# salemmohammed/Distributed-TensorFlow-Guide

Hardware: AMD Instinct MI355X
Metric: images/sec (whole node) ResNet-50 sync DP at 1/2/4/8 MI355X; scaling efficiency (higher is better)
Workload: dtype bf16; 1 GPU; model=ResNet-50, global_batch=1024, per_gpu_batch=1024, image_size=224, optimizer=momentum-sgd (fused), parallelism=dp1, allreduce=rccl bf16, 8 MB buckets, overlapped, step_launch=eager

## Files before the change

csrc/bindings/ops.cc:

```cpp
#include <torch/extension.h>
#include <c10/core/DeviceGuard.h>
#include <c10/hip/HIPStream.h>

#include "dtg/kernels.h"

namespace {

using at::Tensor;
using dtg::bf16_t;

hipStream_t cur_stream() { return c10::hip::getCurrentHIPStream().stream(); }

at::Tensor zeros_f32(long long n, const at::Tensor& like) {
  c10::DeviceGuard dg(like.device());
  at::Tensor t = at::empty({n}, like.options().dtype(at::kFloat));
  dtg::fill_zero(t.data_ptr(), n * 4, cur_stream());
  return t;
}

#define CHECK_CUDA(x) TORCH_CHECK((x).is_cuda(), #x " must be a GPU tensor")
#define CHECK_CONTIG(x) TORCH_CHECK((x).is_contiguous(), #x " must be contiguous")
#define CHECK_DT(x, dt) TORCH_CHECK((x).scalar_type() == (dt), #x " must be " #dt)
#define CHECK_IN(x) \
  CHECK_CUDA(x);    \
// ... 304 lines not shown
  TORCH_CHECK(C % 8 == 0, "C must be a multiple of 8");
  for (const Tensor* t : {&gamma, &beta, &rmean, &rvar}) {
    CHECK_IN(*t);
    CHECK_DT(*t, at::kFloat);
    TORCH_CHECK(t->numel() == C, "per-channel tensor size mismatch");
  }
  if (res.has_value() && res->defined()) {
    CHECK_IN(*res);
    CHECK_DT(*res, at::kBFloat16);
    TORCH_CHECK(res->sizes() == x.sizes(), "residual shape mismatch");
  }
  c10::DeviceGuard dg(x.device());
  auto y = at::empty_like(x);
  auto fopt = x.options().dtype(at::kFloat);
  auto smean = at::empty({C}, fopt), sinv = at::empty({C}, fopt);
  auto ws = at::empty({dtg::bn_workspace_floats(M, C)}, fopt);
  dtg::bn_fwd_train(cbfp(x), res.has_value() && res->defined() ? cbfp(*res) : nullptr, bfp(y),
                    gamma.data_ptr<float>(), beta.data_ptr<float>(), rmean.data_ptr<float>(), rvar.data_ptr<float>(),
                    smean.data_ptr<float>(), sinv.data_ptr<float>(), ws.data_ptr<float>(), M, C, (float)momentum,
                    (float)eps, relu, cur_stream());
  return {y, smean, sinv};
}

Tensor bn_fwd_infer(Tensor x, c10::optional<Tensor> res, Tensor gamma, Tensor beta, Tensor rmean, Tensor rvar,
                    double eps, bool relu) {
  CHECK_IN(x);
  CHECK_DT(x, at::kBFloat16);
  TORCH_CHECK(x.dim() == 2, "x must be [M, C]");
  const long long M = x.size(0);
  const int C = (int)x.size(1);
  TORCH_CHECK(C % 8 == 0, "C must be a multiple of 8");
  for (const Tensor* t : {&gamma, &beta, &rmean, &rvar}) {
    CHECK_IN(*t);
    CHECK_DT(*t, at::kFloat);
    TORCH_CHECK(t->numel() == C, "per-channel tensor size mismatch");
  }
  if (res.has_value() && res->defined()) {
    CHECK_IN(*res);
    TORCH_CHECK(res->sizes() == x.sizes(), "residual shape mismatch");
  }
  c10::DeviceGuard dg(x.device());
  auto y = at::empty_like(x);
  auto ws = at::empty({2LL * C}, x.options().dtype(at::kFloat));
  dtg::bn_fwd_infer(cbfp(x), res.has_value() && res->defined() ? cbfp(*res) : nullptr, bfp(y),
                    gamma.data_ptr<float>(), beta.data_ptr<float>(), rmean.data_ptr<float>(), rvar.data_ptr<float>(),
                    ws.data_ptr<float>(), M, C, (float)eps, relu, cur_stream());
  return y;
}

std::tuple<Tensor, c10::optional<Tensor>, Tensor, Tensor> bn_bwd(Tensor dy, c10::optional<Tensor> y, Tensor x,
                                                                  Tensor gamma, Tensor smean, Tensor sinv, bool relu,
                                                                  bool want_dres, c10::optional<Tensor> dgamma_acc,
                                                                  c10::optional<Tensor> dbeta_acc) {
  CHECK_IN(dy);
  CHECK_IN(x);
  CHECK_DT(dy, at::kBFloat16);
  CHECK_DT(x, at::kBFloat16);
  TORCH_CHECK(dy.sizes() == x.sizes() && x.dim() == 2, "dy/x must be [M, C]");
  const long long M = x.size(0);
  const int C = (int)x.size(1);
  TORCH_CHECK(C % 8 == 0, "C must be a multiple of 8");
  if (relu) {
    TORCH_CHECK(y.has_value() && y->defined(), "relu backward needs the saved output");
    CHECK_IN(*y);
    TORCH_CHECK(y->sizes() == x.sizes(), "y shape mismatch");
  }
  for (const Tensor* t : {&gamma, &smean, &sinv}) {
    CHECK_IN(*t);
    CHECK_DT(*t, at::kFloat);
    TORCH_CHECK(t->numel() == C, "per-channel tensor size mismatch");
  }
  c10::DeviceGuard dg(x.device());
  auto dx = at::empty_like(x);
  c10::optional<Tensor> dres;
  if (want_dres) dres = at::empty_like(x);
  auto fopt = x.options().dtype(at::kFloat);
  const bool acc = dgamma_acc.has_value() && dgamma_acc->defined() && dbeta_acc.has_value() && dbeta_acc->defined();
  Tensor dgamma, dbeta;
  if (acc) {
    dgamma = *dgamma_acc;
    dbeta = *dbeta_acc;
    for (const Tensor* t : {&dgamma, &dbeta}) {
      CHECK_IN(*t);
      CHECK_DT(*t, at::kFloat);
      TORCH_CHECK(t->numel() == C, "gradient accumulator size mismatch");
    }
  } else {
    dgamma = at::empty({C}, fopt);
    dbeta = at::empty({C}, fopt);
  }
  auto ws = at::empty({dtg::bn_workspace_floats(M, C) + C}, fopt);
  dtg::bn_bwd(cbfp(dy), relu ? cbfp(*y) : nullptr, cbfp(x), gamma.data_ptr<float>(), smean.data_ptr<float>(),
              sinv.data_ptr<float>(), bfp(dx), want_dres ? bfp(*dres) : nullptr, dgamma.data_ptr<float>(),
              dbeta.data_ptr<float>(), ws.data_ptr<float>(), M, C, relu, acc, cur_stream());
  return {dx, dres, dgamma, dbeta};
}

std::tuple<Tensor, c10::optional<Tensor>, Tensor> softmax_xent(Tensor logits, Tensor labels, double scale,
                                                                bool want_grad) {
  CHECK_IN(logits);
  CHECK_IN(labels);
  TORCH_CHECK(logits.dim() == 2, "logits must be [B, V]");
  TORCH_CHECK(logits.scalar_type() == at::kBFloat16 || logits.scalar_type() == at::kFloat, "logits bf16/fp32");
  CHECK_DT(labels, at::kLong);
  TORCH_CHECK(labels.numel() == logits.size(0), "labels size mismatch");
  c10::DeviceGuard dg(logits.device());
  const long long B = logits.size(0);
  const int V = (int)logits.size(1);
  auto fopt = logits.options().dtype(at::kFloat);
  auto loss = at::empty({B}, fopt), lse = at::empty({B}, fopt);
  c10::optional<Tensor> dx;
  if (want_grad) dx = at::empty_like(logits);
  if (B > 0)
    dtg::softmax_xent(logits.data_ptr(), logits.scalar_type() == at::kBFloat16, reinterpret_cast<const long long*>(labels.data_ptr<int64_t>()), B, V,
                      (float)scale, loss.data_ptr<float>(), want_grad ? dx->data_ptr() : nullptr,
                      lse.data_ptr<float>(), cur_stream());
  return {loss, dx, lse};
}

Tensor softmax_xent_bwd(Tensor logits, Tensor labels, Tensor lse, Tensor g, double scale) {
  CHECK_IN(logits);
  CHECK_IN(labels);
  CHECK_IN(lse);
  TORCH_CHECK(logits.dim() == 2, "logits must be [B, V]");
  TORCH_CHECK(logits.scalar_type() == at::kBFloat16 || logits.scalar_type() == at::kFloat, "logits bf16/fp32");
  CHECK_DT(labels, at::kLong);
  CHECK_DT(lse, at::kFloat);
  const long long B = logits.size(0);
  const int V = (int)logits.size(1);
  TORCH_CHECK(labels.numel() == B && lse.numel() == B, "labels / lse size mismatch");
  CHECK_CUDA(g);
  TORCH_CHECK(g.numel() == 1, "g must hold one element");
  Tensor gf = g.scalar_type() == at::kFloat ? g.contiguous() : g.to(at::kFloat);
  c10::DeviceGuard dg(logits.device());
  auto dx = at::empty_like(logits);
  if (B > 0)
    dtg::softmax_xent_bwd(logits.data_ptr(), logits.scalar_type() == at::kBFloat16,
                          reinterpret_cast<const long long*>(labels.data_ptr<int64_t>()), lse.data_ptr<float>(), B, V,
                          (float)scale, gf.data_ptr<float>(), dx.data_ptr(), cur_stream());
  return dx;
}

void gemm(Tensor A, bool a_kc, Tensor B, bool b_kc, Tensor out, double alpha, double beta,
          c10::optional<Tensor> bias, int64_t act, int64_t split_k, c10::optional<Tensor> aux, int64_t aux_mode,
          c10::optional<Tensor> colsum) {
  CHECK_CUDA(A);
  CHECK_CUDA(B);
  CHECK_CUDA(out);
  CHECK_DT(A, at::kBFloat16);
  CHECK_DT(B, at::kBFloat16);
  TORCH_CHECK(A.dim() == 2 && B.dim() == 2 && out.dim() == 2, "gemm operands must be 2-D");
  TORCH_CHECK(A.stride(1) == 1 && B.stride(1) == 1 && out.stride(1) == 1, "inner dim must be contiguous");
  TORCH_CHECK(out.scalar_type() == at::kFloat || out.scalar_type() == at::kBFloat16, "out fp32/bf16");
  const int M = (int)(a_kc ? A.size(0) : A.size(1));
  const int K = (int)(a_kc ? A.size(1) : A.size(0));
  const int N = (int)(b_kc ? B.size(0) : B.size(1));
  const int Kb = (int)(b_kc ? B.size(1) : B.size(0));
  TORCH_CHECK(K == Kb, "gemm K mismatch: ", K, " vs ", Kb);
  TORCH_CHECK(out.size(0) == M && out.size(1) == N, "gemm out shape mismatch");
  TORCH_CHECK(K % 8 == 0 || (!a_kc && !b_kc), "K-contiguous operands need K % 8 == 0 (pad the reduction dim)");
  TORCH_CHECK(a_kc || M % 8 == 0, "K-major A needs M % 8 == 0");
  TORCH_CHECK(b_kc || N % 8 == 0, "K-major B needs N % 8 == 0");
  TORCH_CHECK(A.stride(0) % 8 == 0 && B.stride(0) % 8 == 0, "row strides must be 16-byte multiples");
  TORCH_CHECK(((uintptr_t)A.data_ptr() % 16) == 0 && ((uintptr_t)B.data_ptr() % 16) == 0, "16-byte alignment");
  const float* bptr = nullptr;
  if (bias.has_value() && bias->defined()) {
    CHECK_IN(*bias);
    CHECK_DT(*bias, at::kFloat);
    TORCH_CHECK(bias->numel() == N, "bias size mismatch");
    bptr = bias->data_ptr<float>();
  }
  void* auxp = nullptr;
  if (aux_mode != 0) {
    TORCH_CHECK(aux_mode >= 1 && aux_mode <= 4, "aux_mode in {0, 1, 2, 3, 4}");
    TORCH_CHECK(aux_mode != 3 || act != 0, "aux_mode 3 stores act'(pre): needs an activation");
    TORCH_CHECK(aux.has_value() && aux->defined(), "aux_mode needs an aux tensor");
    TORCH_CHECK(aux->is_cuda() && aux->scalar_type() == at::kBFloat16 && aux->dim() == 2, "aux must be bf16 2-D");
    TORCH_CHECK(aux->size(0) == M && aux->size(1) == N && aux->stride(0) == out.stride(0) && aux->stride(1) == 1,
                "aux must match out's shape and row stride");
    auxp = aux->data_ptr();
  }
  c10::DeviceGuard dg(A.device());
  if (colsum.has_value() && colsum->defined()) {
    CHECK_IN(*colsum);
    CHECK_DT(*colsum, at::kFloat);
    TORCH_CHECK(colsum->numel() == N, "colsum must hold N floats");
    TORCH_CHECK(a_kc && !b_kc && out.scalar_type() == at::kBFloat16 && alpha == 1.0 && beta == 0.0,
                "colsum epilogue: A [M,K], B [K,N], bf16 out, alpha 1, beta 0");
    TORCH_CHECK(out.stride(0) % 8 == 0 && N % 8 == 0 && ((uintptr_t)out.data_ptr() % 16) == 0 &&
                    (bptr == nullptr || ((uintptr_t)bptr % 16) == 0) && (auxp == nullptr || ((uintptr_t)auxp % 16) == 0),
                "colsum epilogue needs 16-byte aligned rows");
    dtg::gemm_bf16_colsum(cbfp(A), A.stride(0), cbfp(B), B.stride(0), bfp(out), out.stride(0), M, N, K, bptr, (int)act,
                          auxp, (int)aux_mode, colsum->data_ptr<float>(), cur_stream());
    return;
  }
  int sk = split_k > 0 ? (int)split_k : dtg::gemm_pick_split(M, N, K, a_kc ? 1 : 0);
  Tensor ws;
  float* wsp = nullptr;
  if (sk > 1) {
    ws = at::empty({dtg::gemm_workspace_floats(M, N, K, sk)}, A.options().dtype(at::kFloat));
    wsp = ws.data_ptr<float>();
  }
  dtg::gemm_bf16(cbfp(A), A.stride(0), a_kc, cbfp(B), B.stride(0), b_kc, out.data_ptr(), out.stride(0),
                 out.scalar_type() == at::kBFloat16, M, N, K, (float)alpha, (float)beta, bptr, (int)act, sk, wsp,
                 cur_stream(), dtg::GemmBatch(), auxp, (int)aux_mode);
}

void check_nhwc(const Tensor& t, const char* what) {
  CHECK_CUDA(t);
  TORCH_CHECK(t.scalar_type() == at::kBFloat16, what, " must be bf16");
  TORCH_CHECK(t.dim() == 4 && t.is_contiguous(), what, " must be a contiguous [N,H,W,C] tensor");
  TORCH_CHECK(((uintptr_t)t.data_ptr() % 16) == 0, what, " must be 16-byte aligned");
}

bool conv_supported(int64_t C, int64_t K, int64_t R, int64_t S, int64_t stride, int64_t pad, int64_t which) {
  return dtg::conv_supported((int)C, (int)K, (int)R, (int)S, (int)stride, (int)pad, (int)which) != 0;
}

Tensor conv_fwd(Tensor x, Tensor w, int64_t stride, int64_t pad) {
  check_nhwc(x, "x");
  check_nhwc(w, "w");
  const int N = x.size(0), H = x.size(1), W = x.size(2), C = x.size(3);
  const int K = w.size(0), R = w.size(1), S = w.size(2);
  TORCH_CHECK(w.size(3) == C, "weight channels mismatch");
  TORCH_CHECK(dtg::conv_supported(C, K, R, S, stride, pad, 0), "conv shape not supported by the HIP kernel");
  const int P = (H + 2 * pad - R) / stride + 1, Q = (W + 2 * pad - S) / stride + 1;
  TORCH_CHECK(P > 0 && Q > 0, "empty output");
  TORCH_CHECK((long long)N * H * W * C < (1LL << 31) && (long long)N * P * Q * K < (1LL << 31), "tensor too large");
  c10::DeviceGuard dg(x.device());
  auto y = at::empty({N, P, Q, K}, x.options());
  dtg::conv_fwd(cbfp(x), cbfp(w), bfp(y), N, H, W, C, K, R, S, stride, pad, cur_stream());
  return y;
}


Tensor conv_dgrad(Tensor dy, Tensor w, int64_t H, int64_t W, int64_t stride, int64_t pad, c10::optional<Tensor> out,
                  double beta, bool zero_rest) {
  check_nhwc(dy, "dy");
  check_nhwc(w, "w");
  const int N = dy.size(0), P = dy.size(1), Q = dy.size(2), K = dy.size(3);
  const int R = w.size(1), S = w.size(2), C = w.size(3);
  TORCH_CHECK(w.size(0) == K, "weight/dy channel mismatch");
  TORCH_CHECK(dtg::conv_supported(C, K, R, S, stride, pad, 1), "dgrad shape not supported by the HIP kernel");
  TORCH_CHECK((H + 2 * pad - R) / stride + 1 == P && (W + 2 * pad - S) / stride + 1 == Q, "dgrad geometry mismatch");
  c10::DeviceGuard dg(dy.device());
  Tensor dx;
  if (out.has_value()) {
    dx = *out;
    check_nhwc(dx, "out");
    TORCH_CHECK(dx.size(0) == N && dx.size(1) == H && dx.size(2) == W && dx.size(3) == C, "out shape mismatch");
  } else {
    TORCH_CHECK(beta == 0.0, "beta != 0 needs out");
    dx = at::empty({N, H, W, C}, dy.options());
  }
  Tensor wT;
  TORCH_CHECK(zero_rest || (stride == 2 && R == 1 && S == 1 && pad == 0 && beta == 0.0),
              "zero_rest=False is for a stride-2 1x1 dgrad (beta 0)");
  dtg::conv_dgrad(cbfp(dy), cbfp(w), bfp(dx), N, H, W, C, K, R, S, stride, pad, (float)beta, cur_stream(),
                  dtg::BnEpi(), wT.defined() ? cbfp(wT) : nullptr, zero_rest ? 1 : 0);
  return dx;
}

std::tuple<Tensor, Tensor> conv_fwd_c8(Tensor x, Tensor w, int64_t R, int64_t S, int64_t stride, int64_t pad,
                                       bool with_stats, int64_t stride_w) {
  check_nhwc(x, "x");
  CHECK_IN(w);
  CHECK_DT(w, at::kBFloat16);
  const int sw = stride_w > 0 ? (int)stride_w : (int)stride;
  const int N = x.size(0), H = x.size(1), W = x.size(2), K = w.size(0);
  TORCH_CHECK(x.size(3) == 8, "conv_fwd_c8 needs 8 input channels");
  TORCH_CHECK(w.dim() == 2 && w.size(1) == (R * S * 8 + 63) / 64 * 64, "w must be [K, ceil64(R*S*8)]");
  TORCH_CHECK(K % 64 == 0, "K % 64");
  TORCH_CHECK(stride > 0 && sw > 0 && pad >= 0, "bad stride / pad");
  const int P = (H + 2 * pad - R) / stride + 1, Q = (W + 2 * pad - S) / sw + 1;
  TORCH_CHECK(P > 0 && Q > 0 && (long long)N * P * Q * K < (1LL << 31), "bad geometry");
  c10::DeviceGuard dg(x.device());
  auto y = at::empty({N, P, Q, K}, x.options());
  Tensor part;
  dtg::BnEpi bn;
  if (with_stats) {
    part = zeros_f32((long long)dtg::kBnStatSlots * 2 * K, x);
    bn.part = part.data_ptr<float>();
    bn.mode = 1;
  } else {
    part = at::empty({0}, x.options().dtype(at::kFloat));
  }
  dtg::conv_fwd_c8(cbfp(x), cbfp(w), bfp(y), N, H, W, K, (int)R, (int)S, (int)stride, (int)pad, cur_stream(), bn, sw);
  return {y, part};
}

constexpr int kPartRing = 16;
constexpr long long kPartCap = (long long)dtg::kBnStatSlots * 2 * 2048;
Tensor bn_part(const Tensor& like, int64_t C, bool pooled = false) {
  if (!pooled || C > 2048) return zeros_f32((long long)dtg::kBnStatSlots * 2 * C, like);
  static Tensor* ring = new Tensor[64];
  static int next[64] = {0};
  const int dev = like.get_device();
  TORCH_CHECK(dev >= 0 && dev < 64, "device index");
  if (!ring[dev].defined()) ring[dev] = zeros_f32((long long)kPartRing * kPartCap, like);
  const int i = next[dev]++ % kPartRing;
  return ring[dev].narrow(0, i * kPartCap, (long long)dtg::kBnStatSlots * 2 * C);
}

dtg::BnEpi bn_bwd_epi(Tensor& part, const Tensor& x, const Tensor& mean, const Tensor& invstd, const Tensor& gamma,
                      const Tensor& beta, long long M, int C) {
  CHECK_IN(x);
  CHECK_DT(x, at::kBFloat16);
  TORCH_CHECK(x.numel() == M * C, "BN input shape mismatch");
  for (const Tensor* t : {&mean, &invstd, &gamma, &beta}) {
    CHECK_IN(*t);
    CHECK_DT(*t, at::kFloat);
    TORCH_CHECK(t->numel() == C, "per-channel tensor size mismatch");
  }
  dtg::BnEpi bn;
  bn.part = part.data_ptr<float>();
  bn.mode = 2;
  bn.x = cbfp(x);
  bn.mean = mean.data_ptr<float>();
  bn.invstd = invstd.data_ptr<float>();
  bn.gamma = gamma.data_ptr<float>();
  bn.beta = beta.data_ptr<float>();
  return bn;
}

std::tuple<Tensor, Tensor> gemm_bn(Tensor A, Tensor B, int64_t mode, c10::optional<Tensor> x,
                                   c10::optional<Tensor> mean, c10::optional<Tensor> invstd,
                                   c10::optional<Tensor> gamma, c10::optional<Tensor> beta,
                                   c10::optional<Tensor> mask, c10::optional<Tensor> out, bool pooled,
                                   c10::optional<Tensor> x2, c10::optional<Tensor> mean2,
                                   c10::optional<Tensor> invstd2, c10::optional<Tensor> part2,
                                   c10::optional<std::tuple<int64_t, int64_t>> sub2_hw) {
  CHECK_IN(A);
  CHECK_DT(A, at::kBFloat16);
  CHECK_CUDA(B);
  CHECK_DT(B, at::kBFloat16);
  TORCH_CHECK(mode >= 1 && mode <= 3, "mode in {1, 2, 3}");
  TORCH_CHECK(A.dim() == 2 && B.dim() == 2 && B.stride(1) == 1, "2-D operands, contiguous rows");
  const int M = (int)A.size(0), K = (int)A.size(1);
  const int N = (int)(mode == 1 ? B.size(0) : B.size(1));
  TORCH_CHECK((mode == 1 ? B.size(1) : B.size(0)) == K, "gemm_bn K mismatch");
  TORCH_CHECK(K % 8 == 0 && N % 8 == 0 && B.stride(0) % 8 == 0, "K, N and row strides must be multiples of 8");
  TORCH_CHECK(((uintptr_t)A.data_ptr() % 16) == 0 && ((uintptr_t)B.data_ptr() % 16) == 0, "16-byte alignment");
  c10::DeviceGuard dg(A.device());
  Tensor o;
  float bt = 0.f;
  if (out.has_value() && out->defined()) {
    TORCH_CHECK(mode == 3, "accumulating into `out` is mode 3 only");
    o = *out;
    CHECK_IN(o);
    CHECK_DT(o, at::kBFloat16);
    TORCH_CHECK(o.numel() == (long long)M * N, "out shape mismatch");
    bt = 1.f;
  } else {
    o = at::empty({M, N}, A.options());
  }
  auto part = bn_part(A, N, pooled);
  dtg::BnEpi bn;
  if (mode >= 2) {
    TORCH_CHECK(x && mean && invstd && gamma && beta, "modes 2/3 need x, mean, invstd, gamma, beta");
    bn = bn_bwd_epi(part, *x, *mean, *invstd, *gamma, *beta, M, N);
    if (mode == 3) {
      TORCH_CHECK(mask.has_value() && mask->defined(), "mode 3 needs the mask tensor");
      CHECK_IN(*mask);
      bn.mode = 3;
      if (x2.has_value() && x2->defined()) {
        TORCH_CHECK(mean2 && invstd2 && part2, "x2 needs mean2, invstd2 and part2");
        CHECK_IN(*x2);
        CHECK_DT(*x2, at::kBFloat16);
        TORCH_CHECK(x2->numel() == (long long)M * N, "x2 shape mismatch");
        for (const Tensor* t : {&*mean2, &*invstd2}) {
          CHECK_IN(*t);
          CHECK_DT(*t, at::kFloat);
          TORCH_CHECK(t->numel() == N, "per-channel tensor size mismatch");
        }
        CHECK_IN(*part2);
        CHECK_DT(*part2, at::kFloat);
        TORCH_CHECK(part2->numel() == (long long)dtg::kBnStatSlots * 2 * N, "part2 size mismatch");
        bn.x2 = cbfp(*x2);
        bn.mean2 = mean2->data_ptr<float>();
        bn.invstd2 = invstd2->data_ptr<float>();
        bn.part2 = part2->data_ptr<float>();
      }
      if (sub2_hw.has_value()) {
        const auto [sh, sw] = *sub2_hw;
        TORCH_CHECK(bt != 0.f && sh > 0 && sw > 0 && (long long)M % (sh * sw) == 0, "sub2_hw needs out and M = N*H*W");
        dtg::bn_sub2_rows(bn, (int)sh, (int)sw);
      }
      if (mask->scalar_type() == at::kByte) {
        TORCH_CHECK(mask->numel() == (long long)M * (N / 8), "mask bits shape mismatch");
        bn.maskbits = mask->data_ptr<uint8_t>();
      } else {
        CHECK_DT(*mask, at::kBFloat16);
        TORCH_CHECK(mask->numel() == (long long)M * N, "mask shape mismatch");
        bn.mask = cbfp(*mask);
      }
    }
  } else {
    bn.part = part.data_ptr<float>();
    bn.mode = 1;
  }
  dtg::gemm_bf16_bn(cbfp(A), A.stride(0), cbfp(B), B.stride(0), bfp(o), N, M, N, K, bt, bn, cur_stream());
  return {o, part};
}

std::tuple<Tensor, Tensor> conv_fwd_bn(Tensor x, Tensor w, int64_t stride, int64_t pad, bool pooled) {
  check_nhwc(x, "x");
  check_nhwc(w, "w");
  const int N = x.size(0), H = x.size(1), W = x.size(2), C = x.size(3);
  const int K = w.size(0), R = w.size(1), S = w.size(2);
  TORCH_CHECK(w.size(3) == C, "weight channels mismatch");
  TORCH_CHECK(dtg::conv_supported(C, K, R, S, stride, pad, 0), "conv shape not supported by the HIP kernel");
  const int P = (H + 2 * pad - R) / stride + 1, Q = (W + 2 * pad - S) / stride + 1;
  TORCH_CHECK(P > 0 && Q > 0, "empty output");
  TORCH_CHECK((long long)N * H * W * C < (1LL << 31) && (long long)N * P * Q * K < (1LL << 31), "tensor too large");
  c10::DeviceGuard dg(x.device());
  auto y = at::empty({N, P, Q, K}, x.options());
  auto part = bn_part(x, K, pooled);
  dtg::BnEpi bn;
  bn.part = part.data_ptr<float>();
  bn.mode = 1;
  dtg::conv_fwd(cbfp(x), cbfp(w), bfp(y), N, H, W, C, K, R, S, stride, pad, cur_stream(), bn);
  return {y, part};
}

uint8_t* bits_ptr(const c10::optional<Tensor>& bits, long long M, int C) {
  if (!bits.has_value() || !bits->defined()) return nullptr;
  CHECK_IN(*bits);
  TORCH_CHECK(bits->scalar_type() == at::kByte && bits->numel() == M * (C / 8), "bits must be uint8 [M, C/8]");
  return bits->data_ptr<uint8_t>();
}

std::tuple<Tensor, Tensor> conv_dgrad_bn(Tensor dy, Tensor w, int64_t H, int64_t W, int64_t stride, int64_t pad,
                                         Tensor x, Tensor mean, Tensor invstd, Tensor gamma, Tensor beta,
                                         bool pooled, c10::optional<Tensor> bits) {
  check_nhwc(dy, "dy");
  check_nhwc(w, "w");
  const int N = dy.size(0), P = dy.size(1), Q = dy.size(2), K = dy.size(3);
  const int R = w.size(1), S = w.size(2), C = w.size(3);
  TORCH_CHECK(w.size(0) == K, "weight/dy channel mismatch");
  TORCH_CHECK(dtg::conv_supported(C, K, R, S, stride, pad, 1), "dgrad shape not supported by the HIP kernel");
  TORCH_CHECK((H + 2 * pad - R) / stride + 1 == P && (W + 2 * pad - S) / stride + 1 == Q, "dgrad geometry mismatch");
  c10::DeviceGuard dg(dy.device());
  auto dx = at::empty({N, H, W, C}, dy.options());
  auto part = bn_part(dy, C, pooled);
  dtg::BnEpi bn = bn_bwd_epi(part, x, mean, invstd, gamma, beta, (long long)N * H * W, C);
  if (uint8_t* mb = bits_ptr(bits, (long long)N * H * W, C)) {
    bn.mode = 3;
    bn.maskbits = mb;
  }
  Tensor wT;
  TORCH_CHECK(dtg::conv_dgrad(cbfp(dy), cbfp(w), bfp(dx), N, H, W, C, K, R, S, stride, pad, 0.f, cur_stream(), bn,
                              wT.defined() ? cbfp(wT) : nullptr),
              "conv_dgrad_bn: geometry leaves rows unwritten (use conv_dgrad + bn_bwd)");
  return {dx, part};
}

std::tuple<Tensor, Tensor, Tensor> bn_fwd_part(Tensor x, Tensor part, c10::optional<Tensor> res, Tensor gamma,
                                               Tensor beta, Tensor rmean, Tensor rvar, double momentum, double eps,
                                               bool relu, c10::optional<Tensor> bits) {
  CHECK_IN(x);
  CHECK_DT(x, at::kBFloat16);
  TORCH_CHECK(x.dim() == 2, "x must be [M, C]");
  const long long M = x.size(0);
  const int C = (int)x.size(1);
  TORCH_CHECK(C % 8 == 0, "C must be a multiple of 8");
  CHECK_IN(part);
  CHECK_DT(part, at::kFloat);
  TORCH_CHECK(part.numel() == (long long)dtg::kBnStatSlots * 2 * C, "partials size mismatch");
  for (const Tensor* t : {&gamma, &beta, &rmean, &rvar}) {
    CHECK_IN(*t);
    CHECK_DT(*t, at::kFloat);
    TORCH_CHECK(t->numel() == C, "per-channel tensor size mismatch");
  }
  const bool has_res = res.has_value() && res->defined();
  if (has_res) {
    CHECK_IN(*res);
    CHECK_DT(*res, at::kBFloat16);
    TORCH_CHECK(res->sizes() == x.sizes(), "residual shape mismatch");
  }
  c10::DeviceGuard dg(x.device());
  auto y = at::empty_like(x);
  auto fopt = x.options().dtype(at::kFloat);
  auto smean = at::empty({C}, fopt), sinv = at::empty({C}, fopt), ws = at::empty({2LL * C}, fopt);
  dtg::bn_fwd_from_part(cbfp(x), has_res ? cbfp(*res) : nullptr, bfp(y), gamma.data_ptr<float>(),
                        beta.data_ptr<float>(), rmean.data_ptr<float>(), rvar.data_ptr<float>(),
                        smean.data_ptr<float>(), sinv.data_ptr<float>(), part.data_ptr<float>(), ws.data_ptr<float>(),
                        M, C, (float)momentum, (float)eps, relu, cur_stream(), bits_ptr(bits, M, C));
  return {y, smean, sinv};
}

std::tuple<Tensor, Tensor, Tensor, Tensor, Tensor> bn_fwd2_part(Tensor x, Tensor part, Tensor gamma, Tensor beta,
                                                                Tensor rmean, Tensor rvar, Tensor r, Tensor part2,
                                                                Tensor gamma2, Tensor beta2, Tensor rmean2,
                                                                Tensor rvar2, double momentum, double eps,
                                                                c10::optional<Tensor> bits) {
  CHECK_IN(x);
  CHECK_IN(r);
  CHECK_DT(x, at::kBFloat16);
  CHECK_DT(r, at::kBFloat16);
  TORCH_CHECK(x.dim() == 2 && r.sizes() == x.sizes(), "x/r must be [M, C]");
  const long long M = x.size(0);
  const int C = (int)x.size(1);
  TORCH_CHECK(C % 8 == 0, "C must be a multiple of 8");
  for (const Tensor* t : {&part, &part2}) {
    CHECK_IN(*t);
    CHECK_DT(*t, at::kFloat);
    TORCH_CHECK(t->numel() == (long long)dtg::kBnStatSlots * 2 * C, "partials size mismatch");
  }
  for (const Tensor* t : {&gamma, &beta, &rmean, &rvar, &gamma2, &beta2, &rmean2, &rvar2}) {
    CHECK_IN(*t);
    CHECK_DT(*t, at::kFloat);
    TORCH_CHECK(t->numel() == C, "per-channel tensor size mismatch");
  }
  c10::DeviceGuard dg(x.device());
  auto y = at::empty_like(x);
  auto fopt = x.options().dtype(at::kFloat);
  auto m1 = at::empty({C}, fopt), i1 = at::empty({C}, fopt), m2 = at::empty({C}, fopt), i2 = at::empty({C}, fopt);
  auto ws = at::empty({4LL * C}, fopt);
  dtg::bn_fwd2_from_part(cbfp(x), cbfp(r), bfp(y), part.data_ptr<float>(), part2.data_ptr<float>(),
                         gamma.data_ptr<float>(), beta.data_ptr<float>(), rmean.data_ptr<float>(),
                         rvar.data_ptr<float>(), m1.data_ptr<float>(), i1.data_ptr<float>(), gamma2.data_ptr<float>(),
                         beta2.data_ptr<float>(), rmean2.data_ptr<float>(), rvar2.data_ptr<float>(),
                         m2.data_ptr<float>(), i2.data_ptr<float>(), ws.data_ptr<float>(), M, C, (float)momentum,
                         (float)eps, cur_stream(), bits_ptr(bits, M, C));
  return {y, m1, i1, m2, i2};
}

static void check_wgrad_fuse(const Tensor& x, const c10::optional<Tensor>& wact, const c10::optional<Tensor>& wgrad) {
  TORCH_CHECK(wact.has_value() && wgrad.has_value() && wact->defined() && wgrad->defined(), "wact needs wgrad");
  CHECK_CUDA(*wact);
  CHECK_DT(*wact, at::kBFloat16);
  CHECK_IN(*wgrad);
  TORCH_CHECK(wgrad->scalar_type() == at::kFloat || wgrad->scalar_type() == at::kBFloat16, "wgrad fp32/bf16");
  const long long M = x.size(0);
  const int C = (int)x.size(1), CI = (int)wact->size(1);
  TORCH_CHECK(wact->dim() == 2 && wact->size(0) == M && wact->stride(1) == 1 && wact->stride(0) % 8 == 0 &&
                  ((uintptr_t)wact->data_ptr() % 16) == 0,
              "wact must be [M, CI] with 16-byte aligned rows");
  TORCH_CHECK(wgrad->numel() == (long long)C * CI, "wgrad must be [C, CI]");
  TORCH_CHECK(dtg::bn_dx_wgrad_ok(M, C, CI), "fused dx + wgrad: unsupported shape (see bn_dx_wgrad_ok)");
}

std::tuple<Tensor, Tensor> bn_bwd2_part(Tensor dp, Tensor x, Tensor part, Tensor gamma, Tensor smean, Tensor sinv,
                                        Tensor dgamma, Tensor dbeta, Tensor x2, Tensor part2, Tensor gamma2,
                                        Tensor smean2, Tensor sinv2, Tensor dgamma2, Tensor dbeta2,
                                        c10::optional<Tensor> wact, c10::optional<Tensor> wgrad,
                                        c10::optional<Tensor> wact2, c10::optional<Tensor> wgrad2) {
  for (const Tensor* t : {&dp, &x, &x2}) {
    CHECK_IN(*t);
    CHECK_DT(*t, at::kBFloat16);
  }
  TORCH_CHECK(x.dim() == 2 && dp.numel() == x.numel() && x2.sizes() == x.sizes(), "dp/x/x2 must be [M, C]");
  const long long M = x.size(0);
  const int C = (int)x.size(1);
  TORCH_CHECK(C % 8 == 0, "C must be a multiple of 8");
  for (const Tensor* t : {&part, &part2}) {
    CHECK_IN(*t);
    CHECK_DT(*t, at::kFloat);
    TORCH_CHECK(t->numel() == (long long)dtg::kBnStatSlots * 2 * C, "partials size mismatch");
  }
  for (const Tensor* t : {&gamma, &smean, &sinv, &dgamma, &dbeta, &gamma2, &smean2, &sinv2, &dgamma2, &dbeta2}) {
    CHECK_IN(*t);
    CHECK_DT(*t, at::kFloat);
    TORCH_CHECK(t->numel() == C, "per-channel tensor size mismatch");
  }
  c10::DeviceGuard dg(x.device());
  auto dx = at::empty_like(x), dx2 = at::empty_like(x);
  auto ws = at::empty({6LL * C}, x.options().dtype(at::kFloat));
  if (wact.has_value() && wact->defined()) {
    check_wgrad_fuse(x, wact, wgrad);
    const int CI = (int)wact->size(1);
    const bool w2 = wact2.has_value() && wact2->defined();
    if (w2) {
      check_wgrad_fuse(x2, wact2, wgrad2);
      TORCH_CHECK(C == 256 && CI == 64 && wact2->size(1) == CI && wgrad2->scalar_type() == wgrad->scalar_type(),
                  "wact2: 256 x 64 only, wgrad2 of wgrad's dtype");
    }
    const long long ns = (long long)dtg::bn_dx_wgrad_slabs(C, CI, w2) * C * CI;
    auto slabs = at::empty({w2 ? 2 * ns : ns}, x.options().dtype(at::kFloat));
    float* w = ws.data_ptr<float>();
    dtg::bn_bwd_coef_from_part(part.data_ptr<float>(), gamma.data_ptr<float>(), smean.data_ptr<float>(),
                               sinv.data_ptr<float>(), w, dgamma.data_ptr<float>(), dbeta.data_ptr<float>(), M, C, 1,
                               cur_stream());
    dtg::bn_bwd_coef_from_part(part2.data_ptr<float>(), gamma2.data_ptr<float>(), smean2.data_ptr<float>(),
                               sinv2.data_ptr<float>(), w + 3LL * C, dgamma2.data_ptr<float>(),
                               dbeta2.data_ptr<float>(), M, C, 1, cur_stream());
    dtg::bn_dx_wgrad(cbfp(dp), cbfp(x), w, cbfp(x2), w + 3LL * C, bfp(dx), bfp(dx2), cbfp(*wact), wact->stride(0),
                     wgrad->data_ptr(), wgrad->scalar_type() == at::kBFloat16, slabs.data_ptr<float>(), M, C, CI,
                     cur_stream(), w2 ? cbfp(*wact2) : nullptr, w2 ? wact2->stride(0) : 0,
                     w2 ? wgrad2->data_ptr() : nullptr, w2 ? slabs.data_ptr<float>() + ns : nullptr);
    return {dx, dx2};
  }
  dtg::bn_bwd2_from_part(cbfp(dp), cbfp(x), cbfp(x2), part.data_ptr<float>(), part2.data_ptr<float>(),
                         gamma.data_ptr<float>(), smean.data_ptr<float>(), sinv.data_ptr<float>(),
                         gamma2.data_ptr<float>(), smean2.data_ptr<float>(), sinv2.data_ptr<float>(), bfp(dx),
                         bfp(dx2), dgamma.data_ptr<float>(), dbeta.data_ptr<float>(), dgamma2.data_ptr<float>(),
                         dbeta2.data_ptr<float>(), ws.data_ptr<float>(), M, C, 1, cur_stream());
  return {dx, dx2};
}

std::tuple<Tensor, c10::optional<Tensor>, Tensor, Tensor> bn_bwd_part(Tensor dp, Tensor x, Tensor part, Tensor gamma,
                                                                       Tensor smean, Tensor sinv, bool want_dres,
                                                                       c10::optional<Tensor> dgamma_acc,
                                                                       c10::optional<Tensor> dbeta_acc,
                                                                       c10::optional<Tensor> wact,
                                                                       c10::optional<Tensor> wgrad) {
  CHECK_IN(dp);
  CHECK_IN(x);
  CHECK_DT(dp, at::kBFloat16);
  CHECK_DT(x, at::kBFloat16);
  TORCH_CHECK(x.dim() == 2 && dp.numel() == x.numel(), "dp/x must be [M, C]");
  const long long M = x.size(0);
  const int C = (int)x.size(1);
  TORCH_CHECK(C % 8 == 0, "C must be a multiple of 8");
  CHECK_IN(part);
  CHECK_DT(part, at::kFloat);
  TORCH_CHECK(part.numel() == (long long)dtg::kBnStatSlots * 2 * C, "partials size mismatch");
  for (const Tensor* t : {&gamma, &smean, &sinv}) {
    CHECK_IN(*t);
    CHECK_DT(*t, at::kFloat);
    TORCH_CHECK(t->numel() == C, "per-channel tensor size mismatch");
  }
  c10::DeviceGuard dg(x.device());
  auto dx = at::empty_like(x);
  c10::optional<Tensor> dres;
  if (want_dres) dres = at::empty_like(x);
  auto fopt = x.options().dtype(at::kFloat);
  const bool acc = dgamma_acc.has_value() && dgamma_acc->defined() && dbeta_acc.has_value() && dbeta_acc->defined();
  Tensor dgamma, dbeta;
  if (acc) {
    dgamma = *dgamma_acc;
    dbeta = *dbeta_acc;
    for (const Tensor* t : {&dgamma, &dbeta}) {
      CHECK_IN(*t);
      CHECK_DT(*t, at::kFloat);
      TORCH_CHECK(t->numel() == C, "gradient accumulator size mismatch");
    }
  } else {
    dgamma = at::empty({C}, fopt);
    dbeta = at::empty({C}, fopt);
  }
  auto ws = at::empty({3LL * C}, fopt);
  if (wact.has_value() && wact->defined()) {
    TORCH_CHECK(!want_dres, "fused dx + wgrad: no dres");
    check_wgrad_fuse(x, wact, wgrad);
    const int CI = (int)wact->size(1);
    auto slabs = at::empty({(long long)dtg::bn_dx_wgrad_slabs(C, CI) * C * CI}, fopt);
    dtg::bn_bwd_coef_from_part(part.data_ptr<float>(), gamma.data_ptr<float>(), smean.data_ptr<float>(),
                               sinv.data_ptr<float>(), ws.data_ptr<float>(), dgamma.data_ptr<float>(),
                               dbeta.data_ptr<float>(), M, C, acc, cur_stream());
    dtg::bn_dx_wgrad(cbfp(dp), cbfp(x), ws.data_ptr<float>(), nullptr, nullptr, bfp(dx), nullptr, cbfp(*wact),
                     wact->stride(0), wgrad->data_ptr(), wgrad->scalar_type() == at::kBFloat16, slabs.data_ptr<float>(),
                     M, C, CI, cur_stream());
    return {dx, dres, dgamma, dbeta};
  }
  dtg::bn_bwd_from_part(cbfp(dp), cbfp(x), gamma.data_ptr<float>(), smean.data_ptr<float>(), sinv.data_ptr<float>(),
                        part.data_ptr<float>(), bfp(dx), want_dres ? bfp(*dres) : nullptr, dgamma.data_ptr<float>(),
                        dbeta.data_ptr<float>(), ws.data_ptr<float>(), M, C, acc, cur_stream());
  return {dx, dres, dgamma, dbeta};
}

void conv_wgrad(Tensor dy, Tensor x, Tensor dw, double beta, int64_t stride, int64_t pad, int64_t stride_w,
                int64_t target_wgs, int64_t sched) {
  check_nhwc(dy, "dy");
  check_nhwc(x, "x");
  CHECK_CUDA(dw);
  TORCH_CHECK(dw.dim() == 4 && dw.is_contiguous(), "dw must be contiguous [K,R,S,C]");
  TORCH_CHECK(dw.scalar_type() == at::kFloat || dw.scalar_type() == at::kBFloat16, "dw fp32/bf16");
  const int N = x.size(0), H = x.size(1), W = x.size(2), C = x.size(3);
  const int K = dw.size(0), R = dw.size(1), S = dw.size(2);
  TORCH_CHECK(dw.size(3) == C && dy.size(3) == K && dy.size(0) == N, "wgrad shape mismatch");
  TORCH_CHECK(dtg::conv_supported(C, K, R, S, stride, pad, 2), "wgrad shape not supported by the HIP kernel");
  const int sw = stride_w > 0 ? (int)stride_w : (int)stride;
  const int P = (H + 2 * pad - R) / stride + 1, Q = (W + 2 * pad - S) / sw + 1;
  TORCH_CHECK(dy.size(1) == P && dy.size(2) == Q, "wgrad geometry mismatch");
  c10::DeviceGuard dg(x.device());
  const int split = dtg::conv_wgrad_split(N, H, W, C, K, R, S, stride, pad, sw, (int)target_wgs);
  auto ws = at::empty({(long long)split * K * R * S * C}, x.options().dtype(at::kFloat));
  dtg::conv_wgrad(cbfp(dy), cbfp(x), dw.data_ptr(), dw.scalar_type() == at::kBFloat16, (float)beta,
                  ws.data_ptr<float>(), split, N, H, W, C, K, R, S, stride, pad, cur_stream(), sw, (int)sched);
}

}

void register_transformer_ops(pybind11::module_& m);
void register_pool_ops(pybind11::module_& m);

PYBIND11_MODULE(TORCH_EXTENSION_NAME, m) {
  m.def("conv_supported", &conv_supported);
  m.def("conv_fwd", &conv_fwd);
  m.def("conv_dgrad", &conv_dgrad, pybind11::arg("dy"), pybind11::arg("w"), pybind11::arg("H"), pybind11::arg("W"),
        pybind11::arg("stride"), pybind11::arg("pad"), pybind11::arg("out") = pybind11::none(),
        pybind11::arg("beta") = 0.0, pybind11::arg("zero_rest") = true);
  m.def("conv_wgrad", &conv_wgrad, pybind11::arg("dy"), pybind11::arg("x"), pybind11::arg("dw"),
        pybind11::arg("beta"), pybind11::arg("stride"), pybind11::arg("pad"), pybind11::arg("stride_w") = 0,
        pybind11::arg("target_wgs") = 0, pybind11::arg("sched") = 0);
  m.def("gemm_bn", &gemm_bn, pybind11::arg("A"), pybind11::arg("B"), pybind11::arg("mode"),
        pybind11::arg("x") = pybind11::none(), pybind11::arg("mean") = pybind11::none(),
        pybind11::arg("invstd") = pybind11::none(), pybind11::arg("gamma") = pybind11::none(),
        pybind11::arg("beta") = pybind11::none(), pybind11::arg("mask") = pybind11::none(),
        pybind11::arg("out") = pybind11::none(), pybind11::arg("pooled") = false,
        pybind11::arg("x2") = pybind11::none(), pybind11::arg("mean2") = pybind11::none(),
        pybind11::arg("invstd2") = pybind11::none(), pybind11::arg("part2") = pybind11::none(),
        pybind11::arg("sub2_hw") = pybind11::none());
  m.def("bn_part_alloc", [](Tensor like, int64_t C, bool pooled) { return bn_part(like, C, pooled); },
        pybind11::arg("like"), pybind11::arg("C"), pybind11::arg("pooled") = false);
  m.def("bn_bwd2_part", &bn_bwd2_part, pybind11::arg("dp"), pybind11::arg("x"), pybind11::arg("part"),
        pybind11::arg("gamma"), pybind11::arg("smean"), pybind11::arg("sinv"), pybind11::arg("dgamma"),
        pybind11::arg("dbeta"), pybind11::arg("x2"), pybind11::arg("part2"), pybind11::arg("gamma2"),
        pybind11::arg("smean2"), pybind11::arg("sinv2"), pybind11::arg("dgamma2"), pybind11::arg("dbeta2"),
        pybind11::arg("wact") = pybind11::none(), pybind11::arg("wgrad") = pybind11::none(),
        pybind11::arg("wact2") = pybind11::none(), pybind11::arg("wgrad2") = pybind11::none());
  m.def("bn_dx_wgrad_ok", [](int64_t M, int64_t C, int64_t CI) { return dtg::bn_dx_wgrad_ok(M, (int)C, (int)CI); });
  m.def("conv_fwd_bn", &conv_fwd_bn, pybind11::arg("x"), pybind11::arg("w"), pybind11::arg("stride"),
        pybind11::arg("pad"), pybind11::arg("pooled") = false);
  m.def("conv_dgrad_bn", &conv_dgrad_bn, pybind11::arg("dy"), pybind11::arg("w"), pybind11::arg("H"),
        pybind11::arg("W"), pybind11::arg("stride"), pybind11::arg("pad"), pybind11::arg("x"), pybind11::arg("mean"),
        pybind11::arg("invstd"), pybind11::arg("gamma"), pybind11::arg("beta"), pybind11::arg("pooled") = false,
        pybind11::arg("bits") = pybind11::none());
  m.def("bn_fwd2_part", &bn_fwd2_part, pybind11::arg("x"), pybind11::arg("part"), pybind11::arg("gamma"),
        pybind11::arg("beta"), pybind11::arg("rmean"), pybind11::arg("rvar"), pybind11::arg("r"), pybind11::arg("part2"),
        pybind11::arg("gamma2"), pybind11::arg("beta2"), pybind11::arg("rmean2"), pybind11::arg("rvar2"),
        pybind11::arg("momentum"), pybind11::arg("eps"), pybind11::arg("bits") = pybind11::none());
  m.def("conv_fwd_c8", &conv_fwd_c8, pybind11::arg("x"), pybind11::arg("w"), pybind11::arg("R"), pybind11::arg("S"),
        pybind11::arg("stride"), pybind11::arg("pad"), pybind11::arg("with_stats") = false,
        pybind11::arg("stride_w") = 0);
  m.def("bn_fwd_part", &bn_fwd_part, pybind11::arg("x"), pybind11::arg("part"), pybind11::arg("res"),
        pybind11::arg("gamma"), pybind11::arg("beta"), pybind11::arg("rmean"), pybind11::arg("rvar"),
        pybind11::arg("momentum"), pybind11::arg("eps"), pybind11::arg("relu"), pybind11::arg("bits") = pybind11::none());
  m.def("bn_bwd_part", &bn_bwd_part, pybind11::arg("dp"), pybind11::arg("x"), pybind11::arg("part"),
        pybind11::arg("gamma"), pybind11::arg("smean"), pybind11::arg("sinv"), pybind11::arg("want_dres"),
        pybind11::arg("dgamma_acc") = pybind11::none(), pybind11::arg("dbeta_acc") = pybind11::none(),
        pybind11::arg("wact") = pybind11::none(), pybind11::arg("wgrad") = pybind11::none());
  m.doc() = "dtg gfx950 HIP kernels";
  m.def("sgd_apply", &sgd_apply);
  m.def("momentum_apply", &momentum_apply);
  m.def("adagrad_apply", &adagrad_apply);
  m.def("adam_apply", &adam_apply);
  m.def("axpby", &axpby);
  m.def("sgd_sum_apply", &sgd_sum_apply);
  m.def("momentum_sum_apply", &momentum_sum_apply);
  m.def("adagrad_sum_apply", &adagrad_sum_apply);
  m.def("adam_sum_apply", &adam_sum_apply);
  m.def("grad_sum", &grad_sum);
  m.def("state_chunk_table", &state_chunk_table);
  m.def("state_pack", &state_pack);
  m.def("state_unpack", &state_unpack);
  m.def("comm_spin", [](double seconds, int64_t wgs, int64_t lds_bytes) {
    dtg::comm_spin(seconds, (int)wgs, (int)lds_bytes, cur_stream());
  }, pybind11::arg("seconds"), pybind11::arg("wgs") = 32, pybind11::arg("lds_bytes") = 0);
  m.def("comm_emu", [](double seconds, int64_t wgs, int64_t mode, c10::optional<Tensor> scratch, int64_t base,
                       int64_t traffic_bytes, c10::optional<Tensor> bucket, double factor) {
    long long sbytes = 0, n = 0;
    int bf = 0;
    const Tensor* dev_t = nullptr;
    if (scratch.has_value() && scratch->defined()) {
      CHECK_IN(*scratch);
      TORCH_CHECK(((uintptr_t)scratch->data_ptr() % 16) == 0, "scratch: 16-B aligned");
      sbytes = scratch->numel() * scratch->element_size();
      dev_t = &*scratch;
    }
    if (bucket.has_value() && bucket->defined()) {
      CHECK_IN(*bucket);
      TORCH_CHECK(bucket->scalar_type() == at::kFloat || bucket->scalar_type() == at::kBFloat16, "bucket fp32/bf16");
      n = bucket->numel();
      bf = bucket->scalar_type() == at::kBFloat16;
      dev_t = &*bucket;
    }
    TORCH_CHECK(!(mode & 2) || sbytes > 0, "traffic mode needs scratch");
    TORCH_CHECK(!(mode & 4) || n > 0 || !(bucket.has_value() && bucket->defined()), "data mode needs the bucket");
    c10::optional<c10::DeviceGuard> dg;
    if (dev_t) dg.emplace(dev_t->device());
    return dtg::comm_emu(seconds, (int)wgs, (int)mode, sbytes ? scratch->data_ptr() : nullptr, sbytes, base,
                         traffic_bytes, n ? bucket->data_ptr() : nullptr, n, bf, (float)factor, cur_stream());
  }, pybind11::arg("seconds"), pybind11::arg("wgs") = 32, pybind11::arg("mode") = 0,
        pybind11::arg("scratch") = pybind11::none(), pybind11::arg("base") = 0, pybind11::arg("traffic_bytes") = 0,
        pybind11::arg("bucket") = pybind11::none(), pybind11::arg("factor") = 1.0);
  m.def("stem_stream_set", [](int64_t on) { dtg::stem_stream_set((int)on); });
  m.def("gemm_expand_k256_set", [](int64_t on) { dtg::gemm_expand_k256_set((int)on); });
  m.def("stem_pool_rows_set", [](int64_t on) { dtg::stem_pool_rows_set((int)on); });
  m.def("gemm_expand_s2_set", [](int64_t on) { dtg::gemm_expand_s2_set((int)on); });
  m.def("conv_halo_fwd_set", [](int64_t on) { dtg::conv3x3_halo_fwd_set((int)on); });
  m.def("conv_halo_dgrad_set", [](int64_t on) { dtg::conv3x3_halo_dgrad_set((int)on); });
  m.def("conv_halo_wgrad_set", [](int64_t on) { dtg::conv3x3_halo_wgrad_set((int)on); });
  m.def("conv_lin_wgrad_set", [](int64_t on) { dtg::conv3x3_lin_wgrad_set((int)on); });
  m.def("hyper_tick", [](Tensor hyper) {
    check_hyper(hyper);
    c10::DeviceGuard dg(hyper.device());
    dtg::hyper_tick(hyper.data_ptr<float>(), cur_stream());
  });
  m.def("stem_pack_weights", [](Tensor w) {
    CHECK_CUDA(w);
    CHECK_DT(w, at::kBFloat16);
    TORCH_CHECK(w.dim() == 4 && w.is_contiguous(at::MemoryFormat::ChannelsLast) && w.size(1) <= 4,
                "w: channels_last [K, C<=4, R, S]");
    const int K = w.size(0), C = w.size(1), R = w.size(2), S = w.size(3), S2 = (S + 1) / 2;
    const int KP = (R * S2 * 8 + 63) / 64 * 64;
    c10::DeviceGuard dg(w.device());
    auto wp = at::empty({K, KP}, w.options().memory_format(at::MemoryFormat::Contiguous));
    dtg::stem_pack_weights(cbfp(w), bfp(wp), K, C, R, S, S2, KP, cur_stream());
    return wp;
  });
  m.def("stem_dw_add", [](Tensor src, Tensor grad, bool pair) {
    CHECK_IN(src);
    CHECK_DT(src, at::kFloat);
    CHECK_CUDA(grad);
    TORCH_CHECK(grad.dim() == 4 && grad.is_contiguous(at::MemoryFormat::ChannelsLast), "grad: channels_last [K,C,R,S]");
    TORCH_CHECK(grad.scalar_type() == at::kFloat || grad.scalar_type() == at::kBFloat16, "grad fp32/bf16");
    const int K = grad.size(0), C = grad.size(1), R = grad.size(2), S = grad.size(3);
    TORCH_CHECK(src.dim() == 4 && src.size(0) == K && src.size(1) == R && src.size(3) == 8 && C <= 4 &&
                    src.size(2) == (pair ? (S + 1) / 2 : S), "stem dw source shape");
    c10::DeviceGuard dg(grad.device());
    dtg::stem_dw_add(src.data_ptr<float>(), grad.data_ptr(), grad.scalar_type() == at::kBFloat16, K, R, S, C,
                     (int)src.size(2), pair ? 1 : 0, cur_stream());
  });
  m.def("stream_probe", [](int64_t kind, Tensor a, c10::optional<Tensor> b, c10::optional<Tensor> o, Tensor sink,
                           int64_t wgs, int64_t unroll, bool nt) {
    CHECK_IN(a);
    CHECK_IN(sink);
    TORCH_CHECK(sink.scalar_type() == at::kInt && sink.numel() >= wgs, "sink: int32 with >= wgs elements");
    const long long bytes = a.numel() * a.element_size();
    TORCH_CHECK(bytes % 16 == 0 && ((uintptr_t)a.data_ptr() % 16) == 0, "a: 16-B multiple, 16-B aligned");
    for (const auto* t : {&b, &o})
      if (t->has_value() && (*t)->defined()) {
        CHECK_IN(**t);
        TORCH_CHECK((*t)->numel() * (*t)->element_size() == bytes && ((uintptr_t)(*t)->data_ptr() % 16) == 0,
                    "b / o: the byte size of a, 16-B aligned");
      }
    TORCH_CHECK(kind >= 0 && kind <= 3, "kind 0..3");
    TORCH_CHECK(kind == 0 || (o.has_value() && o->defined()), "kinds 1-3 write o");
    TORCH_CHECK(kind != 3 || (b.has_value() && b->defined()), "kind 3 reads b");
    TORCH_CHECK(wgs >= 1 && wgs <= 65536, "wgs");
    c10::DeviceGuard dg(a.device());
    dtg::stream_probe((int)kind, a.data_ptr(), opt_ptr<void>(b), opt_ptr<void>(o), bytes / 16,
                      reinterpret_cast<unsigned*>(sink.data_ptr()), (int)wgs, (int)unroll, nt ? 1 : 0, cur_stream());
  }, pybind11::arg("kind"), pybind11::arg("a"), pybind11::arg("b") = pybind11::none(),
        pybind11::arg("o") = pybind11::none(), pybind11::arg("sink"), pybind11::arg("wgs") = 1024,
        pybind11::arg("unroll") = 4, pybind11::arg("nt") = false);
  m.def("launch_probe", [](int64_t grid, int64_t lds_bytes) {
    dtg::launch_probe((int)grid, (int)lds_bytes, cur_stream());
  });
  m.def("f32_to_bf16", &f32_to_bf16);
  m.def("bn_fwd_train", &bn_fwd_train);
  m.def("bn_fwd_infer", &bn_fwd_infer);
  m.def("bn_bwd", &bn_bwd, pybind11::arg("dy"), pybind11::arg("y"), pybind11::arg("x"), pybind11::arg("gamma"),
        pybind11::arg("smean"), pybind11::arg("sinv"), pybind11::arg("relu"), pybind11::arg("want_dres"),
        pybind11::arg("dgamma_acc") = pybind11::none(), pybind11::arg("dbeta_acc") = pybind11::none());
  m.def("softmax_xent", &softmax_xent);
  m.def("gemm_bn_force_cfg", [](int64_t c) { dtg::gemm_bn_force_cfg((int)c); });
  m.def("conv_force_tile", [](int64_t which, int64_t c) { dtg::conv_force_tile((int)which, (int)c); });
  m.def("conv_set_stages", [](int64_t which, int64_t s) { dtg::conv_set_stages((int)which, (int)s); });
  m.def("softmax_xent_bwd", &softmax_xent_bwd);
  m.def("gemm_pick_split", [](int64_t M, int64_t N, int64_t K, bool a_kc, int64_t target_wgs) {
    return dtg::gemm_pick_split((int)M, (int)N, (int)K, a_kc ? 1 : 0, (int)target_wgs);
  }, pybind11::arg("M"), pybind11::arg("N"), pybind11::arg("K"), pybind11::arg("a_kc") = false,
        pybind11::arg("target_wgs") = 0);
  m.def("gemm", &gemm, pybind11::arg("A"), pybind11::arg("a_kc"), pybind11::arg("B"), pybind11::arg("b_kc"),
        pybind11::arg("out"), pybind11::arg("alpha") = 1.0, pybind11::arg("beta") = 0.0,
        pybind11::arg("bias") = pybind11::none(), pybind11::arg("act") = 0, pybind11::arg("split_k") = 0,
        pybind11::arg("aux") = pybind11::none(), pybind11::arg("aux_mode") = 0,
        pybind11::arg("colsum") = pybind11::none());
  register_transformer_ops(m);
  register_pool_ops(m);
}
```

csrc/include/dtg/kernels.h:

```cpp
#pragma once
#include <hip/hip_runtime.h>
#include <stdint.h>

namespace dtg {
typedef unsigned short bf16_t;

void sgd_apply(float* w, bf16_t* mirror, void* grad, int grad_bf16, long long n, const float* hyper, float wd,
               float gscale, int zero_grad, hipStream_t st);
void momentum_apply(float* w, bf16_t* mirror, void* grad, int grad_bf16, float* mom, long long n,
                    const float* hyper, float mu, float wd, int nesterov, float gscale, int zero_grad,
                    hipStream_t st);
void adagrad_apply(float* w, bf16_t* mirror, void* grad, int grad_bf16, float* acc, long long n,
                   const float* hyper, float eps, float gscale, int zero_grad, hipStream_t st);
void adam_apply(float* w, bf16_t* mirror, void* grad, int grad_bf16, float* m, float* v, long long n,
                const float* hyper, float b1, float b2, float eps, float wd, float gscale, int zero_grad,
                hipStream_t st);
void axpby(float* acc, const void* g, int g_bf16, long long n, float alpha, float beta, hipStream_t st);
void f32_to_bf16(const float* x, bf16_t* y, long long n, hipStream_t st);
void hyper_tick(float* hyper, hipStream_t st);
struct GradSrcs {
  const void* p[8] = {nullptr, nullptr, nullptr, nullptr, nullptr, nullptr, nullptr, nullptr};
};
void sgd_sum_apply(float* w, bf16_t* mirror, const float* acc, const GradSrcs& src, int k, int src_bf16, long long n,
                   const float* hyper, float wd, float gscale, hipStream_t st);
void momentum_sum_apply(float* w, bf16_t* mirror, const float* acc, const GradSrcs& src, int k, int src_bf16,
                        float* mom, long long n, const float* hyper, float mu, float wd, int nesterov, float gscale,
                        hipStream_t st);
void adagrad_sum_apply(float* w, bf16_t* mirror, const float* acc, const GradSrcs& src, int k, int src_bf16,
                       float* slot, long long n, const float* hyper, float eps, float gscale, hipStream_t st);
void adam_sum_apply(float* w, bf16_t* mirror, const float* acc, const GradSrcs& src, int k, int src_bf16, float* m,
                    float* v, long long n, const float* hyper, float b1, float b2, float eps, float wd, float gscale,
                    hipStream_t st);
void grad_sum(float* acc, const GradSrcs& src, int k, int src_bf16, long long n, int first, float scale,
              hipStream_t st);
constexpr int kMaxStateSrcs = 4;
constexpr int kStateChunk = 2048;
struct StatePtrs {
  float* p[4] = {nullptr, nullptr, nullptr, nullptr};
};
void state_pack(const StatePtrs& src, int k, float* image, long long n, const long long* rows, const int* chunks,
                int n_chunks, hipStream_t st);
void state_unpack(const StatePtrs& dst, int k, const float* image, long long n, const long long* rows,
                  const int* chunks, int n_chunks, hipStream_t st);
void mul_bf16(const bf16_t* a, const bf16_t* b, bf16_t* out, long long n, hipStream_t st);
void mask_additive(const void* mask, int is_f32, float* out, long long n, hipStream_t st);
void fill_zero(void* p, long long bytes, hipStream_t st);

void comm_spin(double seconds, int wgs, int lds_bytes, hipStream_t st);
long long comm_emu(double seconds, int wgs, int mode, void* scratch, long long scratch_bytes, long long base,
                   long long traffic_bytes, void* buf, long long n, int buf_bf16, float factor, hipStream_t st);
void launch_probe(int grid, int lds_bytes, hipStream_t st);
void stream_probe(int kind, const void* a, const void* b, void* o, long long n16, unsigned* sink, int wgs, int unroll,
                  int nt, hipStream_t st);

constexpr int kBnStatSlots = 32;
struct BnEpi {
  float* part = nullptr;
  int mode = 0;
  const bf16_t* x = nullptr;
  const float* mean = nullptr;
  const float* invstd = nullptr;
  const float* gamma = nullptr;
  const float* beta = nullptr;
  const bf16_t* mask = nullptr;
  const uint8_t* maskbits = nullptr;
  const bf16_t* x2 = nullptr;
  const float* mean2 = nullptr;
  const float* invstd2 = nullptr;
  float* part2 = nullptr;
  int old_sub2 = 0;
  uint32_t old_hw = 1, old_w = 1, hw_m = 0, hw_l = 0, w_m = 0, w_l = 0;
};

inline void bn_sub2_rows(BnEpi& bn, int H, int W) {
  auto magic = [](uint32_t d, uint32_t& m, uint32_t& l) {
    l = 0;
    while ((1u << l) < d) ++l;
    m = (uint32_t)((((uint64_t)1 << 32) * (((uint64_t)1 << l) - d)) / d + 1);
  };
  bn.old_sub2 = 1;
  bn.old_hw = (uint32_t)(H * W);
  bn.old_w = (uint32_t)W;
  magic(bn.old_hw, bn.hw_m, bn.hw_l);
  magic(bn.old_w, bn.w_m, bn.w_l);
}

long long bn_workspace_floats(long long M, int C);
void bn_fwd_from_part(const bf16_t* x, const bf16_t* res, bf16_t* y, const float* gamma, const float* beta,
                      float* rmean, float* rvar, float* smean, float* sinv, const float* part, float* ws, long long M,
                      int C, float momentum, float eps, int relu, hipStream_t st, uint8_t* bits = nullptr);
void bn_fwd2_from_part(const bf16_t* x, const bf16_t* r, bf16_t* y, const float* part, const float* part2,
                       const float* gamma, const float* beta, float* rmean, float* rvar, float* smean, float* sinv,
                       const float* gamma2, const float* beta2, float* rmean2, float* rvar2, float* smean2,
                       float* sinv2, float* ws, long long M, int C, float momentum, float eps, hipStream_t st,
                       uint8_t* bits = nullptr);
void bn_bwd2_from_part(const bf16_t* dp, const bf16_t* x, const bf16_t* x2, const float* part, const float* part2,
                       const float* gamma, const float* smean, const float* sinv, const float* gamma2,
                       const float* smean2, const float* sinv2, bf16_t* dx, bf16_t* dx2, float* dgamma, float* dbeta,
                       float* dgamma2, float* dbeta2, float* ws, long long M, int C, int accum, hipStream_t st);
void bn_bwd_coef_from_part(const float* part, const float* gamma, const float* smean, const float* sinv, float* coef,
                           float* dgamma, float* dbeta, long long M, int C, int accum, hipStream_t st);
void bn_dx_from_coef(const bf16_t* dp, const bf16_t* x, const float* coef, bf16_t* dx, bf16_t* dres, long long M, int C,
                     hipStream_t st);
bool bn_dx_wgrad_ok(long long M, int C, int CI);
int bn_dx_wgrad_slabs(int C, int CI, int w2 = 0);
void bn_dx_wgrad(const bf16_t* dp, const bf16_t* x, const float* coef, const bf16_t* x2, const float* coef2,
                 bf16_t* dx, bf16_t* dx2, const bf16_t* act, long long ldact, void* wgrad, int wgrad_bf16,
                 float* slabs, long long M, int C, int CI, hipStream_t st, const bf16_t* act2 = nullptr,
                 long long ldact2 = 0, void* wgrad2 = nullptr, float* slabs2 = nullptr);
void bn_bwd_from_part(const bf16_t* dp, const bf16_t* x, const float* gamma, const float* smean, const float* sinv,
                      const float* part, bf16_t* dx, bf16_t* dres, float* dgamma, float* dbeta, float* ws, long long M,
                      int C, int accum, hipStream_t st);
void bn_fwd_train(const bf16_t* x, const bf16_t* res, bf16_t* y, const float* gamma, const float* beta,
                  float* rmean, float* rvar, float* smean, float* sinv, float* ws, long long M, int C,
                  float momentum, float eps, int relu, hipStream_t st);
void bn_fwd_infer(const bf16_t* x, const bf16_t* res, bf16_t* y, const float* gamma, const float* beta,
                  const float* rmean, const float* rvar, float* ws, long long M, int C, float eps, int relu,
                  hipStream_t st);
void bn_bwd(const bf16_t* dy, const bf16_t* y, const bf16_t* x, const float* gamma, const float* smean,
            const float* sinv, bf16_t* dx, bf16_t* dres, float* dgamma, float* dbeta, float* ws, long long M, int C,
            int relu, int accum, hipStream_t st);

void softmax_xent(const void* x, int x_bf16, const long long* label, long long B, int V, float scale, float* loss,
                  void* dx, float* lse, hipStream_t st);
void softmax_xent_bwd(const void* x, int x_bf16, const long long* label, const float* lse, long long B, int V,
                      float scale, const float* g, void* dx, hipStream_t st);

struct GemmBatch {
  int count = 1, nh = 1;
  long long sa_b = 0, sa_h = 0, sb_b = 0, sb_h = 0, sc_b = 0, sc_h = 0;
};
void gemm_bn_force_cfg(int cfg);
void conv_force_tile(int which, int code);
long long gemm_workspace_floats(int M, int N, int K, int split_k);
int gemm_pick_split(int M, int N, int K, int a_kc = 0, int target_wgs = 0);
void gemm_bf16(const bf16_t* A, long long lda, int a_kc, const bf16_t* B, long long ldb, int b_kc, void* C,
               long long ldc, int c_bf16, int M, int N, int K, float alpha, float beta, const float* bias, int act,
               int split_k, float* ws, hipStream_t st, const GemmBatch& batch = GemmBatch(), void* aux = nullptr,
               int aux_mode = 0);
void gemm_bf16_bn(const bf16_t* A, long long lda, const bf16_t* B, long long ldb, bf16_t* C, long long ldc, int M,
                  int N, int K, float beta, const BnEpi& bn, hipStream_t st);
void gemm_bf16_colsum(const bf16_t* A, long long lda, const bf16_t* B, long long ldb, bf16_t* C, long long ldc, int M,
                      int N, int K, const float* bias, int act, void* aux, int aux_mode, float* colsum, hipStream_t st);

int ln_max_hidden();
void ln_fwd(const bf16_t* h, const bf16_t* res, const float* gamma, const float* beta, bf16_t* y, bf16_t* s_out,
            float* mean, float* rstd, int T, int H, float eps, float p_in, uint32_t seed_in, float p_out,
            uint32_t seed_out, hipStream_t st);
int ln_bwd_blocks(int T);
void ln_bwd(const bf16_t* dy, const bf16_t* s, const float* gamma, const float* mean, const float* rstd,
            bf16_t* ds_out, bf16_t* dh_out, float* dgamma, float* dbeta, float* dbias, float* ws, int T, int H,
            float p_in, uint32_t seed_in, float p_out, uint32_t seed_out, hipStream_t st);
int attn_max_keys();
void attn_softmax_fwd(const float* sc, const float* mask, bf16_t* P, bf16_t* Pd, int rows, int rows_per_b, int Sk,
                      float p, uint32_t seed, hipStream_t st);
void attn_softmax_bwd(const bf16_t* P, const bf16_t* Pd, const float* dPd, bf16_t* dS, int rows, int Sk, float scale,
                      hipStream_t st);
int colsum_splits(int T, int N);
void colsum(const bf16_t* x, long long ld, int T, int N, const long long* sel, int nsel, void* out, int out_bf16,
            int accumulate, float* ws, int splits, hipStream_t st);
void emb_fwd(const long long* ids, const long long* tt, const bf16_t* word, const bf16_t* pos, const bf16_t* type,
             bf16_t* s, int T, int S, int H, hipStream_t st);
void emb_word_bwd(const bf16_t* ds, const long long* sorted, const long long* perm, bf16_t* gW, int T, int H,
                  hipStream_t st);
void emb_pos_bwd(const bf16_t* ds, bf16_t* gP, int T, int S, int H, hipStream_t st);

void gather_rows(const bf16_t* src, const long long* pos, bf16_t* out, int R, int P, int S, int H, hipStream_t st);
void scatter_rows_add(bf16_t* dst, const long long* pos, const bf16_t* src, int R, int P, int S, int H,
                      hipStream_t st);
void nsp_loss_fwd(const bf16_t* pooled, const bf16_t* wn, const float* bn, const long long* labels, const float* extra,
                  float* probs, float* out, int B, int H, hipStream_t st);
void nsp_loss_bwd(const bf16_t* pooled, const bf16_t* wn, const float* probs, const long long* labels, const float* gout,
                  bf16_t* dpre, bf16_t* gwn, float* gbn, int B, int H, hipStream_t st);
void row_sum(const float* x, float* out, long long n, float scale, hipStream_t st);
void emb_word_bwd_owned(const bf16_t* ds, const long long* ids, bf16_t* gW, int T, int H, int V, hipStream_t st);

int attn_fused_supported(int S, int dh, int backward);
void attn_fwd(const bf16_t* qkv, const float* mask, bf16_t* out, float* lse, int B, int S, int nh, float p,
              uint32_t seed, hipStream_t st);
void attn_bwd(const bf16_t* qkv, const bf16_t* o, const bf16_t* dout, const float* lse, const float* mask,
              bf16_t* dqkv, int B, int S, int nh, float p, uint32_t seed, float* dbias, hipStream_t st);

void maxpool_fwd(const bf16_t* x, bf16_t* y, uint8_t* idx, int N, int H, int W, int C, int k, int s, int pad, int P,
                 int Q, hipStream_t st);
void maxpool_bwd(const bf16_t* dy, const uint8_t* idx, bf16_t* dx, int N, int H, int W, int C, int k, int s, int pad,
                 int P, int Q, hipStream_t st);
void avgpool_fwd(const bf16_t* x, bf16_t* y, int N, int HW, int C, hipStream_t st);
void avgpool_bwd(const bf16_t* dy, bf16_t* dx, int N, int HW, int C, hipStream_t st);

void stem_bn_pool_fwd(const bf16_t* y, const float* part, const float* gamma, const float* beta, float* rmean,
                      float* rvar, float* smean, float* sinv, float* coef, bf16_t* out, uint8_t* idx, int N, int H,
                      int W, int C, int k, int s, int pad, int P, int Q, float momentum, float eps, hipStream_t st,
                      bf16_t* yam = nullptr);
long long stem_bwd_workspace_floats(long long M, int C);
bool stem_pooled_stats_ok(int C);
void stem_pack_weights(const bf16_t* w, bf16_t* wp, int K, int C, int R, int S, int S2, int KP, hipStream_t st);
void stem_dw_add(const float* src, void* grad, int grad_bf16, int K, int R, int S, int C, int S2, int pair,
                 hipStream_t st);
void stem_pack_pairs(const bf16_t* x, bf16_t* xp, int N, int H, int W, int C, int pad, int Hp, int Wp,
                     hipStream_t st);
void stem_bn_pool_bwd(const bf16_t* dout, const uint8_t* idx, const bf16_t* y, const float* gamma, const float* beta,
                      const float* smean, const float* sinv, bf16_t* dy, float* dgamma, float* dbeta, int accum,
                      float* ws, int N, int H, int W, int C, int k, int s, int pad, int P, int Q, hipStream_t st,
                      const bf16_t* yam = nullptr);

void im2col(const bf16_t* x, bf16_t* cols, int N, int H, int W, int C, int R, int S, int stride, int pad, int Kp,
            hipStream_t st);
void col2im(const bf16_t* dcols, bf16_t* dx, int N, int H, int W, int C, int R, int S, int stride, int pad, int Kp,
            hipStream_t st);

int conv_supported(int C, int K, int R, int S, int stride, int pad, int which);
int conv3x3_halo_bn_ok(int C, int K, int H, int W);
bool conv3x3_halo_bn_fwd(const bf16_t* x, const bf16_t* w, bf16_t* y, int N, int H, int W, float* part, hipStream_t st);
void conv3x3_halo_fwd_set(int on);
bool conv3x3_halo_bn_dgrad(const bf16_t* dy, const bf16_t* w, bf16_t* dp, int N, int H, int W, const BnEpi& bn,
                           hipStream_t st);
void conv3x3_halo_dgrad_set(int on);
int conv3x3_halo_wgrad_split(int N, int H, int W, int C, int K, int R, int S, int stride, int pad, int stride_w);
void conv3x3_halo_wgrad(const bf16_t* dy, const bf16_t* x, float* ws, int grid, int N, int H, hipStream_t st);
void conv3x3_halo_wgrad_set(int on);
int conv3x3_lin_wgrad_split(int N, int H, int W, int C, int K, int R, int S, int stride, int pad, int stride_w);
void conv3x3_lin_wgrad(const bf16_t* dy, const bf16_t* x, float* ws, int split, int N, int H, int W, int C, int K,
                       hipStream_t st);
void conv3x3_lin_wgrad_set(int on);
void conv_fwd(const bf16_t* x, const bf16_t* w, bf16_t* y, int N, int H, int W, int C, int K, int R, int S,
              int stride, int pad, hipStream_t st, const BnEpi& bn = BnEpi());
int conv_dgrad(const bf16_t* dy, const bf16_t* w, bf16_t* dx, int N, int H, int W, int C, int K, int R, int S,
               int stride, int pad, float beta, hipStream_t st, const BnEpi& bn = BnEpi(),
               const bf16_t* wT = nullptr, int zero_rest = 1);
void stem_stream_set(int on);
void stem_pool_rows_set(int on);
void gemm_expand_k256_set(int on);
void gemm_expand_s2_set(int on);
bool conv1x1_s2_expand_bn(const bf16_t* x, int Nb, int H, int W, int Cin, const bf16_t* w, bf16_t* y, int Kout,
                          float* part, hipStream_t st);
void conv_fwd_c8(const bf16_t* x, const bf16_t* w, bf16_t* y, int N, int H, int W, int K, int R, int S, int stride,
                 int pad, hipStream_t st, const BnEpi& bn = BnEpi(), int stride_w = 0);
void conv_set_stages(int which, int stages);
int conv_wgrad_split(int N, int H, int W, int C, int K, int R, int S, int stride, int pad, int stride_w = 0,
                     int target_wgs = 0);
void conv_wgrad(const bf16_t* dy, const bf16_t* x, void* dw, int dw_bf16, float beta, float* ws, int split, int N,
                int H, int W, int C, int K, int R, int S, int stride, int pad, hipStream_t st, int stride_w = 0,
                int sched = 0);

}
```

csrc/kernels/batchnorm.hip:

```cpp
#include <stdlib.h>
#include "dtg/common.h"
#include "dtg/kernels.h"
#include "dtg/bn_finalize.cuh"

namespace dtg {

long long bn_workspace_floats(long long M, int C) {
  BnGeom g = bn_geom(M, C);
  return (long long)g.nchunk * 2 * C + 4LL * C;
}

template <int TPR>
__global__ void __launch_bounds__(kBlk) bn_stats_kernel(const bf16_t* __restrict__ x, long long M, int C,
                                                        long long rpc, float* __restrict__ part) {
  constexpr int RPP = kBlk / TPR, CW = TPR * 8;
  __shared__ float sh[2][RPP][CW + 4];
  const int tx = threadIdx.x % TPR, ty = threadIdx.x / TPR;
  const int c0 = blockIdx.y * CW + tx * 8;
  const long long m0 = (long long)blockIdx.x * rpc;
  const long long m1 = m0 + rpc < M ? m0 + rpc : M;
  float s[8] = {0, 0, 0, 0, 0, 0, 0, 0}, q[8] = {0, 0, 0, 0, 0, 0, 0, 0};
  if (c0 < C) {
    long long m = m0 + ty;
    for (; m + RPP < m1; m += 2 * RPP) {
      float a[8], b[8];
      load8_bf16(x + m * C + c0, a);
      load8_bf16(x + (m + RPP) * C + c0, b);
#pragma unroll
      for (int k = 0; k < 8; ++k) { s[k] += a[k] + b[k]; q[k] += a[k] * a[k] + b[k] * b[k]; }
    }
    if (m < m1) {
      float a[8];
      load8_bf16(x + m * C + c0, a);
#pragma unroll
      for (int k = 0; k < 8; ++k) { s[k] += a[k]; q[k] += a[k] * a[k]; }
    }
  }
#pragma unroll
  for (int k = 0; k < 8; ++k) { sh[0][ty][tx * 8 + k] = s[k]; sh[1][ty][tx * 8 + k] = q[k]; }
  __syncthreads();
  for (int c = threadIdx.x; c < CW; c += kBlk) {
    float ts = 0.f, tq = 0.f;
#pragma unroll 4
    for (int r = 0; r < RPP; ++r) { ts += sh[0][r][c]; tq += sh[1][r][c]; }
    const int cc = blockIdx.y * CW + c;
    if (cc < C) {
      part[((long long)blockIdx.x * 2 + 0) * C + cc] = ts;
      part[((long long)blockIdx.x * 2 + 1) * C + cc] = tq;
    }
  }
}

__device__ __forceinline__ uint8_t pos_bits8(const float (&v)[8]) {
  uint32_t b = 0;
#pragma unroll
  for (int k = 0; k < 8; ++k) b |= (v[k] > 0.f ? 1u : 0u) << k;
  return (uint8_t)b;
}

__device__ __forceinline__ void store_bits(uint8_t* bits, long long off, const float (&v)[8], int tx, int C) {
  const uint32_t b = pos_bits8(v);
  if ((C & 31) == 0) {
    uint32_t w = b << (8 * (tx & 3));
    w |= __shfl_xor(w, 1, 64);
    w |= __shfl_xor(w, 2, 64);
    if ((tx & 3) == 0) *reinterpret_cast<uint32_t*>(bits + (off >> 3)) = w;
  } else {
    bits[off >> 3] = (uint8_t)b;
  }
}

template <int TPR, bool RES, bool RELU, int RU = 4>
__global__ void __launch_bounds__(kBlk) bn_apply_kernel(const bf16_t* __restrict__ x, const bf16_t* __restrict__ res,
                                                        bf16_t* __restrict__ y, const float* __restrict__ coef,
                                                        long long M, int C, long long rpc,
                                                        uint8_t* __restrict__ bits = nullptr) {
  constexpr int RPP = kBlk / TPR, CW = TPR * 8;
  const int tx = threadIdx.x % TPR, ty = threadIdx.x / TPR;
  const int c0 = blockIdx.y * CW + tx * 8;
  if (c0 >= C) return;
  float sc[8], sf[8];
  load8_f32(coef + c0, sc);
  load8_f32(coef + C + c0, sf);
  const long long m0 = (long long)blockIdx.x * rpc;
  const long long m1 = m0 + rpc < M ? m0 + rpc : M;
  auto finish = [&](float (&a)[8], const float (&r)[8], long long off) {
#pragma unroll
    for (int k = 0; k < 8; ++k) {
      float v = a[k] * sc[k] + sf[k];
      if constexpr (RES) v += r[k];
      if constexpr (RELU) v = fmaxf(v, 0.f);
      a[k] = v;
    }
    store8_bf16(y + off, a);
    if (bits) store_bits(bits, off, a, tx, C);
  };
  long long m = m0 + ty;
  for (; m + (RU - 1) * RPP < m1; m += RU * RPP) {
    float a[RU][8], r[RU][8];
#pragma unroll
    for (int u = 0; u < RU; ++u) {
      load8_bf16(x + (m + u * RPP) * C + c0, a[u]);
      if constexpr (RES) load8_bf16(res + (m + u * RPP) * C + c0, r[u]);
    }
#pragma unroll
    for (int u = 0; u < RU; ++u) finish(a[u], r[u], (m + u * RPP) * C + c0);
  }
  for (; m < m1; m += RPP) {
    const long long o0 = m * C + c0;
    float a0[8], r0[8];
    load8_bf16(x + o0, a0);
    if constexpr (RES) load8_bf16(res + o0, r0);
    finish(a0, r0, o0);
  }
}

template <int TPR, int RU = 4>
__global__ void __launch_bounds__(kBlk) bn_apply2_kernel(const bf16_t* __restrict__ x, const bf16_t* __restrict__ r,
                                                         bf16_t* __restrict__ y, const float* __restrict__ coef,
                                                         const float* __restrict__ coef2, long long M, int C,
                                                         long long rpc, uint8_t* __restrict__ bits) {
  constexpr int RPP = kBlk / TPR, CW = TPR * 8;
  const int tx = threadIdx.x % TPR, ty = threadIdx.x / TPR;
  const int c0 = blockIdx.y * CW + tx * 8;
  if (c0 >= C) return;
  float sc[8], sf[8], sc2[8], sf2[8];
  load8_f32(coef + c0, sc);
  load8_f32(coef + C + c0, sf);
  load8_f32(coef2 + c0, sc2);
  load8_f32(coef2 + C + c0, sf2);
#pragma unroll
  for (int k = 0; k < 8; ++k) sf[k] += sf2[k];
  const long long m0 = (long long)blockIdx.x * rpc;
  const long long m1 = m0 + rpc < M ? m0 + rpc : M;
  auto finish = [&](float (&a)[8], const float (&b)[8], long long o) {
#pragma unroll
    for (int k = 0; k < 8; ++k) a[k] = fmaxf(fmaf(a[k], sc[k], fmaf(b[k], sc2[k], sf[k])), 0.f);
    store8_bf16(y + o, a);
    if (bits) store_bits(bits, o, a, tx, C);
  };
  long long m = m0 + ty;
  for (; m + (RU - 1) * RPP < m1; m += RU * RPP) {
    float a[RU][8], b[RU][8];
#pragma unroll
    for (int u = 0; u < RU; ++u) {
      load8_bf16(x + (m + u * RPP) * C + c0, a[u]);
      load8_bf16(r + (m + u * RPP) * C + c0, b[u]);
    }
#pragma unroll
    for (int u = 0; u < RU; ++u) finish(a[u], b[u], (m + u * RPP) * C + c0);
  }
  for (; m < m1; m += RPP) {
    const long long o0 = m * C + c0;
    float a0[8], b0[8];
    load8_bf16(x + o0, a0);
    load8_bf16(r + o0, b0);
    finish(a0, b0, o0);
  }
}

template <int TPR, bool RELU>
__global__ void __launch_bounds__(kBlk) bn_bwd_reduce_kernel(const bf16_t* __restrict__ dy,
                                                             const bf16_t* __restrict__ y,
                                                             const bf16_t* __restrict__ x,
                                                             const float* __restrict__ smean,
                                                             const float* __restrict__ sinv, long long M, int C,
                                                             long long rpc, float* __restrict__ part) {
  constexpr int RPP = kBlk / TPR, CW = TPR * 8;
  __shared__ float sh[2][RPP][CW + 4];
  const int tx = threadIdx.x % TPR, ty = threadIdx.x / TPR;
  const int c0 = blockIdx.y * CW + tx * 8;
  float s[8] = {0, 0, 0, 0, 0, 0, 0, 0}, q[8] = {0, 0, 0, 0, 0, 0, 0, 0};
  if (c0 < C) {
    float mu[8], is[8];
    load8_f32(smean + c0, mu);
    load8_f32(sinv + c0, is);
    const long long m0 = (long long)blockIdx.x * rpc;
    const long long m1 = m0 + rpc < M ? m0 + rpc : M;
    auto acc = [&](float (&g)[8], const float (&xv)[8], const float (&yv)[8]) {
      if constexpr (RELU) {
#pragma unroll
        for (int k = 0; k < 8; ++k) g[k] = yv[k] > 0.f ? g[k] : 0.f;
      }
#pragma unroll
      for (int k = 0; k < 8; ++k) { s[k] += g[k]; q[k] += g[k] * (xv[k] - mu[k]) * is[k]; }
    };
    long long m = m0 + ty;
    for (; m + RPP < m1; m += 2 * RPP) {
      const long long o0 = m * C + c0, o1 = (m + RPP) * C + c0;
      float g0[8], g1[8], x0[8], x1[8], y0[8], y1[8];
      load8_bf16(dy + o0, g0);
      load8_bf16(dy + o1, g1);
      load8_bf16(x + o0, x0);
      load8_bf16(x + o1, x1);
      if constexpr (RELU) {
        load8_bf16(y + o0, y0);
        load8_bf16(y + o1, y1);
      }
      acc(g0, x0, y0);
      acc(g1, x1, y1);
    }
    if (m < m1) {
      const long long o0 = m * C + c0;
      float g0[8], x0[8], y0[8];
      load8_bf16(dy + o0, g0);
      load8_bf16(x + o0, x0);
      if constexpr (RELU) load8_bf16(y + o0, y0);
      acc(g0, x0, y0);
    }
  }
#pragma unroll
  for (int k = 0; k < 8; ++k) { sh[0][ty][tx * 8 + k] = s[k]; sh[1][ty][tx * 8 + k] = q[k]; }
  __syncthreads();
  for (int c = threadIdx.x; c < CW; c += kBlk) {
    float ts = 0.f, tq = 0.f;
#pragma unroll 4
    for (int r = 0; r < RPP; ++r) { ts += sh[0][r][c]; tq += sh[1][r][c]; }
    const int cc = blockIdx.y * CW + c;
    if (cc < C) {
      part[((long long)blockIdx.x * 2 + 0) * C + cc] = ts;
      part[((long long)blockIdx.x * 2 + 1) * C + cc] = tq;
    }
  }
}

template <int TPR, bool RELU, bool DRES, bool NT = true, int RU = 4>
__global__ void __launch_bounds__(kBlk) bn_bwd_dx_kernel(const bf16_t* __restrict__ dy, const bf16_t* __restrict__ y,
                                                         const bf16_t* __restrict__ x, const float* __restrict__ coef,
                                                         bf16_t* __restrict__ dx, bf16_t* __restrict__ dres,
                                                         long long M, int C, long long rpc) {
  constexpr int RPP = kBlk / TPR, CW = TPR * 8;
  const int tx = threadIdx.x % TPR, ty = threadIdx.x / TPR;
  const int c0 = blockIdx.y * CW + tx * 8;
  if (c0 >= C) return;
  float a[8], bx[8], cc[8];
  load8_f32(coef + c0, a);
  load8_f32(coef + C + c0, bx);
  load8_f32(coef + 2 * C + c0, cc);
  const long long m0 = (long long)blockIdx.x * rpc;
  const long long m1 = m0 + rpc < M ? m0 + rpc : M;
  auto finish = [&](float (&g)[8], const float (&xv)[8], const float (&yv)[8], long long off) {
    if constexpr (RELU) {
#pragma unroll
      for (int k = 0; k < 8; ++k) g[k] = yv[k] > 0.f ? g[k] : 0.f;
    }
    if constexpr (DRES) store8_bf16(dres + off, g);
    float o[8];
#pragma unroll
    for (int k = 0; k < 8; ++k) o[k] = a[k] * g[k] + bx[k] * xv[k] + cc[k];
    store8_bf16(dx + off, o);
  };
  auto ld = [&](const bf16_t* p, float (&v)[8]) {
    if constexpr (NT) load8_bf16_nt(p, v);
    else load8_bf16(p, v);
  };
  long long m = m0 + ty;
  for (; m + (RU - 1) * RPP < m1; m += RU * RPP) {
    float g[RU][8], xv[RU][8], yv[RU][8];
#pragma unroll
    for (int u = 0; u < RU; ++u) {
      const long long o = (m + u * RPP) * C + c0;
      ld(dy + o, g[u]);
      ld(x + o, xv[u]);
      if constexpr (RELU) load8_bf16(y + o, yv[u]);
    }
#pragma unroll
    for (int u = 0; u < RU; ++u) finish(g[u], xv[u], yv[u], (m + u * RPP) * C + c0);
  }
  for (; m < m1; m += RPP) {
    const long long o0 = m * C + c0;
    float g0[8], x0[8], y0[8];
    ld(dy + o0, g0);
    ld(x + o0, x0);
    if constexpr (RELU) load8_bf16(y + o0, y0);
    finish(g0, x0, y0, o0);
  }
}

#define DTG_RU_SWITCH(...) \
  { constexpr int RU = 2; __VA_ARGS__; }

static void bn_apply_launch(const BnGeom& g, const bf16_t* x, const bf16_t* res, bf16_t* y, const float* coef,
                            long long M, int C, int relu, hipStream_t st, uint8_t* bits = nullptr) {
  const long long rpa = elementwise_rpc(g, M);
  dim3 ga((unsigned)((M + rpa - 1) / rpa), g.gy);
  DTG_TPR_SWITCH(g.tpr, DTG_RU_SWITCH({
    if (res) {
      if (relu) { bn_apply_kernel<T, true, true, RU><<<ga, kBlk, 0, st>>>(x, res, y, coef, M, C, rpa, bits); DTG_LAUNCH_CHECK(); }
      else { bn_apply_kernel<T, true, false, RU><<<ga, kBlk, 0, st>>>(x, res, y, coef, M, C, rpa, bits); DTG_LAUNCH_CHECK(); }
    } else {
      if (relu) { bn_apply_kernel<T, false, true, RU><<<ga, kBlk, 0, st>>>(x, res, y, coef, M, C, rpa, bits); DTG_LAUNCH_CHECK(); }
      else { bn_apply_kernel<T, false, false, RU><<<ga, kBlk, 0, st>>>(x, res, y, coef, M, C, rpa, bits); DTG_LAUNCH_CHECK(); }
    }
  }));
}

void bn_fwd_train(const bf16_t* x, const bf16_t* res, bf16_t* y, const float* gamma, const float* beta,
                  float* rmean, float* rvar, float* smean, float* sinv, float* ws, long long M, int C,
                  float momentum, float eps, int relu, hipStream_t st) {
  const BnGeom g = bn_geom(M, C);
  float* part = ws;
  float* coef = ws + (long long)g.nchunk * 2 * C;
  dim3 grid(g.nchunk, g.gy);
  DTG_TPR_SWITCH(g.tpr, bn_stats_kernel<T><<<grid, kBlk, 0, st>>>(x, M, C, g.rows_per_chunk, part)); DTG_LAUNCH_CHECK();
  bn_finalize_kernel<16><<<(C + 63) / 64, 1024, 0, st>>>(part, g.nchunk, M, C, 0, gamma, beta, rmean, rvar, smean, sinv,
                                                    momentum, eps, coef, nullptr, nullptr); DTG_LAUNCH_CHECK();
  bn_apply_launch(g, x, res, y, coef, M, C, relu, st);
}

void bn_fwd_from_part(const bf16_t* x, const bf16_t* res, bf16_t* y, const float* gamma, const float* beta,
                      float* rmean, float* rvar, float* smean, float* sinv, const float* part, float* ws, long long M,
                      int C, float momentum, float eps, int relu, hipStream_t st, uint8_t* bits) {
  const BnGeom g = bn_geom(M, C);
  bn_finalize_kernel<16><<<(C + 63) / 64, 1024, 0, st>>>(part, kBnStatSlots, M, C, 0, gamma, beta, rmean, rvar, smean,
                                                    sinv, momentum, eps, ws, nullptr, nullptr, 1); DTG_LAUNCH_CHECK();
  bn_apply_launch(g, x, res, y, ws, M, C, relu, st, bits);
}

__global__ void bn_infer_coef_kernel(const float* gamma, const float* beta, const float* rmean, const float* rvar,
                                     float eps, int C, float* coef) {
  const int c = blockIdx.x * blockDim.x + threadIdx.x;
  if (c >= C) return;
  const float inv = rsqrtf(rvar[c] + eps);
  const float sc = (gamma ? gamma[c] : 1.f) * inv;
  coef[c] = sc;
  coef[C + c] = (beta ? beta[c] : 0.f) - rmean[c] * sc;
}

void bn_fwd_infer(const bf16_t* x, const bf16_t* res, bf16_t* y, const float* gamma, const float* beta,
                  const float* rmean, const float* rvar, float* ws, long long M, int C, float eps, int relu,
                  hipStream_t st) {
  const BnGeom g = bn_geom(M, C);
  float* coef = ws;
  bn_infer_coef_kernel<<<(C + 255) / 256, 256, 0, st>>>(gamma, beta, rmean, rvar, eps, C, coef); DTG_LAUNCH_CHECK();
  dim3 grid(g.nchunk, g.gy);
  const long long rpa = elementwise_rpc(g, M);
  dim3 ga((unsigned)((M + rpa - 1) / rpa), g.gy);
  DTG_TPR_SWITCH(g.tpr, {
    if (res) {
      if (relu) { bn_apply_kernel<T, true, true><<<ga, kBlk, 0, st>>>(x, res, y, coef, M, C, rpa); DTG_LAUNCH_CHECK(); }
      else { bn_apply_kernel<T, true, false><<<ga, kBlk, 0, st>>>(x, res, y, coef, M, C, rpa); DTG_LAUNCH_CHECK(); }
    } else {
      if (relu) { bn_apply_kernel<T, false, true><<<ga, kBlk, 0, st>>>(x, res, y, coef, M, C, rpa); DTG_LAUNCH_CHECK(); }
      else { bn_apply_kernel<T, false, false><<<ga, kBlk, 0, st>>>(x, res, y, coef, M, C, rpa); DTG_LAUNCH_CHECK(); }
    }
  });
}

void bn_bwd(const bf16_t* dy, const bf16_t* y, const bf16_t* x, const float* gamma, const float* smean,
            const float* sinv, bf16_t* dx, bf16_t* dres, float* dgamma, float* dbeta, float* ws, long long M, int C,
            int relu, int accum, hipStream_t st) {
  const BnGeom g = bn_geom(M, C);
  float* part = ws;
  float* coef = ws + (long long)g.nchunk * 2 * C;
  dim3 grid(g.nchunk, g.gy);
  DTG_TPR_SWITCH(g.tpr, {
    if (relu) { bn_bwd_reduce_kernel<T, true><<<grid, kBlk, 0, st>>>(dy, y, x, smean, sinv, M, C, g.rows_per_chunk, part); DTG_LAUNCH_CHECK(); }
    else { bn_bwd_reduce_kernel<T, false><<<grid, kBlk, 0, st>>>(dy, y, x, smean, sinv, M, C, g.rows_per_chunk, part); DTG_LAUNCH_CHECK(); }
  });
  bn_finalize_kernel<16><<<(C + 63) / 64, 1024, 0, st>>>(part, g.nchunk, M, C, accum ? 2 : 1, gamma, nullptr, nullptr, nullptr,
                                                    const_cast<float*>(smean), const_cast<float*>(sinv), 0.f, 0.f,
                                                    coef, dgamma, dbeta); DTG_LAUNCH_CHECK();
  const long long rpa = elementwise_rpc(g, M);
  dim3 ga((unsigned)((M + rpa - 1) / rpa), g.gy);
  DTG_TPR_SWITCH(g.tpr, {
    if (relu) {
      if (dres) { bn_bwd_dx_kernel<T, true, true><<<ga, kBlk, 0, st>>>(dy, y, x, coef, dx, dres, M, C, rpa); DTG_LAUNCH_CHECK(); }
      else { bn_bwd_dx_kernel<T, true, false><<<ga, kBlk, 0, st>>>(dy, y, x, coef, dx, dres, M, C, rpa); DTG_LAUNCH_CHECK(); }
    } else {
      if (dres) { bn_bwd_dx_kernel<T, false, true><<<ga, kBlk, 0, st>>>(dy, y, x, coef, dx, dres, M, C, rpa); DTG_LAUNCH_CHECK(); }
      else { bn_bwd_dx_kernel<T, false, false><<<ga, kBlk, 0, st>>>(dy, y, x, coef, dx, dres, M, C, rpa); DTG_LAUNCH_CHECK(); }
    }
  });
}

void bn_fwd2_from_part(const bf16_t* x, const bf16_t* r, bf16_t* y, const float* part, const float* part2,
                       const float* gamma, const float* beta, float* rmean, float* rvar, float* smean, float* sinv,
                       const float* gamma2, const float* beta2, float* rmean2, float* rvar2, float* smean2,
                       float* sinv2, float* ws, long long M, int C, float momentum, float eps, hipStream_t st,
                       uint8_t* bits) {
  const BnGeom g = bn_geom(M, C);
  bn_finalize_kernel<16><<<(C + 63) / 64, 1024, 0, st>>>(part, kBnStatSlots, M, C, 0, gamma, beta, rmean, rvar, smean,
                                                    sinv, momentum, eps, ws, nullptr, nullptr, 1); DTG_LAUNCH_CHECK();
  bn_finalize_kernel<16><<<(C + 63) / 64, 1024, 0, st>>>(part2, kBnStatSlots, M, C, 0, gamma2, beta2, rmean2, rvar2,
                                                    smean2, sinv2, momentum, eps, ws + 2LL * C, nullptr, nullptr, 1); DTG_LAUNCH_CHECK();
  const long long rpa = elementwise_rpc(g, M);
  dim3 ga((unsigned)((M + rpa - 1) / rpa), g.gy);
  DTG_TPR_SWITCH(g.tpr, DTG_RU_SWITCH(bn_apply2_kernel<T, RU><<<ga, kBlk, 0, st>>>(x, r, y, ws, ws + 2LL * C, M, C, rpa,
                                                                                 bits))); DTG_LAUNCH_CHECK();
}

template <int TPR, int RU = 4>
__global__ void __launch_bounds__(kBlk) bn_bwd_dx2_kernel(const bf16_t* __restrict__ dp, const bf16_t* __restrict__ x,
                                                          const bf16_t* __restrict__ x2,
                                                          const float* __restrict__ coef,
                                                          const float* __restrict__ coef2, bf16_t* __restrict__ dx,
                                                          bf16_t* __restrict__ dx2, long long M, int C, long long rpc) {
  constexpr int RPP = kBlk / TPR, CW = TPR * 8;
  const int tx = threadIdx.x % TPR, ty = threadIdx.x / TPR;
  const int c0 = blockIdx.y * CW + tx * 8;
  if (c0 >= C) return;
  float a[8], bx[8], cc[8], a2[8], bx2[8], cc2[8];
  load8_f32(coef + c0, a);
  load8_f32(coef + C + c0, bx);
  load8_f32(coef + 2 * C + c0, cc);
  load8_f32(coef2 + c0, a2);
  load8_f32(coef2 + C + c0, bx2);
  load8_f32(coef2 + 2 * C + c0, cc2);
  const long long m0 = (long long)blockIdx.x * rpc;
  const long long m1 = m0 + rpc < M ? m0 + rpc : M;
  auto finish = [&](const float (&g)[8], const float (&xv)[8], const float (&x2v)[8], long long o) {
    float o1[8], o2[8];
#pragma unroll
    for (int k = 0; k < 8; ++k) {
      o1[k] = fmaf(a[k], g[k], fmaf(bx[k], xv[k], cc[k]));
      o2[k] = fmaf(a2[k], g[k], fmaf(bx2[k], x2v[k], cc2[k]));
    }
    store8_bf16(dx + o, o1);
    store8_bf16(dx2 + o, o2);
  };
  long long m = m0 + ty;
  for (; m + (RU - 1) * RPP < m1; m += RU * RPP) {
    float g[RU][8], xv[RU][8], x2v[RU][8];
#pragma unroll
    for (int u = 0; u < RU; ++u) {
      const long long o = (m + u * RPP) * C + c0;
      load8_bf16(dp + o, g[u]);
      load8_bf16(x + o, xv[u]);
      load8_bf16(x2 + o, x2v[u]);
    }
#pragma unroll
    for (int u = 0; u < RU; ++u) finish(g[u], xv[u], x2v[u], (m + u * RPP) * C + c0);
  }
  for (; m < m1; m += RPP) {
    const long long o = m * C + c0;
    float g[8], xv[8], x2v[8];
    load8_bf16(dp + o, g);
    load8_bf16(x + o, xv);
    load8_bf16(x2 + o, x2v);
    finish(g, xv, x2v, o);
  }
}

void bn_bwd2_from_part(const bf16_t* dp, const bf16_t* x, const bf16_t* x2, const float* part, const float* part2,
                       const float* gamma, const float* smean, const float* sinv, const float* gamma2,
                       const float* smean2, const float* sinv2, bf16_t* dx, bf16_t* dx2, float* dgamma, float* dbeta,
                       float* dgamma2, float* dbeta2, float* ws, long long M, int C, int accum, hipStream_t st) {
  const BnGeom g = bn_geom(M, C);
  bn_finalize_kernel<16><<<(C + 63) / 64, 1024, 0, st>>>(part, kBnStatSlots, M, C, accum ? 2 : 1, gamma, nullptr, nullptr,
                                                    nullptr, const_cast<float*>(smean), const_cast<float*>(sinv), 0.f,
                                                    0.f, ws, dgamma, dbeta, 1); DTG_LAUNCH_CHECK();
  bn_finalize_kernel<16><<<(C + 63) / 64, 1024, 0, st>>>(part2, kBnStatSlots, M, C, accum ? 2 : 1, gamma2, nullptr,
                                                    nullptr, nullptr, const_cast<float*>(smean2),
                                                    const_cast<float*>(sinv2), 0.f, 0.f, ws + 3LL * C, dgamma2,
                                                    dbeta2, 1); DTG_LAUNCH_CHECK();
  const long long rpa = elementwise_rpc(g, M);
  dim3 ga((unsigned)((M + rpa - 1) / rpa), g.gy);
  DTG_TPR_SWITCH(g.tpr, DTG_RU_SWITCH(bn_bwd_dx2_kernel<T, RU><<<ga, kBlk, 0, st>>>(dp, x, x2, ws, ws + 3LL * C, dx,
                                                                                   dx2, M, C, rpa))); DTG_LAUNCH_CHECK();
}

void bn_bwd_coef_from_part(const float* part, const float* gamma, const float* smean, const float* sinv, float* coef,
                           float* dgamma, float* dbeta, long long M, int C, int accum, hipStream_t st) {
  bn_finalize_kernel<16><<<(C + 63) / 64, 1024, 0, st>>>(part, kBnStatSlots, M, C, accum ? 2 : 1, gamma, nullptr, nullptr,
                                                    nullptr, const_cast<float*>(smean), const_cast<float*>(sinv), 0.f,
                                                    0.f, coef, dgamma, dbeta, 1); DTG_LAUNCH_CHECK();
}

void bn_dx_from_coef(const bf16_t* dp, const bf16_t* x, const float* coef, bf16_t* dx, bf16_t* dres, long long M, int C,
                     hipStream_t st) {
  const BnGeom g = bn_geom(M, C);
  const long long rpa = elementwise_rpc(g, M);
  dim3 ga((unsigned)((M + rpa - 1) / rpa), g.gy);
  const float* ws = coef;
  DTG_TPR_SWITCH(g.tpr, DTG_RU_SWITCH({
    if (dres) { bn_bwd_dx_kernel<T, false, true, true, RU><<<ga, kBlk, 0, st>>>(dp, nullptr, x, ws, dx, dres, M, C,
                                                                                      rpa); DTG_LAUNCH_CHECK(); }
    else { bn_bwd_dx_kernel<T, false, false, true, RU><<<ga, kBlk, 0, st>>>(dp, nullptr, x, ws, dx, dres, M, C, rpa); DTG_LAUNCH_CHECK(); }
  }));
}

void bn_bwd_from_part(const bf16_t* dp, const bf16_t* x, const float* gamma, const float* smean, const float* sinv,
                      const float* part, bf16_t* dx, bf16_t* dres, float* dgamma, float* dbeta, float* ws, long long M,
                      int C, int accum, hipStream_t st) {
  bn_bwd_coef_from_part(part, gamma, smean, sinv, ws, dgamma, dbeta, M, C, accum, st);
  bn_dx_from_coef(dp, x, ws, dx, dres, M, C, st);
}

}
```

csrc/kernels/bn_dx_wgrad.hip:

```cpp
#include "dtg/common.h"
#include "dtg/kernels.h"
#include "dtg/mfma_gemm.cuh"
#include "dtg/gemm_epi.cuh"

namespace dtg {

namespace {
using namespace gemm;

constexpr int kDC = 256;
constexpr int kDR = 32;
constexpr int kDX_LDS = kDR * kDC * 2;

template <int CI, bool DUAL, bool W2 = false>
__global__ void __launch_bounds__(256, (CI == 64 && !W2) ? 2 : 1) bn_dx_wgrad_kernel(const bf16_t* __restrict__ dp, const bf16_t* __restrict__ x,
                                                          const float* __restrict__ coef,
                                                          const bf16_t* __restrict__ x2,
                                                          const float* __restrict__ coef2, bf16_t* __restrict__ dx,
                                                          bf16_t* __restrict__ dx2, const bf16_t* __restrict__ act,
                                                          long long ldact, float* __restrict__ slabs, int nblk,
                                                          int C, const bf16_t* __restrict__ act2, long long ldact2,
                                                          float* __restrict__ slabs2) {
  static_assert(!W2 || (DUAL && CI == 64), "the second weight gradient is the dual form's, at 256 x 64");
  constexpr int kACT_LDS = kDR * CI * 2;
  constexpr int NJ = CI / 16;
  constexpr int NX = W2 ? 2 : 1;
  __shared__ __attribute__((aligned(16))) char smem_raw[NX * (kDX_LDS + 2 * kACT_LDS)];
  lds_char* sdx = (lds_char*)smem_raw;
  lds_char* sact = sdx + kDX_LDS;
  lds_char* sdx2 = sact + 2 * kACT_LDS;
  lds_char* sact2 = sdx2 + kDX_LDS;
  const int tid = threadIdx.x, lane = tid & 63;
  const int wave = __builtin_amdgcn_readfirstlane(tid >> 6);
  const int G = gridDim.x;
  const int ns = C / kDC, gid = xcd_remap(blockIdx.x, G);
  const int sl = gid % ns;
  const int c8 = tid & 31, rs = tid >> 5, c0 = sl * kDC + c8 * 8;
  float a[8], bx[8], cc[8], a2[8], bx2[8], cc2[8];
  load8_f32(coef + c0, a);
  load8_f32(coef + C + c0, bx);
  load8_f32(coef + 2 * C + c0, cc);
  if constexpr (DUAL) {
    load8_f32(coef2 + c0, a2);
    load8_f32(coef2 + C + c0, bx2);
    load8_f32(coef2 + 2 * C + c0, cc2);
  }
  DenseMC<false> sa{act, ldact, CI, 0};
  DenseMC<false> sa2{act2, ldact2, CI, 0};
  f32x4 acc[4][NJ], acc2[W2 ? 4 : 1][W2 ? NJ : 1];
#pragma unroll
  for (int i = 0; i < 4; ++i)
#pragma unroll
    for (int j = 0; j < NJ; ++j) acc[i][j] = f32x4{0.f, 0.f, 0.f, 0.f};
  if constexpr (W2) {
#pragma unroll
    for (int i = 0; i < 4; ++i)
#pragma unroll
      for (int j = 0; j < NJ; ++j) acc2[i][j] = f32x4{0.f, 0.f, 0.f, 0.f};
  }

  auto unpack = [](const u32x4v& v, float (&f)[8]) {
    f[0] = __uint_as_float(v.x << 16); f[1] = __uint_as_float(v.x & 0xffff0000u);
    f[2] = __uint_as_float(v.y << 16); f[3] = __uint_as_float(v.y & 0xffff0000u);
    f[4] = __uint_as_float(v.z << 16); f[5] = __uint_as_float(v.z & 0xffff0000u);
    f[6] = __uint_as_float(v.w << 16); f[7] = __uint_as_float(v.w & 0xffff0000u);
  };
  u32x4v g[4], xv[4], x2v[4];
  auto issue = [&](int b, int slot) {
    const long long m0 = (long long)b * kDR;
    stage_mc<CI, DenseMC<false>, 4, kDR>(sa, sact + slot * kACT_LDS, 0, (int)m0, wave, lane);
    if constexpr (W2) stage_mc<CI, DenseMC<false>, 4, kDR>(sa2, sact2 + slot * kACT_LDS, 0, (int)m0, wave, lane);
#pragma unroll
    for (int u = 0; u < 4; ++u) {
      const long long off = (m0 + rs + 8 * u) * C + c0;
      g[u] = *reinterpret_cast<const u32x4v*>(dp + off);
      xv[u] = *reinterpret_cast<const u32x4v*>(x + off);
      if constexpr (DUAL) x2v[u] = *reinterpret_cast<const u32x4v*>(x2 + off);
    }
  };
  const int b0 = gid / ns, gb = G / ns;
  if (b0 < nblk) issue(b0, 0);
  int slot = 0;
  for (int b = b0; b < nblk; b += gb, slot ^= 1) {
    const long long m0 = (long long)b * kDR;
#pragma unroll
    for (int u = 0; u < 4; ++u) {
      const int m = rs + 8 * u;
      const long long off = (m0 + m) * C + c0;
      float gf[8], xf[8], o[8];
      unpack(g[u], gf);
      unpack(xv[u], xf);
#pragma unroll
      for (int k = 0; k < 8; ++k) o[k] = fmaf(a[k], gf[k], fmaf(bx[k], xf[k], cc[k]));
      u32x4v w;
      w.x = pack_bf2(o[0], o[1]);
      w.y = pack_bf2(o[2], o[3]);
      w.z = pack_bf2(o[4], o[5]);
      w.w = pack_bf2(o[6], o[7]);
      *reinterpret_cast<u32x4v*>(dx + off) = w;
      *reinterpret_cast<__attribute__((address_space(3))) u32x4v*>(sdx + m * (kDC * 2) +
                                                                   ((c8 ^ mc_swz<kDC / 8>(m)) << 4)) = w;
      if constexpr (DUAL) {
        float x2f[8], o2[8];
        unpack(x2v[u], x2f);
#pragma unroll
        for (int k = 0; k < 8; ++k) o2[k] = fmaf(a2[k], gf[k], fmaf(bx2[k], x2f[k], cc2[k]));
        u32x4v w2;
        w2.x = pack_bf2(o2[0], o2[1]);
        w2.y = pack_bf2(o2[2], o2[3]);
        w2.z = pack_bf2(o2[4], o2[5]);
        w2.w = pack_bf2(o2[6], o2[7]);
        *reinterpret_cast<u32x4v*>(dx2 + off) = w2;
        if constexpr (W2)
          *reinterpret_cast<__attribute__((address_space(3))) u32x4v*>(sdx2 + m * (kDC * 2) +
                                                                       ((c8 ^ mc_swz<kDC / 8>(m)) << 4)) = w2;
      }
    }
    const bool more = b + gb < nblk;
    if (more) issue(b + gb, slot ^ 1);
    constexpr int PIECES = (CI / 64) * (W2 ? 2 : 1);
    if (more) asm volatile("s_waitcnt vmcnt(%0) lgkmcnt(0)" ::"n"(DUAL ? 8 + PIECES + 12 : 4 + PIECES + 8) : "memory");
    else asm volatile("s_waitcnt vmcnt(%0) lgkmcnt(0)" ::"n"(DUAL ? 8 : 4) : "memory");
    __builtin_amdgcn_s_barrier();
    v8bf fa[4], fb[NJ];
#pragma unroll
    for (int i = 0; i < 4; ++i) fa[i] = frag_mc<kDC>(sdx, wave * 64 + i * 16, 0, lane);
#pragma unroll
    for (int j = 0; j < NJ; ++j) fb[j] = frag_mc<CI>(sact + slot * kACT_LDS, j * 16, 0, lane);
#pragma unroll
    for (int i = 0; i < 4; ++i)
#pragma unroll
      for (int j = 0; j < NJ; ++j)
        acc[i][j] = __builtin_amdgcn_mfma_f32_16x16x32_bf16(fa[i], fb[j], acc[i][j], 0, 0, 0);
    if constexpr (W2) {
#pragma unroll
      for (int i = 0; i < 4; ++i) fa[i] = frag_mc<kDC>(sdx2, wave * 64 + i * 16, 0, lane);
#pragma unroll
      for (int j = 0; j < NJ; ++j) fb[j] = frag_mc<CI>(sact2 + slot * kACT_LDS, j * 16, 0, lane);
#pragma unroll
      for (int i = 0; i < 4; ++i)
#pragma unroll
        for (int j = 0; j < NJ; ++j)
          acc2[i][j] = __builtin_amdgcn_mfma_f32_16x16x32_bf16(fa[i], fb[j], acc2[i][j], 0, 0, 0);
    }
    asm volatile("s_waitcnt lgkmcnt(0)" ::: "memory");
    __builtin_amdgcn_s_barrier();
  }
  asm volatile("s_waitcnt vmcnt(0)" ::: "memory");
  float* slab = slabs + ((long long)(gid / ns) * C + sl * kDC) * CI;
  const int q = lane & 15, gq = lane >> 4;
#pragma unroll
  for (int i = 0; i < 4; ++i)
#pragma unroll
    for (int j = 0; j < NJ; ++j)
#pragma unroll
      for (int r = 0; r < 4; ++r) slab[(wave * 64 + i * 16 + gq * 4 + r) * CI + j * 16 + q] = acc[i][j][r];
  if constexpr (W2) {
    float* slab2 = slabs2 + ((long long)(gid / ns) * C + sl * kDC) * CI;
#pragma unroll
    for (int i = 0; i < 4; ++i)
#pragma unroll
      for (int j = 0; j < NJ; ++j)
#pragma unroll
        for (int r = 0; r < 4; ++r) slab2[(wave * 64 + i * 16 + gq * 4 + r) * CI + j * 16 + q] = acc2[i][j][r];
  }
}

template <int CI, bool W2 = false>
int dx_wgrad_grid() {
  static int G = 0;
  if (G == 0) {
    int dev = 0, cus = 0, per_cu = 0;
    DTG_HIP_CHECK(hipGetDevice(&dev));
    DTG_HIP_CHECK(hipDeviceGetAttribute(&cus, hipDeviceAttributeMultiprocessorCount, dev));
    DTG_HIP_CHECK(hipOccupancyMaxActiveBlocksPerMultiprocessor(&per_cu, bn_dx_wgrad_kernel<CI, true, W2>, 256, 0));
    G = cus * (per_cu < 1 ? 1 : (per_cu > 2 ? 2 : per_cu));
    G -= G % 8;
    if (G < 8) G = 8;
  }
  return G;
}

}

bool bn_dx_wgrad_ok(long long M, int C, int CI) {
  return ((C == 256 && CI == 64) || (C == 512 && CI == 128)) && M % kDR == 0 && M >= 64LL * kDR;
}

int bn_dx_wgrad_slabs(int C, int CI, int w2) {
  return (w2 ? dx_wgrad_grid<64, true>() : CI == 64 ? dx_wgrad_grid<64>() : dx_wgrad_grid<128>()) / (C / kDC);
}

void bn_dx_wgrad(const bf16_t* dp, const bf16_t* x, const float* coef, const bf16_t* x2, const float* coef2,
                 bf16_t* dx, bf16_t* dx2, const bf16_t* act, long long ldact, void* wgrad, int wgrad_bf16,
                 float* slabs, long long M, int C, int CI, hipStream_t st, const bf16_t* act2, long long ldact2,
                 void* wgrad2, float* slabs2) {
  const int nblk = (int)(M / kDR);
  auto launch = [&](auto kern, int G) {
    hipLaunchKernelGGL(kern, dim3(G), dim3(256), 0, st, dp, x, coef, x2, coef2, dx, dx2, act, ldact, slabs, nblk, C,
                       act2, ldact2, slabs2);
    DTG_LAUNCH_CHECK();
    return G;
  };
  int G;
  if (act2) {
    G = launch(bn_dx_wgrad_kernel<64, true, true>, dx_wgrad_grid<64, true>());
    Epi e2{wgrad2, CI, wgrad_bf16, 1.f, 1.f, nullptr, 0};
    gemm_splitk_reduce(slabs2, G / (C / kDC), C, CI, e2, st);
  } else if (CI == 64) G = x2 ? launch(bn_dx_wgrad_kernel<64, true>, dx_wgrad_grid<64>())
                              : launch(bn_dx_wgrad_kernel<64, false>, dx_wgrad_grid<64>());
  else G = x2 ? launch(bn_dx_wgrad_kernel<128, true>, dx_wgrad_grid<128>())
              : launch(bn_dx_wgrad_kernel<128, false>, dx_wgrad_grid<128>());
  Epi e{wgrad, CI, wgrad_bf16, 1.f, 1.f, nullptr, 0};
  gemm_splitk_reduce(slabs, G / (C / kDC), C, CI, e, st);
}

}
```

csrc/kernels/gemm.hip:

```cpp
#include "dtg/common.h"
#include "dtg/kernels.h"
#include "dtg/gemm_launch.cuh"
#include <stdlib.h>
#include <type_traits>

namespace dtg {
using namespace gemm;


__global__ void __launch_bounds__(256) splitk_reduce_kernel(const float* __restrict__ ws, int split_k, int M, int N,
                                                            Epi e) {
  const int cgs = (N + 7) / 8;
  const long long total = (long long)M * cgs;
  const long long plane = (long long)M * N;
  const bool vec = (N & 7) == 0;
  for (long long i = (long long)blockIdx.x * blockDim.x + threadIdx.x; i < total;
       i += (long long)gridDim.x * blockDim.x) {
    const int m = (int)(i / cgs), n = (int)(i % cgs) * 8;
    const long long off = (long long)m * N + n;
    float s[8] = {0, 0, 0, 0, 0, 0, 0, 0};
    if (vec) {
      int k = 0;
      for (; k + 4 <= split_k; k += 4) {
        float v0[8], v1[8], v2[8], v3[8];
        load8_f32(ws + (k + 0) * plane + off, v0);
        load8_f32(ws + (k + 1) * plane + off, v1);
        load8_f32(ws + (k + 2) * plane + off, v2);
        load8_f32(ws + (k + 3) * plane + off, v3);
#pragma unroll
        for (int j = 0; j < 8; ++j) s[j] += (v0[j] + v1[j]) + (v2[j] + v3[j]);
      }
      for (; k < split_k; ++k) {
        float v[8];
        load8_f32(ws + k * plane + off, v);
#pragma unroll
        for (int j = 0; j < 8; ++j) s[j] += v[j];
      }
    } else {
      for (int k = 0; k < split_k; ++k)
        for (int j = 0; j < 8 && n + j < N; ++j) s[j] += ws[k * plane + off + j];
    }
    epi_store8(e, N, m, n, s);
  }
}

__global__ void __launch_bounds__(256) splitk_reduce_par_kernel(const float* __restrict__ ws, int split_k, int M,
                                                                int N, Epi e) {
  __shared__ float red[8][256 + 8];
  const long long plane = (long long)M * N;
  const long long base = (long long)blockIdx.x * 256;
  const int lane = threadIdx.x & 31, grp = threadIdx.x >> 5;
  float s[8] = {0, 0, 0, 0, 0, 0, 0, 0};
  if (base + lane * 8 < plane) {
    for (int k = grp; k < split_k; k += 8) {
      float v[8];
      load8_f32(ws + k * plane + base + lane * 8, v);
#pragma unroll
      for (int j = 0; j < 8; ++j) s[j] += v[j];
    }
  }
#pragma unroll
  for (int j = 0; j < 8; ++j) red[grp][lane * 8 + j] = s[j];
  __syncthreads();
  if (grp == 0 && base + lane * 8 < plane) {
#pragma unroll
    for (int g = 1; g < 8; ++g)
#pragma unroll
      for (int j = 0; j < 8; ++j) s[j] += red[g][lane * 8 + j];
    const long long i = base + lane * 8;
    epi_store8(e, N, (int)(i / N), (int)(i % N), s);
  }
}

long long gemm_workspace_floats(int M, int N, int K, int split_k) {
  return split_k > 1 ? (long long)split_k * M * N : 0;
}

static bool skinny(int N) { return N <= 64; }

static bool short_m(int M, int N) { return M <= 64 && N >= 128; }

int gemm_pick_split(int M, int N, int K, int a_kc, int target_wgs) {
  const int BMv = skinny(N) ? 256 : (short_m(M, N) ? 64 : 128), BNv = skinny(N) ? 64 : (short_m(M, N) ? 256 : 128);
  const long long tiles = (long long)((M + BMv - 1) / BMv) * ((N + BNv - 1) / BNv);
  if (a_kc && tiles >= 128) {
    int s = 1;
    if (K >= 8192)
      while (tiles * s < 384 && (long long)K / (s * 2) >= 4096) s *= 2;
    return s;
  }
  int s = 1;
  const long long target = target_wgs > 0 ? target_wgs : 512;
  while (tiles * s < target && (long long)K / (s * 2) >= 1024 && s < 256) s *= 2;
  return s;
}

template <int BM_, int BN_>
static void launch_cfg(int a_kc, int b_kc, const bf16_t* A, long long lda, const bf16_t* B, long long ldb, int M,
                       int N, int K, int split_k, int kps, const Epi& e, float* ws, hipStream_t st,
                       const GemmBatch& bt) {
  const bool full = (M % BM_ == 0) && (N % BN_ == 0) && (K % BK == 0);
  const bool short_k = kps <= 2 * BK;
  if (full) {
    if (short_k) launch_layout<Cfg<BM_, BN_, 1>, false>(a_kc, b_kc, A, lda, B, ldb, M, N, K, split_k, kps, e, ws, st, bt);
    else launch_layout<Cfg<BM_, BN_, 2>, false>(a_kc, b_kc, A, lda, B, ldb, M, N, K, split_k, kps, e, ws, st, bt);
  } else {
    if (short_k) launch_layout<Cfg<BM_, BN_, 1>, true>(a_kc, b_kc, A, lda, B, ldb, M, N, K, split_k, kps, e, ws, st, bt);
    else launch_layout<Cfg<BM_, BN_, 2>, true>(a_kc, b_kc, A, lda, B, ldb, M, N, K, split_k, kps, e, ws, st, bt);
  }
}


static bool use_rp(int M, int N, int kps) {
  if ((long long)((M + 127) / 128) * ((N + 127) / 128) > 2048) return false;
  if (kps >= 2048) return true;
  const double flop = 2.0 * M * N * kps, bytes = 2.0 * ((double)M * kps + (double)N * kps + (double)M * N);
  return kps >= 768 && flop / bytes >= 300.0;
}

void gemm_splitk_reduce(const float* ws, int split_k, int M, int N, const Epi& e, hipStream_t st) {
  if (N % 8 == 0 && split_k > 16) {
    const long long plane = (long long)M * N;
    splitk_reduce_par_kernel<<<(unsigned)((plane + 255) / 256), 256, 0, st>>>(ws, split_k, M, N, e); DTG_LAUNCH_CHECK();
  } else {
    const long long total = (long long)M * ((N + 7) / 8);
    splitk_reduce_kernel<<<grid_for(total, 256, 1 << 16), 256, 0, st>>>(ws, split_k, M, N, e); DTG_LAUNCH_CHECK();
  }
}

void gemm_bf16(const bf16_t* A, long long lda, int a_kc, const bf16_t* B, long long ldb, int b_kc, void* C,
               long long ldc, int c_bf16, int M, int N, int K, float alpha, float beta, const float* bias, int act,
               int split_k, float* ws, hipStream_t st, const GemmBatch& bt, void* aux, int aux_mode) {
  if (M <= 0 || N <= 0) return;
  if (bt.count > 1) split_k = 1;
  if (split_k < 1) split_k = 1;
  int kps = (K + split_k - 1) / split_k;
  kps = (kps + BK - 1) / BK * BK;
  if (kps < BK) kps = BK;
  split_k = (K + kps - 1) / kps;
  if (split_k < 1) split_k = 1;
  Epi e{C, ldc, c_bf16, alpha, beta, bias, act, aux, aux_mode};
  if (split_k > 1 || !a_kc) {
    launch_exact<Cfg<128, 128, 1, 4, 64, true>>(a_kc, b_kc, A, lda, B, ldb, M, N, K, split_k, kps, e, ws, st, bt);
    return;
  }
  if (short_m(M, N)) {
    launch_cfg<64, 256>(a_kc, b_kc, A, lda, B, ldb, M, N, K, split_k, kps, e, ws, st, bt);
    return;
  }
  const long long tiles128 = (long long)((M + 127) / 128) * ((N + 127) / 128) * split_k * bt.count;
  if (use_rp(M, N, kps)) {
    launch_exact<Cfg<128, 128, 1, 4, 64, true>>(a_kc, b_kc, A, lda, B, ldb, M, N, K, split_k, kps, e, ws, st, bt);
  } else if (tiles128 < 512 && kps >= 2048) {
    launch_exact<Cfg<128, 128, 2>>(a_kc, b_kc, A, lda, B, ldb, M, N, K, split_k, kps, e, ws, st, bt);
  } else if (skinny(N)) {
    launch_exact<Cfg<256, 64, 1>>(a_kc, b_kc, A, lda, B, ldb, M, N, K, split_k, kps, e, ws, st, bt);
  } else if (N >= 256 && M >= 64 && kps <= 256) {
    launch_exact<Cfg<64, 256, 1>>(a_kc, b_kc, A, lda, B, ldb, M, N, K, split_k, kps, e, ws, st, bt);
  } else {
    launch_exact<Cfg<128, 128, 1>>(a_kc, b_kc, A, lda, B, ldb, M, N, K, split_k, kps, e, ws, st, bt);
  }
}

template <class CF, int MODE, bool GUARD, bool PF>
static void launch_bn(const bf16_t* A, long long lda, const bf16_t* B, long long ldb, int M, int N, int K,
                      const Epi& e, const BnEpi& bn, hipStream_t st) {
  using SB = std::conditional_t<MODE == 1, DenseKC<GUARD>, DenseMC<GUARD>>;
  SB sb{B, ldb, N, K};
  const int tiles_m = (M + CF::BM - 1) / CF::BM, tiles_n = (N + CF::BN - 1) / CF::BN;
  using SA = DenseKC<GUARD>;
  SA sa{A, lda, M, K};
  hipLaunchKernelGGL((gemm_kernel<CF, true, MODE == 1, SA, SB, MODE, false, PF>), dim3(tiles_m * tiles_n, 1, 1),
                     dim3(CF::NTH), 0, st, sa, sb, M, N, K, tiles_n, 1, K, e, (float*)nullptr, GemmBatch(), bn); DTG_LAUNCH_CHECK();
}


template <class CF, int MODE>
static void launch_bn_cfg(const bf16_t* A, long long lda, const bf16_t* B, long long ldb, int M, int N, int K,
                          const Epi& e, const BnEpi& bn, hipStream_t st) {
  const bool full = (M % CF::BM == 0) && (N % CF::BN == 0) && (K % BK == 0);
  if constexpr (MODE >= 2 && MODE <= 4) {
    if (N >= 512 || K <= 128) {
      if (full) launch_bn<CF, MODE, false, true>(A, lda, B, ldb, M, N, K, e, bn, st);
      else launch_bn<CF, MODE, true, true>(A, lda, B, ldb, M, N, K, e, bn, st);
      return;
    }
  }
  if (full) launch_bn<CF, MODE, false, false>(A, lda, B, ldb, M, N, K, e, bn, st);
  else launch_bn<CF, MODE, true, false>(A, lda, B, ldb, M, N, K, e, bn, st);
}

static int g_bn_gemm_cfg = 0;
void gemm_bn_force_cfg(int cfg) { g_bn_gemm_cfg = cfg; }

template <int MODE>
static void gemm_bn_dispatch(const bf16_t* A, long long lda, const bf16_t* B, long long ldb, int M, int N, int K,
                             const Epi& e, const BnEpi& bn, hipStream_t st) {
  switch (g_bn_gemm_cfg) {
    case 1: return launch_bn_cfg<Cfg<128, 128, 1>, MODE>(A, lda, B, ldb, M, N, K, e, bn, st);
    case 2: return launch_bn_cfg<Cfg<64, 256, 1>, MODE>(A, lda, B, ldb, M, N, K, e, bn, st);
    case 3: return launch_bn_cfg<Cfg<128, 128, 1, 4, 64, true>, MODE>(A, lda, B, ldb, M, N, K, e, bn, st);
    case 4: return launch_bn_cfg<Cfg<256, 64, 1>, MODE>(A, lda, B, ldb, M, N, K, e, bn, st);
    case 5: return launch_bn_cfg<Cfg<128, 256, 1, 8>, MODE>(A, lda, B, ldb, M, N, K, e, bn, st);
    case 6: return launch_bn_cfg<Cfg<256, 128, 1, 8>, MODE>(A, lda, B, ldb, M, N, K, e, bn, st);
    default: break;
  }
  if (MODE == 1 && K <= 128 && N >= 256 && M >= 128) {
    launch_bn_cfg<Cfg<128, 128, 1>, MODE>(A, lda, B, ldb, M, N, K, e, bn, st);
    return;
  }
  if (MODE >= 2 && MODE <= 4 && K >= 256 && N >= 128) {
    launch_bn_cfg<Cfg<128, 128, 1, 4, 64, true>, MODE>(A, lda, B, ldb, M, N, K, e, bn, st);
    return;
  }
  if (use_rp(M, N, K)) launch_bn_cfg<Cfg<128, 128, 1, 4, 64, true>, MODE>(A, lda, B, ldb, M, N, K, e, bn, st);
  else if ((long long)((M + 127) / 128) * ((N + 127) / 128) < 512 && K >= 2048)
    launch_bn_cfg<Cfg<128, 128, 2>, MODE>(A, lda, B, ldb, M, N, K, e, bn, st);
  else if (skinny(N)) launch_bn_cfg<Cfg<256, 64, 1>, MODE>(A, lda, B, ldb, M, N, K, e, bn, st);
  else if (N >= 256 && M >= 64 && K <= 256) launch_bn_cfg<Cfg<64, 256, 1>, MODE>(A, lda, B, ldb, M, N, K, e, bn, st);
  else launch_bn_cfg<Cfg<128, 128, 1>, MODE>(A, lda, B, ldb, M, N, K, e, bn, st);
}

bool gemm_expand_bn(const bf16_t* A, long long lda, const bf16_t* W, long long ldw, bf16_t* C, long long ldc, int M,
                    int N, int K, float* part, hipStream_t st, int variant);

void gemm_bf16_bn(const bf16_t* A, long long lda, const bf16_t* B, long long ldb, bf16_t* C, long long ldc, int M,
                  int N, int K, float beta, const BnEpi& bn, hipStream_t st) {
  if (M <= 0 || N <= 0) return;
  Epi e{C, ldc, 1, 1.f, bn.mode == 3 ? beta : 0.f, nullptr, 0};
  if (bn.mode == 1) {
    if ((g_bn_gemm_cfg == 0 || g_bn_gemm_cfg <= -2) &&
        gemm_expand_bn(A, lda, B, ldb, C, ldc, M, N, K, bn.part, st, g_bn_gemm_cfg == 0 ? 0 : -1 - g_bn_gemm_cfg))
      return;
    gemm_bn_dispatch<1>(A, lda, B, ldb, M, N, K, e, bn, st);
  }
  else if (bn.mode == 2) gemm_bn_dispatch<2>(A, lda, B, ldb, M, N, K, e, bn, st);
  else if (bn.x2) gemm_bn_dispatch<4>(A, lda, B, ldb, M, N, K, e, bn, st);
  else gemm_bn_dispatch<3>(A, lda, B, ldb, M, N, K, e, bn, st);
}

void gemm_bf16_colsum(const bf16_t* A, long long lda, const bf16_t* B, long long ldb, bf16_t* C, long long ldc, int M,
                      int N, int K, const float* bias, int act, void* aux, int aux_mode, float* colsum, hipStream_t st) {
  if (M <= 0 || N <= 0) return;
  Epi e{C, ldc, 1, 1.f, 0.f, bias, act, aux, aux_mode};
  BnEpi bn;
  bn.part = colsum;
  bn.mode = 5;
  gemm_bn_dispatch<5>(A, lda, B, ldb, M, N, K, e, bn, st);
}

}
```

csrc/kernels/gemm_expand.hip:

```cpp
#include "dtg/common.h"
#include "dtg/kernels.h"
#include "dtg/mfma_gemm.cuh"

namespace dtg {

namespace {
using namespace gemm;

constexpr int kXR = 64;
constexpr int kXS = 3;

struct ExpandGather {
  int H, W;
  FastDiv fPQ, fQ;
};

template <int K, bool NT, int MINB, bool S2 = false>
__global__ void __launch_bounds__(256, MINB > 0 ? MINB : 1) gemm_expand_bn_kernel(const bf16_t* __restrict__ A, long long lda,
                                                             const bf16_t* __restrict__ W, long long ldw,
                                                             bf16_t* __restrict__ C, long long ldc,
                                                             float* __restrict__ part, int N, int nslice, int tiles,
                                                             ExpandGather gth) {
  constexpr int KS = K / 32;
  constexpr int KH = K / 64;
  constexpr int BLK = kXR * K * 2;
  constexpr int D = KH * 2;
  constexpr int T = 8;
  __shared__ __attribute__((aligned(16))) char smem_raw[kXS * BLK];
  lds_char* smem = (lds_char*)smem_raw;
  const int tid = threadIdx.x, lane = tid & 63;
  const int wave = __builtin_amdgcn_readfirstlane(tid >> 6);
  const int G = gridDim.x;
  const int base = xcd_remap(blockIdx.x, G);
  const int my = base < tiles ? (tiles - base + G - 1) / G : 0;
  if (my == 0) return;
  const int slice = base % nslice;
  const int col0 = slice * 256 + wave * 64;
  const int q = lane & 15, g = lane >> 4;

  v8bf wf[4][KS];
#pragma unroll
  for (int j = 0; j < 4; ++j)
#pragma unroll
    for (int ks = 0; ks < KS; ++ks) {
      const int n = col0 + 32 * (j >> 1) + 8 * (q >> 2) + 4 * (j & 1) + (q & 3);
      wf[j][ks] = *reinterpret_cast<const v8bf*>(W + (long long)n * ldw + ks * 32 + 8 * g);
    }

  const int rb0 = base / nslice, gs = G / nslice;
  auto stage = [&](int it) {
    const int rb = rb0 + (it < my ? it : my - 1) * gs;
    lds_char* dst = smem + (it % kXS) * BLK;
#pragma unroll
    for (int i = 0; i < 2; ++i) {
      const int r0 = (wave * 2 + i) * 8, r = r0 + (lane >> 3);
      const int c = (lane & 7) ^ (r & 7);
      long long arow = (long long)rb * kXR + r;
      if constexpr (S2) {
        uint32_t n, pq, pp, qq;
        gth.fPQ.divmod((uint32_t)arow, n, pq);
        gth.fQ.divmod(pq, pp, qq);
        arow = ((long long)n * gth.H + 2 * (int)pp) * gth.W + 2 * (int)qq;
      }
      const char* src = (const char*)(A + arow * lda + c * 8);
#pragma unroll
      for (int h = 0; h < KH; ++h)
        __builtin_amdgcn_global_load_lds((const void*)(src + h * 128), (lds_void*)(dst + h * kXR * 128 + r0 * 128), 16,
                                         0, 0);
    }
  };

  float s[16], sq[16];
#pragma unroll
  for (int c = 0; c < 16; ++c) s[c] = sq[c] = 0.f;
  const f32x4 zero4 = {0.f, 0.f, 0.f, 0.f};

  stage(0);
  stage(1);
  for (int it = 0; it < my; ++it) {
    if (it == 0) asm volatile("s_waitcnt vmcnt(%0)" ::"n"(D) : "memory");
    else if (it == 1) asm volatile("s_waitcnt vmcnt(%0)" ::"n"(D + T) : "memory");
    else asm volatile("s_waitcnt vmcnt(%0)" ::"n"(2 * T + D) : "memory");
    __builtin_amdgcn_s_barrier();
    stage(it + 2);
    const lds_char* ta = smem + (it % kXS) * BLK;
    const long long row0 = (long long)(rb0 + it * gs) * kXR;
#pragma unroll
    for (int i = 0; i < 4; ++i) {
      v8bf af[KS];
#pragma unroll
      for (int ks = 0; ks < KS; ++ks) af[ks] = frag_kc(ta + (ks >> 1) * kXR * 128, 16 * i, ks & 1, lane);
      f32x4 acc[4];
#pragma unroll
      for (int j = 0; j < 4; ++j) acc[j] = __builtin_amdgcn_mfma_f32_16x16x32_bf16(wf[j][0], af[0], zero4, 0, 0, 0);
#pragma unroll
      for (int ks = 1; ks < KS; ++ks)
#pragma unroll
        for (int j = 0; j < 4; ++j)
          acc[j] = __builtin_amdgcn_mfma_f32_16x16x32_bf16(wf[j][ks], af[ks], acc[j], 0, 0, 0);
      u32x4v w0, w1;
      w0.x = pack_bf2(acc[0][0], acc[0][1]);
      w0.y = pack_bf2(acc[0][2], acc[0][3]);
      w0.z = pack_bf2(acc[1][0], acc[1][1]);
      w0.w = pack_bf2(acc[1][2], acc[1][3]);
      w1.x = pack_bf2(acc[2][0], acc[2][1]);
      w1.y = pack_bf2(acc[2][2], acc[2][3]);
      w1.z = pack_bf2(acc[3][0], acc[3][1]);
      w1.w = pack_bf2(acc[3][2], acc[3][3]);
      const uint32_t wd[8] = {w0.x, w0.y, w0.z, w0.w, w1.x, w1.y, w1.z, w1.w};
#pragma unroll
      for (int c = 0; c < 8; ++c) {
        const float lo = __uint_as_float(wd[c] << 16), hi = __uint_as_float(wd[c] & 0xffff0000u);
        s[2 * c] += lo;
        s[2 * c + 1] += hi;
        sq[2 * c] = fmaf(lo, lo, sq[2 * c]);
        sq[2 * c + 1] = fmaf(hi, hi, sq[2 * c + 1]);
      }
      bf16_t* dst = C + (row0 + 16 * i + q) * ldc + col0 + 8 * g;
      if constexpr (NT) {
        __builtin_nontemporal_store(w0, reinterpret_cast<u32x4v*>(dst));
        __builtin_nontemporal_store(w1, reinterpret_cast<u32x4v*>(dst + 32));
      } else {
        *reinterpret_cast<u32x4v*>(dst) = w0;
        *reinterpret_cast<u32x4v*>(dst + 32) = w1;
      }
    }
  }
  asm volatile("s_waitcnt vmcnt(0)" ::: "memory");

#pragma unroll
  for (int c = 0; c < 16; ++c) {
#pragma unroll
    for (int o = 1; o < 16; o <<= 1) {
      s[c] += __shfl_xor(s[c], o, 64);
      sq[c] += __shfl_xor(sq[c], o, 64);
    }
  }
  if (q == 0) {
    float* p = part + (long long)(blockIdx.x % kBnStatSlots) * 2 * N + col0 + 8 * g;
#pragma unroll
    for (int c = 0; c < 16; ++c) {
      const int off = c < 8 ? c : 24 + c;
      atomicAdd(p + off, s[c]);
      atomicAdd(p + N + off, sq[c]);
    }
  }
}

template <int K, bool NT, int MINB, bool S2 = false>
int expand_grid(int nslice) {
  static int per_cu = -1, cus = 0;
  if (per_cu < 0) {
    int dev = 0;
    DTG_HIP_CHECK(hipGetDevice(&dev));
    DTG_HIP_CHECK(hipDeviceGetAttribute(&cus, hipDeviceAttributeMultiprocessorCount, dev));
    DTG_HIP_CHECK(hipOccupancyMaxActiveBlocksPerMultiprocessor(&per_cu, gemm_expand_bn_kernel<K, NT, MINB, S2>, 256, 0));
    if (per_cu < 1) per_cu = 1;
  }
  int G = cus * per_cu;
  const int mult = nslice > 8 ? nslice : 8;
  G -= G % mult;
  return G > 0 ? G : mult;
}

struct StemStreamGeom {
  int Hp, Wp2, P, Q;
  FastDiv fPQ, fQ;
};

__global__ void __launch_bounds__(256, 2) stem_stream_bn_kernel(const bf16_t* __restrict__ x8,
                                                                 const bf16_t* __restrict__ W,
                                                                 bf16_t* __restrict__ C, float* __restrict__ part,
                                                                 StemStreamGeom sg, int nblocks) {
  constexpr int K = 256, KS = K / 32, KH = K / 64, N = 64;
  constexpr int BLK = kXR * K * 2;
  constexpr int D = KH * 2;
  constexpr int T = 2;
  constexpr int TAPS = 28;
  constexpr int RING = 2;
  __shared__ __attribute__((aligned(16))) char smem_raw[RING * BLK];
  lds_char* smem = (lds_char*)smem_raw;
  const int tid = threadIdx.x, lane = tid & 63;
  const int wave = __builtin_amdgcn_readfirstlane(tid >> 6);
  const int G = gridDim.x;
  const int base = xcd_remap(blockIdx.x, G);
  const int my = base < nblocks ? (nblocks - base + G - 1) / G : 0;
  if (my == 0) return;
  const int q = lane & 15, g = lane >> 4;

  v8bf wf[4][KS];
#pragma unroll
  for (int j = 0; j < 4; ++j)
#pragma unroll
    for (int ks = 0; ks < KS; ++ks) {
      const int n = 32 * (j >> 1) + 8 * (q >> 2) + 4 * (j & 1) + (q & 3);
      wf[j][ks] = *reinterpret_cast<const v8bf*>(W + (long long)n * K + ks * 32 + 8 * g);
    }

  auto stage = [&](int it) {
    const int rb = base + (it < my ? it : my - 1) * G;
    lds_char* dst = smem + (it % RING) * BLK;
#pragma unroll
    for (int i = 0; i < 2; ++i) {
      const int r0 = (wave * 2 + i) * 8, r = r0 + (lane >> 3);
      uint32_t n, pq, p, qq;
      sg.fPQ.divmod((uint32_t)(rb * kXR + r), n, pq);
      sg.fQ.divmod(pq, p, qq);
      const bf16_t* rowp = x8 + (((long long)n * sg.Hp + 2 * (int)p) * sg.Wp2 + (int)qq) * 8;
#pragma unroll
      for (int h = 0; h < KH; ++h) {
        const int t = 8 * h + ((lane & 7) ^ (r & 7));
        const void* src = sel(t < TAPS, rowp + ((t >> 2) * sg.Wp2 + (t & 3)) * 8);
        __builtin_amdgcn_global_load_lds(src, (lds_void*)(dst + h * kXR * 128 + r0 * 128), 16, 0, 0);
      }
    }
  };

  float s[16], sq[16];
#pragma unroll
  for (int c = 0; c < 16; ++c) s[c] = sq[c] = 0.f;
  const f32x4 zero4 = {0.f, 0.f, 0.f, 0.f};

  stage(0);
  for (int it = 0; it < my; ++it) {
    if (it == 0) asm volatile("s_waitcnt vmcnt(0)" ::: "memory");
    else asm volatile("s_waitcnt vmcnt(%0)" ::"n"(T) : "memory");
    __builtin_amdgcn_s_barrier();
    __builtin_amdgcn_sched_barrier(0);
    stage(it + RING - 1);
    const lds_char* ta = smem + (it % RING) * BLK;
    const long long row0 = (long long)(base + it * G) * kXR;
    v8bf af[KS];
#pragma unroll
    for (int ks = 0; ks < KS; ++ks) af[ks] = frag_kc(ta + (ks >> 1) * kXR * 128, 16 * wave, ks & 1, lane);
    f32x4 acc[4];
#pragma unroll
    for (int j = 0; j < 4; ++j) acc[j] = __builtin_amdgcn_mfma_f32_16x16x32_bf16(wf[j][0], af[0], zero4, 0, 0, 0);
#pragma unroll
    for (int ks = 1; ks < KS; ++ks)
#pragma unroll
      for (int j = 0; j < 4; ++j) acc[j] = __builtin_amdgcn_mfma_f32_16x16x32_bf16(wf[j][ks], af[ks], acc[j], 0, 0, 0);
    u32x4v w0, w1;
    w0.x = pack_bf2(acc[0][0], acc[0][1]);
    w0.y = pack_bf2(acc[0][2], acc[0][3]);
    w0.z = pack_bf2(acc[1][0], acc[1][1]);
    w0.w = pack_bf2(acc[1][2], acc[1][3]);
    w1.x = pack_bf2(acc[2][0], acc[2][1]);
    w1.y = pack_bf2(acc[2][2], acc[2][3]);
    w1.z = pack_bf2(acc[3][0], acc[3][1]);
    w1.w = pack_bf2(acc[3][2], acc[3][3]);
    const uint32_t wd[8] = {w0.x, w0.y, w0.z, w0.w, w1.x, w1.y, w1.z, w1.w};
#pragma unroll
    for (int c = 0; c < 8; ++c) {
      const float lo = __uint_as_float(wd[c] << 16), hi = __uint_as_float(wd[c] & 0xffff0000u);
      s[2 * c] += lo;
      s[2 * c + 1] += hi;
      sq[2 * c] = fmaf(lo, lo, sq[2 * c]);
      sq[2 * c + 1] = fmaf(hi, hi, sq[2 * c + 1]);
    }
    bf16_t* dst = C + (row0 + 16 * wave + q) * N + 8 * g;
    *reinterpret_cast<u32x4v*>(dst) = w0;
    *reinterpret_cast<u32x4v*>(dst + 32) = w1;
  }
  asm volatile("s_waitcnt vmcnt(0)" ::: "memory");
#pragma unroll
  for (int c = 0; c < 16; ++c) {
#pragma unroll
    for (int o = 1; o < 16; o <<= 1) {
      s[c] += __shfl_xor(s[c], o, 64);
      sq[c] += __shfl_xor(sq[c], o, 64);
    }
  }
  if (q == 0) {
    float* pp = part + (long long)(blockIdx.x % kBnStatSlots) * 2 * N + 8 * g;
#pragma unroll
    for (int c = 0; c < 16; ++c) {
      const int off = c < 8 ? c : 24 + c;
      atomicAdd(pp + off, s[c]);
      atomicAdd(pp + N + off, sq[c]);
    }
  }
}

}

static int g_expand_k256 = 1;
void gemm_expand_k256_set(int on) { g_expand_k256 = on; }

bool gemm_expand_bn(const bf16_t* A, long long lda, const bf16_t* W, long long ldw, bf16_t* C, long long ldc, int M,
                    int N, int K, float* part, hipStream_t st, int variant) {
  if ((K != 64 && K != 128 && !(K == 256 && g_expand_k256)) || N % 256 || M % kXR || (lda & 7) || (ldw & 7) ||
      (ldc & 7))
    return false;
  if ((long long)M * N < (1LL << 24)) return false;
  const int nslice = N / 256;
  if (nslice & (nslice - 1)) return false;
  const int tiles = (M / kXR) * nslice;
  auto launch = [&](auto kern, int G) {
    hipLaunchKernelGGL(kern, dim3(G), dim3(256), 0, st, A, lda, W, ldw, C, ldc, part, N, nslice, tiles, ExpandGather());
  };
  if (K == 64) {
    if (variant == 1) launch(gemm_expand_bn_kernel<64, true, 0>, expand_grid<64, true, 0>(nslice));
    else if (variant == 2) launch(gemm_expand_bn_kernel<64, false, 3>, expand_grid<64, false, 3>(nslice));
    else launch(gemm_expand_bn_kernel<64, false, 0>, expand_grid<64, false, 0>(nslice));
  } else if (K == 256) {
    launch(gemm_expand_bn_kernel<256, false, 0>, expand_grid<256, false, 0>(nslice));
  } else {
    if (variant == 1) launch(gemm_expand_bn_kernel<128, true, 0>, expand_grid<128, true, 0>(nslice));
    else if (variant == 2) launch(gemm_expand_bn_kernel<128, false, 2>, expand_grid<128, false, 2>(nslice));
    else launch(gemm_expand_bn_kernel<128, false, 0>, expand_grid<128, false, 0>(nslice));
  }
  DTG_LAUNCH_CHECK();
  return true;
}

static int g_expand_s2 = 1;
void gemm_expand_s2_set(int on) { g_expand_s2 = on; }

bool conv1x1_s2_expand_bn(const bf16_t* x, int Nb, int H, int W, int Cin, const bf16_t* w, bf16_t* y, int Kout,
                          float* part, hipStream_t st) {
  if (!g_expand_s2 || Cin != 256 || Kout % 256 || (H & 1) || (W & 1)) return false;
  const int P = H / 2, Q = W / 2;
  const long long M = (long long)Nb * P * Q;
  if (M % kXR || M >= (1LL << 31) || (long long)Nb * H * W * Cin >= (1LL << 40)) return false;
  if (M * Kout < (1LL << 24)) return false;
  const int nslice = Kout / 256;
  if (nslice & (nslice - 1)) return false;
  ExpandGather gth;
  gth.H = H;
  gth.W = W;
  gth.fPQ = FastDiv((uint32_t)(P * Q));
  gth.fQ = FastDiv((uint32_t)Q);
  const int tiles = (int)(M / kXR) * nslice;
  hipLaunchKernelGGL((gemm_expand_bn_kernel<256, false, 0, true>), dim3(expand_grid<256, false, 0, true>(nslice)),
                     dim3(256), 0, st, x, (long long)Cin, w, (long long)Cin, y, (long long)Kout, part, Kout, nslice, tiles,
                     gth);
  DTG_LAUNCH_CHECK();
  return true;
}

static int g_stem_stream = 1;
void stem_stream_set(int on) { g_stem_stream = on; }

bool stem_conv_stream_bn(const bf16_t* x8, const bf16_t* w8, bf16_t* y, int N, int Hp, int Wp2, int P, int Q,
                         float* part, hipStream_t st) {
  if (!g_stem_stream) return false;
  const long long M = (long long)N * P * Q;
  if (M % kXR || M / kXR > (1LL << 30) || (long long)N * Hp * Wp2 * 8 >= (1LL << 31)) return false;
  if (2 * (P - 1) + 7 > Hp || (Q - 1) + 4 > Wp2) return false;
  StemStreamGeom sg;
  sg.Hp = Hp;
  sg.Wp2 = Wp2;
  sg.P = P;
  sg.Q = Q;
  sg.fPQ = FastDiv((uint32_t)(P * Q));
  sg.fQ = FastDiv((uint32_t)Q);
  static int G = 0;
  if (G == 0) {
    int dev = 0, cus = 0, per_cu = 0;
    DTG_HIP_CHECK(hipGetDevice(&dev));
    DTG_HIP_CHECK(hipDeviceGetAttribute(&cus, hipDeviceAttributeMultiprocessorCount, dev));
    DTG_HIP_CHECK(hipOccupancyMaxActiveBlocksPerMultiprocessor(&per_cu, stem_stream_bn_kernel, 256, 0));
    G = cus * (per_cu < 1 ? 1 : per_cu);
    G -= G % 8;
    if (G < 8) G = 8;
  }
  hipLaunchKernelGGL(stem_stream_bn_kernel, dim3(G), dim3(256), 0, st, x8, w8, y, part, sg, (int)(M / kXR));
  DTG_LAUNCH_CHECK();
  return true;
}

}
```

distributed-tensorflow-guide_amd/models/resnet_fused.py:

```python
import os

import torch
import torch.nn.functional as F

from ..ops import conv as conv_ops
from ..ops._native import lib
from ..ops.gemm import gemm
from ..parallel import grad_sink, overlap


def _rows(t):
    n, c, h, w = t.shape
    if not t.is_contiguous(memory_format=torch.channels_last):
        t = t.contiguous(memory_format=torch.channels_last)
    return t.permute(0, 2, 3, 1).reshape(n * h * w, c)


def _mat(w):
    return w.reshape(w.shape[0], w.shape[1]) if w.is_contiguous() else w.as_strided((w.shape[0], w.shape[1]),
                                                                                     (w.shape[1], 1))


def _krsc(w):
    return w.permute(0, 2, 3, 1)


_FUSE = True
_LINK = True
_SUB2 = True
_DXW = True
_DXW2 = True


class _Bn3Link:
    __slots__ = ("y3", "m3", "i3", "gamma", "beta", "bits", "yd", "md", "idd", "part", "part2", "dp")

    def __init__(self, y3, m3, i3, gamma, beta, bits, yd=None, md=None, idd=None):
        self.y3, self.m3, self.i3, self.gamma, self.beta = y3, m3, i3, gamma, beta
        self.bits = bits
        self.yd, self.md, self.idd = yd, md, idd
        self.part = self.part2 = self.dp = None


def _gacc(p):
    if grad_sink.enabled(p):
        return p.grad, True
    return torch.zeros_like(p, dtype=torch.float32 if p.dim() <= 1 else p.dtype), False


_BITS = True


_WSPLIT_WGS = int(os.environ.get("DTG_RESNET_WSPLIT_WGS", "256"))
_CWSPLIT_WGS = int(os.environ.get("DTG_RESNET_CWSPLIT_WGS", "256"))
_wsplit_cache = {}


def _wgrad(dy, x, out):
    tgt = _WSPLIT_WGS if overlap.enabled() else 0
    key = (dy.shape[1], x.shape[1], dy.shape[0], tgt)
    sk = _wsplit_cache.get(key)
    if sk is None:
        sk = _wsplit_cache[key] = lib().gemm_pick_split(key[0], key[1], key[2], False, tgt) if tgt > 0 else 0
    gemm(dy, False, x, False, out=out, beta=1.0, split_k=sk)


def _conv_wgrad(dy4, x4, dw, st, pad):
    lib().conv_wgrad(dy4, x4, dw, 1.0, st, pad, target_wgs=_CWSPLIT_WGS if overlap.enabled() else 0)


def _relu_bits(y):
    return torch.empty(y.shape[0], y.shape[1] // 8, device=y.device, dtype=torch.uint8) if _BITS else None


class _BottleneckFn(torch.autograd.Function):
    @staticmethod
    def forward(ctx, x, blk, link_in, holder, *params):
        L = lib()
        n, c, h, w = x.shape
        st = blk.c2.conv.stride
        width = blk.c1.conv.weight.shape[0]
        cout = blk.c3.conv.weight.shape[0]
        x2 = _rows(x)
        p_, q_ = (h + 2 - 3) // st + 1, (w + 2 - 3) // st + 1
        b1, b2, b3 = blk.c1.bn, blk.c2.bn, blk.c3.bn
        w1, w2, w3 = blk.c1.conv.weight, blk.c2.conv.weight, blk.c3.conv.weight
        if _FUSE:
            y1, p1 = L.gemm_bn(x2, _mat(w1), 1, pooled=True)
            bits1 = _relu_bits(y1)
            a1, m1, i1 = L.bn_fwd_part(y1, p1, None, b1.weight, b1.bias, b1.running_mean, b1.running_var,
                                       b1.momentum, b1.eps, True, bits=bits1)
            y2, p2 = L.conv_fwd_bn(a1.view(n, h, w, width), _krsc(w2), st, 1, pooled=True)
            y2 = y2.view(-1, width)
            bits2 = _relu_bits(y2)
            a2, m2, i2 = L.bn_fwd_part(y2, p2, None, b2.weight, b2.bias, b2.running_mean, b2.running_var,
                                       b2.momentum, b2.eps, True, bits=bits2)
            y3, p3 = L.gemm_bn(a2, _mat(w3), 1, pooled=True)
            ctx.bits12 = (bits1, bits2)
        else:
            y1 = gemm(x2, True, _mat(w1), True)
            a1, m1, i1 = L.bn_fwd_train(y1, None, b1.weight, b1.bias, b1.running_mean, b1.running_var, b1.momentum,
                                        b1.eps, True)
            y2 = L.conv_fwd(a1.view(n, h, w, width), _krsc(w2), st, 1).view(-1, width)
            a2, m2, i2 = L.bn_fwd_train(y2, None, b2.weight, b2.bias, b2.running_mean, b2.running_var, b2.momentum,
                                        b2.eps, True)
            y3 = gemm(a2, True, _mat(w3), True)
        yd = md = idd = None
        if blk.down is not None:
            bd, wd = blk.down.bn, blk.down.conv.weight
            if _FUSE:
                if st == 1:
                    yd, pd = L.gemm_bn(x2, _mat(wd), 1, pooled=True)
                else:
                    yd, pd = L.conv_fwd_bn(x2.view(n, h, w, c), _krsc(wd), st, 0, pooled=True)
                    yd = yd.view(-1, cout)
                idn = None
            else:
                if st == 1:
                    yd = gemm(x2, True, _mat(wd), True)
                else:
                    yd = L.conv_fwd(x2.view(n, h, w, c), _krsc(wd), st, 0).view(-1, cout)
                idn, md, idd = L.bn_fwd_train(yd, None, bd.weight, bd.bias, bd.running_mean, bd.running_var,
                                              bd.momentum, bd.eps, False)
        else:
            idn = x2
        bits = None
        if _FUSE and _LINK:
            bits = torch.empty(y3.shape[0], cout // 8, device=y3.device, dtype=torch.uint8)
        if _FUSE and blk.down is not None:
            assert bd.momentum == b3.momentum and bd.eps == b3.eps
            out, m3, i3, md, idd = L.bn_fwd2_part(y3, p3, b3.weight, b3.bias, b3.running_mean, b3.running_var, yd, pd,
                                                  bd.weight, bd.bias, bd.running_mean, bd.running_var, b3.momentum,
                                                  b3.eps, bits=bits)
        elif _FUSE:
            out, m3, i3 = L.bn_fwd_part(y3, p3, idn, b3.weight, b3.bias, b3.running_mean, b3.running_var,
                                        b3.momentum, b3.eps, True, bits=bits)
        else:
            out, m3, i3 = L.bn_fwd_train(y3, idn, b3.weight, b3.bias, b3.running_mean, b3.running_var, b3.momentum,
                                         b3.eps, True)
        ctx.blk = blk
        ctx.link_in = link_in if (_FUSE and _LINK) else None
        ctx.link_out = _Bn3Link(y3, m3, i3, b3.weight, b3.bias, bits, yd, md, idd) if (_FUSE and _LINK) else None
        holder.append(ctx.link_out)
        ctx.geom = (n, c, h, w, st, width, cout, p_, q_)
        ctx.save_for_backward(x2, y1, a1, m1, i1, y2, a2, m2, i2, y3, out, m3, i3,
                              *((yd, md, idd) if yd is not None else ()))
        return out.view(n, p_, q_, cout).permute(0, 3, 1, 2)

    @staticmethod
    def backward(ctx, dout):
        L = lib()
        blk = ctx.blk
        n, c, h, w, st, width, cout, p_, q_ = ctx.geom
        sv = ctx.saved_tensors
        x2, y1, a1, m1, i1, y2, a2, m2, i2, y3, out, m3, i3 = sv[:13]
        b1, b2, b3 = blk.c1.bn, blk.c2.bn, blk.c3.bn
        w1, w2, w3 = blk.c1.conv.weight, blk.c2.conv.weight, blk.c3.conv.weight
        params = [w1, b1.weight, b1.bias, w2, b2.weight, b2.bias, w3, b3.weight, b3.bias]
        if blk.down is not None:
            params += [blk.down.conv.weight, blk.down.bn.weight, blk.down.bn.bias]
        accs = [_gacc(p) for p in params]
        g = {id(p): a for p, (a, _) in zip(params, accs)}
        do = _rows(dout)
        lk = ctx.link_out
        dyd = None
        w3_kw = (dict(wact=a2, wgrad=g[id(w3)].view(cout, width))
                 if _DXW and a2 is not None and L.bn_dx_wgrad_ok(y3.shape[0], cout, width) else None)
        w3_done = wd_done = False
        if (lk is not None and lk.part is not None and do.data_ptr() == lk.dp.data_ptr()
                and do.shape == lk.dp.shape):
            if lk.part2 is not None:
                bd = blk.down.bn
                kw = dict(w3_kw or {})
                if _DXW2 and w3_kw is not None and st == 1 and c == width == 64 and cout == 256:
                    kw.update(wact2=x2, wgrad2=g[id(blk.down.conv.weight)].view(cout, c))
                    wd_done = True
                dy3, dyd = L.bn_bwd2_part(do, y3, lk.part, b3.weight, m3, i3, g[id(b3.weight)], g[id(b3.bias)],
                                          sv[13], lk.part2, bd.weight, sv[14], sv[15], g[id(bd.weight)],
                                          g[id(bd.bias)], **kw)
                w3_done = w3_kw is not None
            else:
                dy3 = L.bn_bwd_part(do, y3, lk.part, b3.weight, m3, i3, False, g[id(b3.weight)], g[id(b3.bias)],
                                    **(w3_kw or {}))[0]
                w3_done = w3_kw is not None
            dres = do
        else:
            for pt in ((lk.part, lk.part2) if lk is not None else ()):
                if pt is not None:
                    pt.zero_()
            dy3, dres, _, _ = L.bn_bwd(do, out, y3, b3.weight, m3, i3, True, True, g[id(b3.weight)],
                                       g[id(b3.bias)])
        if lk is not None:
            lk.part = lk.part2 = lk.dp = None
        bits1, bits2 = ctx.bits12 if _FUSE else (None, None)
        ctx.bits12 = None
        if _FUSE and bits2 is not None:
            dp2, q2 = L.gemm_bn(dy3, _mat(w3), 3, y2, m2, i2, b2.weight, b2.bias, mask=bits2, pooled=True)
        elif _FUSE:
            dp2, q2 = L.gemm_bn(dy3, _mat(w3), 2, y2, m2, i2, b2.weight, b2.bias, pooled=True)
        else:
            da2 = gemm(dy3, True, _mat(w3), False)
        if w3_done:
            pass
        else:
            with overlap.wgrad_scope(dy3, a2):
                _wgrad(dy3, a2, g[id(w3)].view(cout, width))
        if _FUSE:
            dy2 = L.bn_bwd_part(dp2, y2, q2, b2.weight, m2, i2, False, g[id(b2.weight)], g[id(b2.bias)])[0]
        else:
            dy2 = L.bn_bwd(da2, a2, y2, b2.weight, m2, i2, True, False, g[id(b2.weight)], g[id(b2.bias)])[0]
        dy2_4 = dy2.view(n, p_, q_, width)
        if _FUSE:
            dp1, q1 = L.conv_dgrad_bn(dy2_4, _krsc(w2).contiguous(), h, w, st, 1, y1, m1, i1, b1.weight, b1.bias,
                                       pooled=True, bits=bits1)
            dp1 = dp1.view(-1, width)
        else:
            da1 = L.conv_dgrad(dy2_4, _krsc(w2).contiguous(), h, w, st, 1).view(-1, width)
        with overlap.wgrad_scope(dy2_4, a1):
            _conv_wgrad(dy2_4, a1.view(n, h, w, width), g[id(w2)].permute(0, 2, 3, 1), st, 1)
        dx_done = False
        sub2_hw = None
        lk_in = ctx.link_in
        ctx.link_in = None
        if lk_in is not None and lk_in.y3.shape != x2.shape:
            lk_in = None
        if _FUSE:
            dy1 = L.bn_bwd_part(dp1, y1, q1, b1.weight, m1, i1, False, g[id(b1.weight)], g[id(b1.bias)])[0]
        else:
            dy1 = L.bn_bwd(da1, a1, y1, b1.weight, m1, i1, True, False, g[id(b1.weight)], g[id(b1.bias)])[0]
        if blk.down is not None:
            yd, md, idd = sv[13:16]
            bd, wd = blk.down.bn, blk.down.conv.weight
            if dyd is None:
                dyd, _, _, _ = L.bn_bwd(dres, None, yd, bd.weight, md, idd, False, False, g[id(bd.weight)],
                                        g[id(bd.bias)])
            if st == 1:
                dx2 = gemm(dyd, True, _mat(wd), False)
                if not wd_done:
                    with overlap.wgrad_scope(dyd, x2):
                        _wgrad(dyd, x2, g[id(wd)].view(cout, c))
            elif lk_in is not None:
                sub2 = st == 2 and _SUB2
                dx2 = L.conv_dgrad(dyd.view(n, p_, q_, cout), _krsc(wd).contiguous(), h, w, st, 0,
                                   zero_rest=not sub2).view(-1, c)
                if sub2:
                    sub2_hw = (h, w)
                with overlap.wgrad_scope(dyd, x2):
                    _conv_wgrad(dyd.view(n, p_, q_, cout), x2.view(n, h, w, c), g[id(wd)].permute(0, 2, 3, 1), st, 0)
            else:
                dx2 = gemm(dy1, True, _mat(w1), False)
                L.conv_dgrad(dyd.view(n, p_, q_, cout), _krsc(wd).contiguous(), h, w, st, 0, out=dx2.view(n, h, w, c),
                             beta=1.0)
                dx_done = True
                with overlap.wgrad_scope(dyd, x2):
                    _conv_wgrad(dyd.view(n, p_, q_, cout), x2.view(n, h, w, c), g[id(wd)].permute(0, 2, 3, 1), st, 0)
        else:
            dx2 = dres
        if not dx_done:
            if lk_in is not None:
                part2 = None
                if lk_in.yd is not None:
                    part2 = L.bn_part_alloc(dp1, c, pooled=True)
                _, part = L.gemm_bn(dy1, _mat(w1), 3, lk_in.y3, lk_in.m3, lk_in.i3, lk_in.gamma, lk_in.beta,
                                    mask=lk_in.bits, out=dx2, pooled=True, x2=lk_in.yd, mean2=lk_in.md,
                                    invstd2=lk_in.idd, part2=part2, sub2_hw=sub2_hw)
                lk_in.part, lk_in.part2, lk_in.dp = part, part2, dx2
            else:
                gemm(dy1, True, _mat(w1), False, out=dx2, beta=1.0)
        with overlap.wgrad_scope(dy1, x2):
            _wgrad(dy1, x2, g[id(w1)].view(width, c))
        if not all(direct for _, direct in accs):
            overlap.sync_current(x2.device)
        grads = []
        for p, (a, direct) in zip(params, accs):
            if direct:
                grad_sink.notify(p)
                grads.append(None)
            else:
                grads.append(a.to(p.dtype))
        return (dx2.view(n, h, w, c).permute(0, 3, 1, 2), None, None, None, *grads)


def fused_ok(blk, x):
    ws = [blk.c1.conv.weight, blk.c2.conv.weight, blk.c3.conv.weight]
    return (blk.training and x.is_cuda and x.dtype == torch.bfloat16 and all(v.dtype == torch.bfloat16 for v in ws)
            and x.shape[1] % 64 == 0 and blk.c1.conv.weight.shape[0] % 64 == 0)


def bottleneck(blk, x):
    params = [blk.c1.conv.weight, blk.c1.bn.weight, blk.c1.bn.bias, blk.c2.conv.weight, blk.c2.bn.weight,
              blk.c2.bn.bias, blk.c3.conv.weight, blk.c3.bn.weight, blk.c3.bn.bias]
    if blk.down is not None:
        params += [blk.down.conv.weight, blk.down.bn.weight, blk.down.bn.bias]
    holder = []
    y = _BottleneckFn.apply(x, blk, getattr(x, "_dtg_bn3", None), holder, *params)
    if holder and holder[0] is not None:
        y._dtg_bn3 = holder[0]
    return y


_STEM = True
_POOL = (3, 2, 1)
_STEM_YAM = True
_STEM_WG_SCHED = 3
_STEM_WG_WGS = 512


class _StemFn(torch.autograd.Function):
    @staticmethod
    def forward(ctx, x, stem, w, gamma, beta):
        L = lib()
        n, c, h, wd = x.shape
        conv, bn = stem.conv, stem.bn
        k, _, r, s = w.shape
        st, pad = conv.stride, conv.padding
        if conv_ops.stem_pairs_ok(x, w, st):
            x8, w8, (rk, sk) = conv_ops.stem_pairs(x, w, st, pad)
            y4, part = L.conv_fwd_c8(x8, w8, rk, sk, st, 0, True, stride_w=1)
            ctx.pairs = True
        else:
            ctx.pairs = False
            x8 = F.pad(x.permute(0, 2, 3, 1), (0, 8 - c)).contiguous()
            w8 = F.pad(w.permute(0, 2, 3, 1), (0, 8 - c)).reshape(k, r * s * 8)
            kp = (r * s * 8 + 63) // 64 * 64
            w8 = F.pad(w8, (0, kp - r * s * 8)).contiguous()
            y4, part = L.conv_fwd_c8(x8, w8, r, s, st, pad, True)
        yam_ok = _STEM_YAM and L.stem_pooled_stats_ok(y4.shape[-1])
        res = L.stem_bn_pool_fwd(y4, part, gamma, beta, bn.running_mean, bn.running_var, bn.momentum, bn.eps,
                                 *_POOL, save_yam=yam_ok)
        out, idx, smean, sinv = res[:4]
        ctx.save_for_backward(x8, y4, idx, smean, sinv, res[4] if yam_ok else None)
        ctx.stem = stem
        ctx.geom = (c, k, r, s, st, pad)
        return out.permute(0, 3, 1, 2)

    @staticmethod
    def backward(ctx, dout):
        L = lib()
        x8, y4, idx, smean, sinv, yam = ctx.saved_tensors
        c, k, r, s, st, pad = ctx.geom
        stem = ctx.stem
        w, gamma, beta = stem.conv.weight, stem.bn.weight, stem.bn.bias
        (dg, dg_direct), (db, db_direct) = _gacc(gamma), _gacc(beta)
        do4 = dout.contiguous(memory_format=torch.channels_last).permute(0, 2, 3, 1)
        dy4 = L.stem_bn_pool_bwd(do4, idx, y4, gamma, beta, smean, sinv, *_POOL, dgamma_acc=dg, dbeta_acc=db,
                                 yam=yam)[0]
        if ctx.pairs:
            dwp = torch.empty(k, r, (s + 1) // 2, 8, device=x8.device, dtype=torch.float32)
            L.conv_wgrad(dy4, x8, dwp, 0.0, st, 0, stride_w=1, sched=_STEM_WG_SCHED,
                         target_wgs=_STEM_WG_WGS)
        else:
            dwp = torch.empty(k, r, s, 8, device=x8.device, dtype=torch.float32)
            L.conv_wgrad(dy4, x8, dwp, 0.0, st, pad)
        grads = []
        if grad_sink.enabled(w):
            L.stem_dw_add(dwp, w.grad, ctx.pairs)
            grad_sink.notify(w)
            grads.append(None)
        else:
            dw = conv_ops.stem_pairs_dw(dwp, c, s) if ctx.pairs else dwp[..., :c].permute(0, 3, 1, 2)
            grads.append(dw.to(w.dtype).contiguous(memory_format=torch.channels_last))
        for p, (a, direct) in ((gamma, (dg, dg_direct)), (beta, (db, db_direct))):
            if direct:
                grad_sink.notify(p)
                grads.append(None)
            else:
                grads.append(a.to(p.dtype))
        return (None, None, *grads)


def stem_ok(stem, x):
    w = stem.conv.weight
    return (_STEM and stem.training and x.is_cuda and x.dtype == torch.bfloat16 and not x.requires_grad
            and w.dtype == torch.bfloat16 and x.shape[1] <= 8 and w.shape[0] % 64 == 0
            and x.is_contiguous(memory_format=torch.channels_last))


def stem_pool(stem, x):
    return _StemFn.apply(x, stem, stem.conv.weight, stem.bn.weight, stem.bn.bias)
```

Before: 16290 images/sec.

## Fold BN2 apply+ReLU into conv3 GEMM prologue and wgrad activation load

For bottleneck blocks with width 64 (by default), the forward pass no longer materializes the BN2+ReLU output a2. It computes per-channel coefficients only and applies them inline in the streaming expand GEMM prologue, which also writes the ReLU mask bits. The backward fused dx+wgrad kernel reapplies the coefficients to y2 when loading the activation, with a fallback that rebuilds a2 on demand. The aim is to remove a full activation write and read per block and to save memory, at the cost of extra per-fragment arithmetic and new kernel template variants.

Result: no change. 16340 images/sec, median of 6 (+0.3%).

```diff
diff --git a/csrc/bindings/ops.cc b/csrc/bindings/ops.cc
--- a/csrc/bindings/ops.cc
+++ b/csrc/bindings/ops.cc
@@ -630,6 +630,8 @@
   return ring[dev].narrow(0, i * kPartCap, (long long)dtg::kBnStatSlots * 2 * C);
 }
 
+uint8_t* bits_ptr(const c10::optional<Tensor>& bits, long long M, int C);
+
 dtg::BnEpi bn_bwd_epi(Tensor& part, const Tensor& x, const Tensor& mean, const Tensor& invstd, const Tensor& gamma,
                       const Tensor& beta, long long M, int C) {
   CHECK_IN(x);
@@ -657,7 +659,8 @@
                                    c10::optional<Tensor> mask, c10::optional<Tensor> out, bool pooled,
                                    c10::optional<Tensor> x2, c10::optional<Tensor> mean2,
                                    c10::optional<Tensor> invstd2, c10::optional<Tensor> part2,
-                                   c10::optional<std::tuple<int64_t, int64_t>> sub2_hw) {
+                                   c10::optional<std::tuple<int64_t, int64_t>> sub2_hw,
+                                   c10::optional<Tensor> a_coef, c10::optional<Tensor> a_bits) {
   CHECK_IN(A);
   CHECK_DT(A, at::kBFloat16);
   CHECK_CUDA(B);
@@ -681,6 +684,23 @@
     bt = 1.f;
   } else {
     o = at::empty({M, N}, A.options());
+  }
+  const bool inl = a_coef.has_value() && a_coef->defined();
+  TORCH_CHECK(inl || !(a_bits.has_value() && a_bits->defined()), "a_bits needs a_coef");
+  if (inl) {
+    TORCH_CHECK(mode == 1, "a_coef is mode 1 only");
+    TORCH_CHECK(dtg::gemm_expand_inline_ok(M, N, K) && A.stride(0) % 8 == 0,
+                "gemm_bn: a_coef given for a shape the streaming expand kernel does not serve (see "
+                "gemm_expand_inline_ok)");
+    CHECK_IN(*a_coef);
+    CHECK_DT(*a_coef, at::kFloat);
+    TORCH_CHECK(a_coef->numel() == 2LL * K, "a_coef must be [2K]");
+    uint8_t* ab = bits_ptr(a_bits, M, K);
+    auto part = bn_part(A, N, pooled);
+    TORCH_CHECK(dtg::gemm_expand_bn(cbfp(A), A.stride(0), cbfp(B), B.stride(0), bfp(o), N, M, N, K,
+                                    part.data_ptr<float>(), cur_stream(), 0, a_coef->data_ptr<float>(), ab),
+                "gemm_bn: the streaming expand kernel refused a shape gemm_expand_inline_ok accepted");
+    return {o, part};
   }
   auto part = bn_part(A, N, pooled);
   dtg::BnEpi bn;
@@ -817,6 +837,41 @@
   return {y, smean, sinv};
 }
 
+std::tuple<Tensor, Tensor, Tensor> bn_fwd_coef_part(Tensor part, int64_t M, Tensor gamma, Tensor beta, Tensor rmean,
+                                                    Tensor rvar, double momentum, double eps) {
+  const int C = (int)gamma.numel();
+  TORCH_CHECK(M > 0 && C > 0, "empty BN");
+  CHECK_IN(part);
+  CHECK_DT(part, at::kFloat);
+  TORCH_CHECK(part.numel() == (long long)dtg::kBnStatSlots * 2 * C, "partials size mismatch");
+  for (const Tensor* t : {&gamma, &beta, &rmean, &rvar}) {
+    CHECK_IN(*t);
+    CHECK_DT(*t, at::kFloat);
+    TORCH_CHECK(t->numel() == C, "per-channel tensor size mismatch");
+  }
+  c10::DeviceGuard dg(part.device());
+  auto fopt = part.options();
+  auto smean = at::empty({C}, fopt), sinv = at::empty({C}, fopt), coef = at::empty({2LL * C}, fopt);
+  dtg::bn_fwd_coef_from_part(part.data_ptr<float>(), gamma.data_ptr<float>(), beta.data_ptr<float>(),
+                             rmean.data_ptr<float>(), rvar.data_ptr<float>(), smean.data_ptr<float>(),
+                             sinv.data_ptr<float>(), coef.data_ptr<float>(), M, C, (float)momentum, (float)eps,
+                             cur_stream());
+  return {coef, smean, sinv};
+}
+
+Tensor bn_apply_coef(Tensor x, Tensor coef, bool relu) {
+  CHECK_IN(x);
+  CHECK_DT(x, at::kBFloat16);
+  TORCH_CHECK(x.dim() == 2 && x.size(1) % 8 == 0, "x must be [M, C], C a multiple of 8");
+  CHECK_IN(coef);
+  CHECK_DT(coef, at::kFloat);
+  TORCH_CHECK(coef.numel() == 2 * x.size(1), "coef must be [2C]");
+  c10::DeviceGuard dg(x.device());
+  auto y = at::empty_like(x);
+  dtg::bn_apply_from_coef(cbfp(x), bfp(y), coef.data_ptr<float>(), x.size(0), (int)x.size(1), relu, cur_stream());
+  return y;
+}
+
 std::tuple<Tensor, Tensor, Tensor, Tensor, Tensor> bn_fwd2_part(Tensor x, Tensor part, Tensor gamma, Tensor beta,
                                                                 Tensor rmean, Tensor rvar, Tensor r, Tensor part2,
                                                                 Tensor gamma2, Tensor beta2, Tensor rmean2,
@@ -854,6 +909,15 @@
   return {y, m1, i1, m2, i2};
 }
 
+static const float* act_coef_ptr(const c10::optional<Tensor>& act_coef, const c10::optional<Tensor>& wact) {
+  if (!act_coef.has_value() || !act_coef->defined()) return nullptr;
+  TORCH_CHECK(wact.has_value() && wact->defined(), "act_coef needs wact: no path that ignores the coefficients");
+  CHECK_IN(*act_coef);
+  CHECK_DT(*act_coef, at::kFloat);
+  TORCH_CHECK(act_coef->numel() == 2 * wact->size(1), "act_coef must be [2 CI]");
+  return act_coef->data_ptr<float>();
+}
+
 static void check_wgrad_fuse(const Tensor& x, const c10::optional<Tensor>& wact, const c10::optional<Tensor>& wgrad) {
   TORCH_CHECK(wact.has_value() && wgrad.has_value() && wact->defined() && wgrad->defined(), "wact needs wgrad");
   CHECK_CUDA(*wact);
@@ -873,7 +937,8 @@
                                         Tensor dgamma, Tensor dbeta, Tensor x2, Tensor part2, Tensor gamma2,
                                         Tensor smean2, Tensor sinv2, Tensor dgamma2, Tensor dbeta2,
                                         c10::optional<Tensor> wact, c10::optional<Tensor> wgrad,
-                                        c10::optional<Tensor> wact2, c10::optional<Tensor> wgrad2) {
+                                        c10::optional<Tensor> wact2, c10::optional<Tensor> wgrad2,
+                                        c10::optional<Tensor> act_coef) {
   for (const Tensor* t : {&dp, &x, &x2}) {
     CHECK_IN(*t);
     CHECK_DT(*t, at::kBFloat16);
@@ -895,6 +960,7 @@
   c10::DeviceGuard dg(x.device());
   auto dx = at::empty_like(x), dx2 = at::empty_like(x);
   auto ws = at::empty({6LL * C}, x.options().dtype(at::kFloat));
+  const float* acf = act_coef_ptr(act_coef, wact);
   if (wact.has_value() && wact->defined()) {
     check_wgrad_fuse(x, wact, wgrad);
     const int CI = (int)wact->size(1);
@@ -904,7 +970,7 @@
       TORCH_CHECK(C == 256 && CI == 64 && wact2->size(1) == CI && wgrad2->scalar_type() == wgrad->scalar_type(),
                   "wact2: 256 x 64 only, wgrad2 of wgrad's dtype");
     }
-    const long long ns = (long long)dtg::bn_dx_wgrad_slabs(C, CI, w2) * C * CI;
+    const long long ns = (long long)dtg::bn_dx_wgrad_slabs(C, CI, w2, acf != nullptr) * C * CI;
     auto slabs = at::empty({w2 ? 2 * ns : ns}, x.options().dtype(at::kFloat));
     float* w = ws.data_ptr<float>();
     dtg::bn_bwd_coef_from_part(part.data_ptr<float>(), gamma.data_ptr<float>(), smean.data_ptr<float>(),
@@ -916,7 +982,7 @@
     dtg::bn_dx_wgrad(cbfp(dp), cbfp(x), w, cbfp(x2), w + 3LL * C, bfp(dx), bfp(dx2), cbfp(*wact), wact->stride(0),
                      wgrad->data_ptr(), wgrad->scalar_type() == at::kBFloat16, slabs.data_ptr<float>(), M, C, CI,
                      cur_stream(), w2 ? cbfp(*wact2) : nullptr, w2 ? wact2->stride(0) : 0,
-                     w2 ? wgrad2->data_ptr() : nullptr, w2 ? slabs.data_ptr<float>() + ns : nullptr);
+                     w2 ? wgrad2->data_ptr() : nullptr, w2 ? slabs.data_ptr<float>() + ns : nullptr, acf);
     return {dx, dx2};
   }
   dtg::bn_bwd2_from_part(cbfp(dp), cbfp(x), cbfp(x2), part.data_ptr<float>(), part2.data_ptr<float>(),
@@ -932,7 +998,8 @@
                                                                        c10::optional<Tensor> dgamma_acc,
                                                                        c10::optional<Tensor> dbeta_acc,
                                                                        c10::optional<Tensor> wact,
-                                                                       c10::optional<Tensor> wgrad) {
+                                                                       c10::optional<Tensor> wgrad,
+                                                                       c10::optional<Tensor> act_coef) {
   CHECK_IN(dp);
   CHECK_IN(x);
   CHECK_DT(dp, at::kBFloat16);
@@ -969,17 +1036,18 @@
     dbeta = at::empty({C}, fopt);
   }
   auto ws = at::empty({3LL * C}, fopt);
+  const float* acf = act_coef_ptr(act_coef, wact);
   if (wact.has_value() && wact->defined()) {
     TORCH_CHECK(!want_dres, "fused dx + wgrad: no dres");
     check_wgrad_fuse(x, wact, wgrad);
     const int CI = (int)wact->size(1);
-    auto slabs = at::empty({(long long)dtg::bn_dx_wgrad_slabs(C, CI) * C * CI}, fopt);
+    auto slabs = at::empty({(long long)dtg::bn_dx_wgrad_slabs(C, CI, 0, acf != nullptr) * C * CI}, fopt);
     dtg::bn_bwd_coef_from_part(part.data_ptr<float>(), gamma.data_ptr<float>(), smean.data_ptr<float>(),
                                sinv.data_ptr<float>(), ws.data_ptr<float>(), dgamma.data_ptr<float>(),
                                dbeta.data_ptr<float>(), M, C, acc, cur_stream());
     dtg::bn_dx_wgrad(cbfp(dp), cbfp(x), ws.data_ptr<float>(), nullptr, nullptr, bfp(dx), nullptr, cbfp(*wact),
                      wact->stride(0), wgrad->data_ptr(), wgrad->scalar_type() == at::kBFloat16, slabs.data_ptr<float>(),
-                     M, C, CI, cur_stream());
+                     M, C, CI, cur_stream(), nullptr, 0, nullptr, nullptr, acf);
     return {dx, dres, dgamma, dbeta};
   }
   dtg::bn_bwd_from_part(cbfp(dp), cbfp(x), gamma.data_ptr<float>(), smean.data_ptr<float>(), sinv.data_ptr<float>(),
@@ -1030,7 +1098,14 @@
         pybind11::arg("out") = pybind11::none(), pybind11::arg("pooled") = false,
         pybind11::arg("x2") = pybind11::none(), pybind11::arg("mean2") = pybind11::none(),
         pybind11::arg("invstd2") = pybind11::none(), pybind11::arg("part2") = pybind11::none(),
-        pybind11::arg("sub2_hw") = pybind11::none());
+        pybind11::arg("sub2_hw") = pybind11::none(), pybind11::arg("a_coef") = pybind11::none(),
+        pybind11::arg("a_bits") = pybind11::none());
+  m.def("gemm_expand_inline_ok",
+        [](int64_t M, int64_t N, int64_t K) { return dtg::gemm_expand_inline_ok(M, (int)N, (int)K); });
+  m.def("bn_fwd_coef_part", &bn_fwd_coef_part, pybind11::arg("part"), pybind11::arg("M"), pybind11::arg("gamma"),
+        pybind11::arg("beta"), pybind11::arg("rmean"), pybind11::arg("rvar"), pybind11::arg("momentum"),
+        pybind11::arg("eps"));
+  m.def("bn_apply_coef", &bn_apply_coef, pybind11::arg("x"), pybind11::arg("coef"), pybind11::arg("relu") = true);
   m.def("bn_part_alloc", [](Tensor like, int64_t C, bool pooled) { return bn_part(like, C, pooled); },
         pybind11::arg("like"), pybind11::arg("C"), pybind11::arg("pooled") = false);
   m.def("bn_bwd2_part", &bn_bwd2_part, pybind11::arg("dp"), pybind11::arg("x"), pybind11::arg("part"),
@@ -1038,7 +1113,8 @@
         pybind11::arg("dbeta"), pybind11::arg("x2"), pybind11::arg("part2"), pybind11::arg("gamma2"),
         pybind11::arg("smean2"), pybind11::arg("sinv2"), pybind11::arg("dgamma2"), pybind11::arg("dbeta2"),
         pybind11::arg("wact") = pybind11::none(), pybind11::arg("wgrad") = pybind11::none(),
-        pybind11::arg("wact2") = pybind11::none(), pybind11::arg("wgrad2") = pybind11::none());
+        pybind11::arg("wact2") = pybind11::none(), pybind11::arg("wgrad2") = pybind11::none(),
+        pybind11::arg("act_coef") = pybind11::none());
   m.def("bn_dx_wgrad_ok", [](int64_t M, int64_t C, int64_t CI) { return dtg::bn_dx_wgrad_ok(M, (int)C, (int)CI); });
   m.def("conv_fwd_bn", &conv_fwd_bn, pybind11::arg("x"), pybind11::arg("w"), pybind11::arg("stride"),
         pybind11::arg("pad"), pybind11::arg("pooled") = false);
@@ -1059,7 +1135,8 @@
   m.def("bn_bwd_part", &bn_bwd_part, pybind11::arg("dp"), pybind11::arg("x"), pybind11::arg("part"),
         pybind11::arg("gamma"), pybind11::arg("smean"), pybind11::arg("sinv"), pybind11::arg("want_dres"),
         pybind11::arg("dgamma_acc") = pybind11::none(), pybind11::arg("dbeta_acc") = pybind11::none(),
-        pybind11::arg("wact") = pybind11::none(), pybind11::arg("wgrad") = pybind11::none());
+        pybind11::arg("wact") = pybind11::none(), pybind11::arg("wgrad") = pybind11::none(),
+        pybind11::arg("act_coef") = pybind11::none());
   m.doc() = "dtg gfx950 HIP kernels";
   m.def("sgd_apply", &sgd_apply);
   m.def("momentum_apply", &momentum_apply);
diff --git a/csrc/include/dtg/kernels.h b/csrc/include/dtg/kernels.h
--- a/csrc/include/dtg/kernels.h
+++ b/csrc/include/dtg/kernels.h
@@ -89,6 +89,10 @@
 void bn_fwd_from_part(const bf16_t* x, const bf16_t* res, bf16_t* y, const float* gamma, const float* beta,
                       float* rmean, float* rvar, float* smean, float* sinv, const float* part, float* ws, long long M,
                       int C, float momentum, float eps, int relu, hipStream_t st, uint8_t* bits = nullptr);
+void bn_fwd_coef_from_part(const float* part, const float* gamma, const float* beta, float* rmean, float* rvar,
+                           float* smean, float* sinv, float* coef, long long M, int C, float momentum, float eps,
+                           hipStream_t st);
+void bn_apply_from_coef(const bf16_t* x, bf16_t* y, const float* coef, long long M, int C, int relu, hipStream_t st);
 void bn_fwd2_from_part(const bf16_t* x, const bf16_t* r, bf16_t* y, const float* part, const float* part2,
                        const float* gamma, const float* beta, float* rmean, float* rvar, float* smean, float* sinv,
                        const float* gamma2, const float* beta2, float* rmean2, float* rvar2, float* smean2,
@@ -103,11 +107,12 @@
 void bn_dx_from_coef(const bf16_t* dp, const bf16_t* x, const float* coef, bf16_t* dx, bf16_t* dres, long long M, int C,
                      hipStream_t st);
 bool bn_dx_wgrad_ok(long long M, int C, int CI);
-int bn_dx_wgrad_slabs(int C, int CI, int w2 = 0);
+int bn_dx_wgrad_slabs(int C, int CI, int w2 = 0, int ta = 0);
 void bn_dx_wgrad(const bf16_t* dp, const bf16_t* x, const float* coef, const bf16_t* x2, const float* coef2,
                  bf16_t* dx, bf16_t* dx2, const bf16_t* act, long long ldact, void* wgrad, int wgrad_bf16,
                  float* slabs, long long M, int C, int CI, hipStream_t st, const bf16_t* act2 = nullptr,
-                 long long ldact2 = 0, void* wgrad2 = nullptr, float* slabs2 = nullptr);
+                 long long ldact2 = 0, void* wgrad2 = nullptr, float* slabs2 = nullptr,
+                 const float* act_coef = nullptr);
 void bn_bwd_from_part(const bf16_t* dp, const bf16_t* x, const float* gamma, const float* smean, const float* sinv,
                       const float* part, bf16_t* dx, bf16_t* dres, float* dgamma, float* dbeta, float* ws, long long M,
                       int C, int accum, hipStream_t st);
@@ -140,6 +145,10 @@
                int aux_mode = 0);
 void gemm_bf16_bn(const bf16_t* A, long long lda, const bf16_t* B, long long ldb, bf16_t* C, long long ldc, int M,
                   int N, int K, float beta, const BnEpi& bn, hipStream_t st);
+bool gemm_expand_inline_ok(long long M, int N, int K);
+bool gemm_expand_bn(const bf16_t* A, long long lda, const bf16_t* W, long long ldw, bf16_t* C, long long ldc, int M,
+                    int N, int K, float* part, hipStream_t st, int variant = 0, const float* a_coef = nullptr,
+                    uint8_t* a_bits = nullptr);
 void gemm_bf16_colsum(const bf16_t* A, long long lda, const bf16_t* B, long long ldb, bf16_t* C, long long ldc, int M,
                       int N, int K, const float* bias, int act, void* aux, int aux_mode, float* colsum, hipStream_t st);
 
diff --git a/csrc/kernels/batchnorm.hip b/csrc/kernels/batchnorm.hip
--- a/csrc/kernels/batchnorm.hip
+++ b/csrc/kernels/batchnorm.hip
@@ -315,6 +315,17 @@
   bn_finalize_kernel<16><<<(C + 63) / 64, 1024, 0, st>>>(part, kBnStatSlots, M, C, 0, gamma, beta, rmean, rvar, smean,
                                                     sinv, momentum, eps, ws, nullptr, nullptr, 1); DTG_LAUNCH_CHECK();
   bn_apply_launch(g, x, res, y, ws, M, C, relu, st, bits);
+}
+
+void bn_fwd_coef_from_part(const float* part, const float* gamma, const float* beta, float* rmean, float* rvar,
+                           float* smean, float* sinv, float* coef, long long M, int C, float momentum, float eps,
+                           hipStream_t st) {
+  bn_finalize_kernel<16><<<(C + 63) / 64, 1024, 0, st>>>(part, kBnStatSlots, M, C, 0, gamma, beta, rmean, rvar, smean,
+                                                    sinv, momentum, eps, coef, nullptr, nullptr, 1); DTG_LAUNCH_CHECK();
+}
+
+void bn_apply_from_coef(const bf16_t* x, bf16_t* y, const float* coef, long long M, int C, int relu, hipStream_t st) {
+  bn_apply_launch(bn_geom(M, C), x, nullptr, y, coef, M, C, relu, st);
 }
 
 __global__ void bn_infer_coef_kernel(const float* gamma, const float* beta, const float* rmean, const float* rvar,
diff --git a/csrc/kernels/bn_dx_wgrad.hip b/csrc/kernels/bn_dx_wgrad.hip
--- a/csrc/kernels/bn_dx_wgrad.hip
+++ b/csrc/kernels/bn_dx_wgrad.hip
@@ -12,7 +12,21 @@
 constexpr int kDR = 32;
 constexpr int kDX_LDS = kDR * kDC * 2;
 
-template <int CI, bool DUAL, bool W2 = false>
+__device__ __forceinline__ v8bf bn_relu_chan(const v8bf& y, float sc, float sh) {
+  const u32x4v u = __builtin_bit_cast(u32x4v, y);
+  u32x4v o;
+  o.x = pack_bf2(fmaxf(fmaf(__uint_as_float(u.x << 16), sc, sh), 0.f),
+                 fmaxf(fmaf(__uint_as_float(u.x & 0xffff0000u), sc, sh), 0.f));
+  o.y = pack_bf2(fmaxf(fmaf(__uint_as_float(u.y << 16), sc, sh), 0.f),
+                 fmaxf(fmaf(__uint_as_float(u.y & 0xffff0000u), sc, sh), 0.f));
+  o.z = pack_bf2(fmaxf(fmaf(__uint_as_float(u.z << 16), sc, sh), 0.f),
+                 fmaxf(fmaf(__uint_as_float(u.z & 0xffff0000u), sc, sh), 0.f));
+  o.w = pack_bf2(fmaxf(fmaf(__uint_as_float(u.w << 16), sc, sh), 0.f),
+                 fmaxf(fmaf(__uint_as_float(u.w & 0xffff0000u), sc, sh), 0.f));
+  return __builtin_bit_cast(v8bf, o);
+}
+
+template <int CI, bool DUAL, bool W2 = false, bool TA = false>
 __global__ void __launch_bounds__(256, (CI == 64 && !W2) ? 2 : 1) bn_dx_wgrad_kernel(const bf16_t* __restrict__ dp, const bf16_t* __restrict__ x,
                                                           const float* __restrict__ coef,
                                                           const bf16_t* __restrict__ x2,
@@ -20,7 +34,8 @@
                                                           bf16_t* __restrict__ dx2, const bf16_t* __restrict__ act,
                                                           long long ldact, float* __restrict__ slabs, int nblk,
                                                           int C, const bf16_t* __restrict__ act2, long long ldact2,
-                                                          float* __restrict__ slabs2) {
+                                                          float* __restrict__ slabs2,
+                                                          const float* __restrict__ act_coef) {
   static_assert(!W2 || (DUAL && CI == 64), "the second weight gradient is the dual form's, at 256 x 64");
   constexpr int kACT_LDS = kDR * CI * 2;
   constexpr int NJ = CI / 16;
@@ -45,6 +60,14 @@
     load8_f32(coef2 + C + c0, bx2);
     load8_f32(coef2 + 2 * C + c0, cc2);
   }
+  float asc[TA ? NJ : 1], ash[TA ? NJ : 1];
+  if constexpr (TA) {
+#pragma unroll
+    for (int j = 0; j < NJ; ++j) {
+      asc[j] = act_coef[j * 16 + (lane & 15)];
+      ash[j] = act_coef[CI + j * 16 + (lane & 15)];
+    }
+  }
   DenseMC<false> sa{act, ldact, CI, 0};
   DenseMC<false> sa2{act2, ldact2, CI, 0};
   f32x4 acc[4][NJ], acc2[W2 ? 4 : 1][W2 ? NJ : 1];
@@ -127,6 +150,10 @@
     for (int i = 0; i < 4; ++i) fa[i] = frag_mc<kDC>(sdx, wave * 64 + i * 16, 0, lane);
 #pragma unroll
     for (int j = 0; j < NJ; ++j) fb[j] = frag_mc<CI>(sact + slot * kACT_LDS, j * 16, 0, lane);
+    if constexpr (TA) {
+#pragma unroll
+      for (int j = 0; j < NJ; ++j) fb[j] = bn_relu_chan(fb[j], asc[j], ash[j]);
+    }
 #pragma unroll
     for (int i = 0; i < 4; ++i)
 #pragma unroll
@@ -166,14 +193,14 @@
   }
 }
 
-template <int CI, bool W2 = false>
+template <int CI, bool W2 = false, bool TA = false>
 int dx_wgrad_grid() {
   static int G = 0;
   if (G == 0) {
     int dev = 0, cus = 0, per_cu = 0;
     DTG_HIP_CHECK(hipGetDevice(&dev));
     DTG_HIP_CHECK(hipDeviceGetAttribute(&cus, hipDeviceAttributeMultiprocessorCount, dev));
-    DTG_HIP_CHECK(hipOccupancyMaxActiveBlocksPerMultiprocessor(&per_cu, bn_dx_wgrad_kernel<CI, true, W2>, 256, 0));
+    DTG_HIP_CHECK(hipOccupancyMaxActiveBlocksPerMultiprocessor(&per_cu, bn_dx_wgrad_kernel<CI, true, W2, TA>, 256, 0));
     G = cus * (per_cu < 1 ? 1 : (per_cu > 2 ? 2 : per_cu));
     G -= G % 8;
     if (G < 8) G = 8;
@@ -187,23 +214,36 @@
   return ((C == 256 && CI == 64) || (C == 512 && CI == 128)) && M % kDR == 0 && M >= 64LL * kDR;
 }
 
-int bn_dx_wgrad_slabs(int C, int CI, int w2) {
+int bn_dx_wgrad_slabs(int C, int CI, int w2, int ta) {
+  if (ta)
+    return (w2 ? dx_wgrad_grid<64, true, true>() : CI == 64 ? dx_wgrad_grid<64, false, true>()
+                                                             : dx_wgrad_grid<128, false, true>()) / (C / kDC);
   return (w2 ? dx_wgrad_grid<64, true>() : CI == 64 ? dx_wgrad_grid<64>() : dx_wgrad_grid<128>()) / (C / kDC);
 }
 
 void bn_dx_wgrad(const bf16_t* dp, const bf16_t* x, const float* coef, const bf16_t* x2, const float* coef2,
                  bf16_t* dx, bf16_t* dx2, const bf16_t* act, long long ldact, void* wgrad, int wgrad_bf16,
                  float* slabs, long long M, int C, int CI, hipStream_t st, const bf16_t* act2, long long ldact2,
-                 void* wgrad2, float* slabs2) {
+                 void* wgrad2, float* slabs2, const float* act_coef) {
   const int nblk = (int)(M / kDR);
   auto launch = [&](auto kern, int G) {
     hipLaunchKernelGGL(kern, dim3(G), dim3(256), 0, st, dp, x, coef, x2, coef2, dx, dx2, act, ldact, slabs, nblk, C,
-                       act2, ldact2, slabs2);
+                       act2, ldact2, slabs2, act_coef);
     DTG_LAUNCH_CHECK();
     return G;
   };
   int G;
-  if (act2) {
+  if (act_coef) {
+    if (act2) G = launch(bn_dx_wgrad_kernel<64, true, true, true>, dx_wgrad_grid<64, true, true>());
+    else if (CI == 64) G = x2 ? launch(bn_dx_wgrad_kernel<64, true, false, true>, dx_wgrad_grid<64, false, true>())
+                              : launch(bn_dx_wgrad_kernel<64, false, false, true>, dx_wgrad_grid<64, false, true>());
+    else G = x2 ? launch(bn_dx_wgrad_kernel<128, true, false, true>, dx_wgrad_grid<128, false, true>())
+                : launch(bn_dx_wgrad_kernel<128, false, false, true>, dx_wgrad_grid<128, false, true>());
+    if (act2) {
+      Epi e2{wgrad2, CI, wgrad_bf16, 1.f, 1.f, nullptr, 0};
+      gemm_splitk_reduce(slabs2, G / (C / kDC), C, CI, e2, st);
+    }
+  } else if (act2) {
     G = launch(bn_dx_wgrad_kernel<64, true, true>, dx_wgrad_grid<64, true>());
     Epi e2{wgrad2, CI, wgrad_bf16, 1.f, 1.f, nullptr, 0};
     gemm_splitk_reduce(slabs2, G / (C / kDC), C, CI, e2, st);
diff --git a/csrc/kernels/gemm.hip b/csrc/kernels/gemm.hip
--- a/csrc/kernels/gemm.hip
+++ b/csrc/kernels/gemm.hip
@@ -221,9 +221,6 @@
   else launch_bn_cfg<Cfg<128, 128, 1>, MODE>(A, lda, B, ldb, M, N, K, e, bn, st);
 }
 
-bool gemm_expand_bn(const bf16_t* A, long long lda, const bf16_t* W, long long ldw, bf16_t* C, long long ldc, int M,
-                    int N, int K, float* part, hipStream_t st, int variant);
-
 void gemm_bf16_bn(const bf16_t* A, long long lda, const bf16_t* B, long long ldb, bf16_t* C, long long ldc, int M,
                   int N, int K, float beta, const BnEpi& bn, hipStream_t st) {
   if (M <= 0 || N <= 0) return;
diff --git a/csrc/kernels/gemm_expand.hip b/csrc/kernels/gemm_expand.hip
--- a/csrc/kernels/gemm_expand.hip
+++ b/csrc/kernels/gemm_expand.hip
@@ -15,18 +15,50 @@
   FastDiv fPQ, fQ;
 };
 
-template <int K, bool NT, int MINB, bool S2 = false>
+typedef __attribute__((address_space(3))) f32x4 lds_f32x4;
+
+template <bool BITS>
+__device__ __forceinline__ v8bf bn_relu_frag(const v8bf& y, const lds_float* sc, const lds_float* sh, uint32_t& pos) {
+  const u32x4v u = __builtin_bit_cast(u32x4v, y);
+  const f32x4 s0 = *reinterpret_cast<const lds_f32x4*>(sc), s1 = *reinterpret_cast<const lds_f32x4*>(sc + 4);
+  const f32x4 h0 = *reinterpret_cast<const lds_f32x4*>(sh), h1 = *reinterpret_cast<const lds_f32x4*>(sh + 4);
+  float v[8];
+  v[0] = fmaxf(fmaf(__uint_as_float(u.x << 16), s0[0], h0[0]), 0.f);
+  v[1] = fmaxf(fmaf(__uint_as_float(u.x & 0xffff0000u), s0[1], h0[1]), 0.f);
+  v[2] = fmaxf(fmaf(__uint_as_float(u.y << 16), s0[2], h0[2]), 0.f);
+  v[3] = fmaxf(fmaf(__uint_as_float(u.y & 0xffff0000u), s0[3], h0[3]), 0.f);
+  v[4] = fmaxf(fmaf(__uint_as_float(u.z << 16), s1[0], h1[0]), 0.f);
+  v[5] = fmaxf(fmaf(__uint_as_float(u.z & 0xffff0000u), s1[1], h1[1]), 0.f);
+  v[6] = fmaxf(fmaf(__uint_as_float(u.w << 16), s1[2], h1[2]), 0.f);
+  v[7] = fmaxf(fmaf(__uint_as_float(u.w & 0xffff0000u), s1[3], h1[3]), 0.f);
+  if constexpr (BITS) {
+    pos = 0;
+#pragma unroll
+    for (int k = 0; k < 8; ++k) pos |= (v[k] > 0.f ? 1u : 0u) << k;
+  }
+  u32x4v o;
+  o.x = pack_bf2(v[0], v[1]);
+  o.y = pack_bf2(v[2], v[3]);
+  o.z = pack_bf2(v[4], v[5]);
+  o.w = pack_bf2(v[6], v[7]);
+  return __builtin_bit_cast(v8bf, o);
+}
+
+template <int K, bool NT, int MINB, bool S2 = false, bool TA = false>
 __global__ void __launch_bounds__(256, MINB > 0 ? MINB : 1) gemm_expand_bn_kernel(const bf16_t* __restrict__ A, long long lda,
                                                              const bf16_t* __restrict__ W, long long ldw,
                                                              bf16_t* __restrict__ C, long long ldc,
                                                              float* __restrict__ part, int N, int nslice, int tiles,
-                                                             ExpandGather gth) {
+                                                             ExpandGather gth, const float* __restrict__ coef,
+                                                             uint8_t* __restrict__ bits) {
+  static_assert(!TA || ((K == 64 || K == 128) && !S2), "the transformed operand: K = 64 / 128, dense rows");
   constexpr int KS = K / 32;
   constexpr int KH = K / 64;
   constexpr int BLK = kXR * K * 2;
   constexpr int D = KH * 2;
   constexpr int T = 8;
   __shared__ __attribute__((aligned(16))) char smem_raw[kXS * BLK];
+  __shared__ __attribute__((aligned(16))) float scoef_raw[TA ? 2 * K : 4];
   lds_char* smem = (lds_char*)smem_raw;
   const int tid = threadIdx.x, lane = tid & 63;
   const int wave = __builtin_amdgcn_readfirstlane(tid >> 6);
@@ -37,6 +69,12 @@
   const int slice = base % nslice;
   const int col0 = slice * 256 + wave * 64;
   const int q = lane & 15, g = lane >> 4;
+  const lds_float* scoef = (const lds_float*)scoef_raw;
+  const bool wb = TA && bits != nullptr && slice == 0;
+  if constexpr (TA) {
+    if (tid < 2 * K) ((lds_float*)scoef_raw)[tid] = coef[tid];
+    __syncthreads();
+  }
 
   v8bf wf[4][KS];
 #pragma unroll
@@ -79,8 +117,13 @@
   stage(1);
   for (int it = 0; it < my; ++it) {
     if (it == 0) asm volatile("s_waitcnt vmcnt(%0)" ::"n"(D) : "memory");
-    else if (it == 1) asm volatile("s_waitcnt vmcnt(%0)" ::"n"(D + T) : "memory");
-    else asm volatile("s_waitcnt vmcnt(%0)" ::"n"(2 * T + D) : "memory");
+    else if (it == 1) {
+      if (wb) asm volatile("s_waitcnt vmcnt(%0)" ::"n"(D + T + 1) : "memory");
+      else asm volatile("s_waitcnt vmcnt(%0)" ::"n"(D + T) : "memory");
+    } else {
+      if (wb) asm volatile("s_waitcnt vmcnt(%0)" ::"n"(2 * (T + 1) + D) : "memory");
+      else asm volatile("s_waitcnt vmcnt(%0)" ::"n"(2 * T + D) : "memory");
+    }
     __builtin_amdgcn_s_barrier();
     stage(it + 2);
     const lds_char* ta = smem + (it % kXS) * BLK;
@@ -90,6 +133,31 @@
       v8bf af[KS];
 #pragma unroll
       for (int ks = 0; ks < KS; ++ks) af[ks] = frag_kc(ta + (ks >> 1) * kXR * 128, 16 * i, ks & 1, lane);
+      if constexpr (TA) {
+        if (wb && i == wave) {
+          uint32_t mw[KS];
+#pragma unroll
+          for (int ks = 0; ks < KS; ++ks) {
+            uint32_t pos;
+            af[ks] = bn_relu_frag<true>(af[ks], scoef + ks * 32 + 8 * g, scoef + K + ks * 32 + 8 * g, pos);
+            uint32_t w = pos << (8 * g);
+            w |= __shfl_xor(w, 16, 64);
+            w |= __shfl_xor(w, 32, 64);
+            mw[ks] = w;
+          }
+          if (g == 0) {
+            uint8_t* bp = bits + (row0 + 16 * i + q) * (K / 8);
+            if constexpr (KS == 2) *reinterpret_cast<uint2*>(bp) = make_uint2(mw[0], mw[1]);
+            else *reinterpret_cast<uint4*>(bp) = make_uint4(mw[0], mw[1], mw[2], mw[3]);
+          }
+        } else {
+#pragma unroll
+          for (int ks = 0; ks < KS; ++ks) {
+            uint32_t pos;
+            af[ks] = bn_relu_frag<false>(af[ks], scoef + ks * 32 + 8 * g, scoef + K + ks * 32 + 8 * g, pos);
+          }
+        }
+      }
       f32x4 acc[4];
 #pragma unroll
       for (int j = 0; j < 4; ++j) acc[j] = __builtin_amdgcn_mfma_f32_16x16x32_bf16(wf[j][0], af[0], zero4, 0, 0, 0);
@@ -147,14 +215,14 @@
   }
 }
 
-template <int K, bool NT, int MINB, bool S2 = false>
+template <int K, bool NT, int MINB, bool S2 = false, bool TA = false>
 int expand_grid(int nslice) {
   static int per_cu = -1, cus = 0;
   if (per_cu < 0) {
     int dev = 0;
     DTG_HIP_CHECK(hipGetDevice(&dev));
     DTG_HIP_CHECK(hipDeviceGetAttribute(&cus, hipDeviceAttributeMultiprocessorCount, dev));
-    DTG_HIP_CHECK(hipOccupancyMaxActiveBlocksPerMultiprocessor(&per_cu, gemm_expand_bn_kernel<K, NT, MINB, S2>, 256, 0));
+    DTG_HIP_CHECK(hipOccupancyMaxActiveBlocksPerMultiprocessor(&per_cu, gemm_expand_bn_kernel<K, NT, MINB, S2, TA>, 256, 0));
     if (per_cu < 1) per_cu = 1;
   }
   int G = cus * per_cu;
@@ -287,8 +355,15 @@
 static int g_expand_k256 = 1;
 void gemm_expand_k256_set(int on) { g_expand_k256 = on; }
 
+bool gemm_expand_inline_ok(long long M, int N, int K) {
+  if ((K != 64 && K != 128) || N % 256 || M % kXR || M >= (1LL << 31)) return false;
+  if (M * N < (1LL << 24)) return false;
+  const int nslice = N / 256;
+  return (nslice & (nslice - 1)) == 0;
+}
+
 bool gemm_expand_bn(const bf16_t* A, long long lda, const bf16_t* W, long long ldw, bf16_t* C, long long ldc, int M,
-                    int N, int K, float* part, hipStream_t st, int variant) {
+                    int N, int K, float* part, hipStream_t st, int variant, const float* a_coef, uint8_t* a_bits) {
   if ((K != 64 && K != 128 && !(K == 256 && g_expand_k256)) || N % 256 || M % kXR || (lda & 7) || (ldw & 7) ||
       (ldc & 7))
     return false;
@@ -297,8 +372,17 @@
   if (nslice & (nslice - 1)) return false;
   const int tiles = (M / kXR) * nslice;
   auto launch = [&](auto kern, int G) {
-    hipLaunchKernelGGL(kern, dim3(G), dim3(256), 0, st, A, lda, W, ldw, C, ldc, part, N, nslice, tiles, ExpandGather());
+    hipLaunchKernelGGL(kern, dim3(G), dim3(256), 0, st, A, lda, W, ldw, C, ldc, part, N, nslice, tiles, ExpandGather(),
+                       a_coef, a_bits);
   };
+  if (a_coef) {
+    if (K == 64) launch(gemm_expand_bn_kernel<64, false, 0, false, true>, expand_grid<64, false, 0, false, true>(nslice));
+    else if (K == 128)
+      launch(gemm_expand_bn_kernel<128, false, 0, false, true>, expand_grid<128, false, 0, false, true>(nslice));
+    else return false;
+    DTG_LAUNCH_CHECK();
+    return true;
+  }
   if (K == 64) {
     if (variant == 1) launch(gemm_expand_bn_kernel<64, true, 0>, expand_grid<64, true, 0>(nslice));
     else if (variant == 2) launch(gemm_expand_bn_kernel<64, false, 3>, expand_grid<64, false, 3>(nslice));
@@ -334,7 +418,7 @@
   const int tiles = (int)(M / kXR) * nslice;
   hipLaunchKernelGGL((gemm_expand_bn_kernel<256, false, 0, true>), dim3(expand_grid<256, false, 0, true>(nslice)),
                      dim3(256), 0, st, x, (long long)Cin, w, (long long)Cin, y, (long long)Kout, part, Kout, nslice, tiles,
-                     gth);
+                     gth, (const float*)nullptr, (uint8_t*)nullptr);
   DTG_LAUNCH_CHECK();
   return true;
 }
diff --git a/distributed-tensorflow-guide_amd/models/resnet_fused.py b/distributed-tensorflow-guide_amd/models/resnet_fused.py
--- a/distributed-tensorflow-guide_amd/models/resnet_fused.py
+++ b/distributed-tensorflow-guide_amd/models/resnet_fused.py
@@ -30,6 +30,7 @@
 _SUB2 = True
 _DXW = True
 _DXW2 = True
+_BN2_INLINE = frozenset(int(v) for v in os.environ.get("DTG_BN2_INLINE", "64").split(",") if v.strip())
 
 
 class _Bn3Link:
@@ -85,6 +86,7 @@
         p_, q_ = (h + 2 - 3) // st + 1, (w + 2 - 3) // st + 1
         b1, b2, b3 = blk.c1.bn, blk.c2.bn, blk.c3.bn
         w1, w2, w3 = blk.c1.conv.weight, blk.c2.conv.weight, blk.c3.conv.weight
+        coef2 = None
         if _FUSE:
             y1, p1 = L.gemm_bn(x2, _mat(w1), 1, pooled=True)
             bits1 = _relu_bits(y1)
@@ -93,9 +95,16 @@
             y2, p2 = L.conv_fwd_bn(a1.view(n, h, w, width), _krsc(w2), st, 1, pooled=True)
             y2 = y2.view(-1, width)
             bits2 = _relu_bits(y2)
-            a2, m2, i2 = L.bn_fwd_part(y2, p2, None, b2.weight, b2.bias, b2.running_mean, b2.running_var,
-                                       b2.momentum, b2.eps, True, bits=bits2)
-            y3, p3 = L.gemm_bn(a2, _mat(w3), 1, pooled=True)
+            if (width in _BN2_INLINE and L.gemm_expand_inline_ok(y2.shape[0], cout, width)
+                    and L.bn_dx_wgrad_ok(y2.shape[0], cout, width)):
+                coef2, m2, i2 = L.bn_fwd_coef_part(p2, y2.shape[0], b2.weight, b2.bias, b2.running_mean,
+                                                   b2.running_var, b2.momentum, b2.eps)
+                a2 = None
+                y3, p3 = L.gemm_bn(y2, _mat(w3), 1, pooled=True, a_coef=coef2, a_bits=bits2)
+            else:
+                a2, m2, i2 = L.bn_fwd_part(y2, p2, None, b2.weight, b2.bias, b2.running_mean, b2.running_var,
+                                           b2.momentum, b2.eps, True, bits=bits2)
+                y3, p3 = L.gemm_bn(a2, _mat(w3), 1, pooled=True)
             ctx.bits12 = (bits1, bits2)
         else:
             y1 = gemm(x2, True, _mat(w1), True)
@@ -106,6 +115,7 @@
                                         b2.eps, True)
             y3 = gemm(a2, True, _mat(w3), True)
         yd = md = idd = None
+        ctx.coef2 = coef2
         if blk.down is not None:
             bd, wd = blk.down.bn, blk.down.conv.weight
             if _FUSE:
@@ -164,8 +174,12 @@
         do = _rows(dout)
         lk = ctx.link_out
         dyd = None
-        w3_kw = (dict(wact=a2, wgrad=g[id(w3)].view(cout, width))
-                 if _DXW and a2 is not None and L.bn_dx_wgrad_ok(y3.shape[0], cout, width) else None)
+        coef2, ctx.coef2 = ctx.coef2, None
+        w3_kw = None
+        if _DXW and L.bn_dx_wgrad_ok(y3.shape[0], cout, width):
+            w3_kw = dict(wact=a2, wgrad=g[id(w3)].view(cout, width))
+            if coef2 is not None:
+                w3_kw.update(wact=y2, act_coef=coef2)
         w3_done = wd_done = False
         if (lk is not None and lk.part is not None and do.data_ptr() == lk.dp.data_ptr()
                 and do.shape == lk.dp.shape):
@@ -202,6 +216,11 @@
             da2 = gemm(dy3, True, _mat(w3), False)
         if w3_done:
             pass
+        elif coef2 is not None:
+            with overlap.wgrad_scope(dy3, y2):
+                a2 = L.bn_apply_coef(y2, coef2, True)
+                _wgrad(dy3, a2, g[id(w3)].view(cout, width))
+                a2 = None
         else:
             with overlap.wgrad_scope(dy3, a2):
                 _wgrad(dy3, a2, g[id(w3)].view(cout, width))
```
